# sbelharbi/tcam-wsol-video

Hardware: AMD Instinct MI355X
Metric: frames/sec CAM+bbox, ResNet50-TCAM 224×224, 1/2/4/8 MI355X (higher is better)
Workload: dtype fp32

## Files before the change

include/tcam_hip.h:

```cpp
#ifndef TCAM_HIP_H
#define TCAM_HIP_H

#include <stdint.h>

#ifdef __cplusplus
extern "C" {
#endif

#define TCAM_OK 0
#define TCAM_E_ARG (-1)
#define TCAM_E_NOMEM (-2)

int tcam_abi_version(void);
const char* tcam_arch(void);

typedef struct tcam_conv_src {
    const float* ptr;
    int C, H, W;
    int stride;
    int up2;
} tcam_conv_src;

int tcam_conv_weight_dims(int K, int Cout, int* Kpad, int* Mpad);

int tcam_conv2d(const tcam_conv_src* srcs, int nsrc, int B,
                const float* wt, const float* bias, const float* residual,
                float* out, int Cout, int Hout, int Wout,
                int KH, int KW, int pad, int relu, void* stream);

int tcam_conv_force_tile(int id);

int tcam_conv_x6_weight_dims(int K, int Cout, int* Kpad, int* Mpad);
size_t tcam_conv_x6_ws_bytes(void);
int tcam_conv2d_x6(const tcam_conv_src* srcs, int nsrc, int B,
                   const void* wt, const float* bias, const void* residual,
                   void* out, int Cout, int Hout, int Wout,
                   int KH, int KW, int pad_h, int pad_w, int relu,
                   int out_cstride, int out_coff, void* ws, size_t ws_bytes,
                   void* stream);
typedef struct tcam_conv_dst {
    void* ptr;
    int c_begin, cstride, coff;
} tcam_conv_dst;
int tcam_conv2d_x6_multi(const tcam_conv_src* srcs, int nsrc, int B,
                         const void* wt, const float* bias, int Cout, int Hout, int Wout,
                         int KH, int KW, int pad_h, int pad_w, int relu,
                         const tcam_conv_dst* dst, int ndst, void* ws, size_t ws_bytes,
                         void* stream);
int tcam_conv_x6_force_tile(int id);
int tcam_conv_x6_force_streamk(int grid);
int tcam_conv_x6_debug(int flags);

int tcam_s3_from_nchw(const float* in, void* out, int B, int C, int H, int W, int Cpad,
                      void* stream);
int tcam_s3_to_nchw(const void* in, float* out, int B, int C, int H, int W, void* stream);
int tcam_maxpool3x3s2_s3(const void* in, void* out, int B, int C, int H, int W, int Ho,
                         int Wo, void* stream);
int tcam_pool2d_s3(const void* in, void* out, int B, int C, int H, int W, int Ho, int Wo,
                   int KH, int KW, int stride, int pad, int mode, int out_cstride,
                   int out_coff, void* stream);
int tcam_up2_resize_s3(const void* in, void* out, int B, int C, int H, int W, int Ho, int Wo,
                       void* stream);
size_t tcam_wgap_s3_ws_bytes(int B, int C, int HW);
int tcam_wgap_s3(const void* x, const float* fc_w, const float* fc_b, float* logits,
                 float* mean, float* ws, int B, int C, int HW, int classes, void* stream);
int tcam_seghead_cam_s3(const void* x, const float* w, const float* b, float* fcams,
                        float* cam, uint8_t* cam_u8, int B, int Cin, int H, int W,
                        int argmax, void* stream);
int tcam_resize_cam(const float* fcams_in, float* fcams_out, float* cam, uint8_t* cam_u8,
                    int B, int Hi, int Wi, int Ho, int Wo, int argmax, void* stream);

int tcam_resize_ac_bwd(const float* dout, float* din, int BC, int Hi, int Wi, int Ho, int Wo,
                       void* stream);
int tcam_std_cam_s3(const void* A, const float* fc_w, const int32_t* cls, float* low,
                    float* cam, uint8_t* cam_u8, int B, int C, int h, int w, int Ho, int Wo,
                    void* stream);

int tcam_conv2d_f16x3(const tcam_conv_src* srcs, int nsrc, int B, const void* wt,
                      const float* wscale, const float* bias, const void* residual, void* out,
                      int Cout, int Hout, int Wout, int KH, int KW, int pad_h, int pad_w,
                      int relu, int out_cstride, int out_coff, int* oflow, void* ws,
                      size_t ws_bytes, void* stream);
int tcam_conv2d_f16x3_multi(const tcam_conv_src* srcs, int nsrc, int B, const void* wt,
                            const float* wscale, const float* bias, int Cout, int Hout,
                            int Wout, int KH, int KW, int pad_h, int pad_w, int relu,
                            const tcam_conv_dst* dst, int ndst, int* oflow, void* ws,
                            size_t ws_bytes, void* stream);
typedef struct tcam_conv_prob {
    tcam_conv_src src;
    const void* wt;
    const float* wscale;
    const float* bias;
    void* out;
    int Cout, Hout, Wout, KH, KW, pad_h, pad_w, relu, out_cstride, out_coff;
} tcam_conv_prob;
int tcam_conv2d_group(const tcam_conv_prob* probs, int nprob, int B, int fmt, int tile,
                      int* oflow, void* stream);
int tcam_stem_window(int KH, int KW, int stride, int* IR, int* IC);
int tcam_stem_f16x3(const float* img, const void* wt, const float* wscale, const float* bias,
                    const int32_t* ktab, int nk, void* out, int B, int C, int H, int W,
                    int Cout, int KH, int KW, int stride, int pad, int* oflow, void* stream);
int tcam_s2_from_nchw(const float* in, void* out, int B, int C, int H, int W, int Cpad,
                      void* stream);
int tcam_s2_to_nchw(const void* in, float* out, int B, int C, int H, int W, void* stream);
int tcam_maxpool3x3s2_s2(const void* in, void* out, int B, int C, int H, int W, int Ho,
                         int Wo, void* stream);
int tcam_pool2d_s2(const void* in, void* out, int B, int C, int H, int W, int Ho, int Wo,
                   int KH, int KW, int stride, int pad, int mode, int out_cstride,
                   int out_coff, void* stream);
int tcam_up2_resize_s2(const void* in, void* out, int B, int C, int H, int W, int Ho, int Wo,
                       void* stream);
int tcam_wgap_s2(const void* x, const float* fc_w, const float* fc_b, float* logits,
                 float* mean, float* ws, int B, int C, int HW, int classes, void* stream);
int tcam_seghead_cam_s2(const void* x, const float* w, const float* b, float* fcams,
                        float* cam, uint8_t* cam_u8, int B, int Cin, int H, int W,
                        int argmax, void* stream);
int tcam_std_cam_s2(const void* A, const float* fc_w, const int32_t* cls, float* low,
                    float* cam, uint8_t* cam_u8, int B, int C, int h, int w, int Ho, int Wo,
                    void* stream);

int tcam_conv2d_f16(const tcam_conv_src* srcs, int nsrc, int B, const void* wt,
                    const float* bias, const void* residual, void* out, int Cout, int Hout,
                    int Wout, int KH, int KW, int pad_h, int pad_w, int relu, int out_cstride,
                    int out_coff, void* ws, size_t ws_bytes, void* stream);
int tcam_s1_from_nchw(const float* in, void* out, int B, int C, int H, int W, int Cpad,
                      void* stream);
int tcam_s1_to_nchw(const void* in, float* out, int B, int C, int H, int W, void* stream);
int tcam_maxpool3x3s2_s1(const void* in, void* out, int B, int C, int H, int W, int Ho,
                         int Wo, void* stream);
int tcam_pool2d_s1(const void* in, void* out, int B, int C, int H, int W, int Ho, int Wo,
                   int KH, int KW, int stride, int pad, int mode, int out_cstride,
                   int out_coff, void* stream);
int tcam_up2_resize_s1(const void* in, void* out, int B, int C, int H, int W, int Ho, int Wo,
                       void* stream);
int tcam_wgap_s1(const void* x, const float* fc_w, const float* fc_b, float* logits,
                 float* mean, float* ws, int B, int C, int HW, int classes, void* stream);
int tcam_seghead_cam_s1(const void* x, const float* w, const float* b, float* fcams,
                        float* cam, uint8_t* cam_u8, int B, int Cin, int H, int W,
                        int argmax, void* stream);
int tcam_std_cam_s1(const void* A, const float* fc_w, const int32_t* cls, float* low,
                    float* cam, uint8_t* cam_u8, int B, int C, int h, int w, int Ho, int Wo,
                    void* stream);

int tcam_maxpool3x3s2(const float* in, float* out, int B, int C, int H, int W,
                      int Ho, int Wo, void* stream);

int tcam_up2_resize(const float* in, float* out, int B, int C, int H, int W,
                    int Ho, int Wo, void* stream);

int tcam_wgap(const float* x, const float* fc_w, const float* fc_b,
              float* logits, float* ws, int B, int C, int HW, int classes,
              void* stream);

int tcam_seghead_cam(const float* x, const float* w, const float* b,
                     float* fcams, float* cam, uint8_t* cam_u8,
                     int B, int Cin, int H, int W, int argmax, void* stream);

int tcam_std_cam(const float* A, const float* fc_w, const int32_t* cls,
                 float* low, float* cam, uint8_t* cam_u8, int B, int C,
                 int h, int w, int Ho, int Wo, void* stream);

int tcam_temporal_max(const float* cams, const int32_t* idx, float* out,
                      int M, int k1, int hw, float t, void* stream);

int tcam_temporal_cam(const float* cams, int N, const int32_t* idx, float* out,
                      uint8_t* out_u8, int M, int k1, int hw, float t, float* scale_ws,
                      void* stream);

int tcam_topk_flags(const float* logits, const int32_t* target, int32_t* top1,
                    int32_t* top5, int B, int C, void* stream);

void tcam_bbox_set_chunks(int n);
size_t tcam_bbox_ws_bytes(int B, int H, int W);
int tcam_bbox_levels(const uint8_t* cam_u8, int32_t* boxes, int32_t* vmax,
                     void* ws, int B, int H, int W, void* stream);

int tcam_bbox_set_debug(uint64_t* buf);
int tcam_bbox_fill_variant(int v);
int tcam_s2_to_s3(const void* in, void* out, long groups, void* stream);
int tcam_s3_to_s2(const void* in, void* out, long groups, void* stream);
int tcam_bbox_scan_line(const uint8_t* p, const uint8_t* u, uint8_t* out, int n, int mode,
                        void* stream);
int tcam_bbox_level_variant(int v);
int tcam_bbox_set_inc_debug(uint64_t* buf);

int tcam_box_accumulate(const int32_t* boxes, const int32_t* vmax,
                        const double* taus, int T, const int32_t* gt,
                        const int32_t* ngt, int G, const int32_t* top1,
                        const int32_t* top5, const double* iou_thr, int n_iou,
                        int32_t* counters, double* best_iou, int B,
                        void* stream);

size_t tcam_bbox_multi_ws_bytes(int B, int H, int W);
int tcam_bbox_multi_iou(const uint8_t* cam_u8, const int32_t* gt, const int32_t* ngt, int G,
                        double* iou, int32_t* vmax, int32_t* canon, void* ws, int B, int H,
                        int W, void* stream);
int tcam_box_accumulate_multi(const double* iou, const int32_t* canon, const int32_t* vmax,
                              const double* taus, int T, const int32_t* gt,
                              const int32_t* ngt, int G, const int32_t* top1,
                              const int32_t* top5, const double* iou_thr, int n_iou,
                              int32_t* counters, double* best_iou, int B, void* stream);
size_t tcam_bbox_contours_ws_bytes(int H, int W);
int tcam_bbox_contours(const uint8_t* cam_u8, int level, int32_t* records, int cap,
                       int32_t* count, void* ws, int H, int W, void* stream);

int tcam_flag_count(const int32_t* flags, int B, int32_t* acc, void* stream);

size_t tcam_bilateral_ws_bytes(int N, int K, int H, int W, int dim);
int tcam_bilateral_batch(const float* images, const float* ins, float* outs,
                         void* ws, size_t ws_bytes, int N, int K, int H, int W,
                         float s_rgb, float s_xy, void* stream);

int tcam_bilateral_prepare(const float* images, void* ws, size_t ws_bytes, int N, int K,
                           int H, int W, float s_rgb, float s_xy, void* stream);
int tcam_bilateral_apply(const float* ins, float* outs, void* ws, size_t ws_bytes, int N,
                         int K, int H, int W, float s_rgb, float s_xy, void* stream);

int tcam_colorbilateral_batch(const float* images, const float* ins, float* outs,
                              void* ws, size_t ws_bytes, int N, int K, int H, int W,
                              float s_rgb, int dim, void* stream);

int tcam_bilateral_status(const void* ws, int N, int* status);
void tcam_bilateral_set_debug(void* dbg);

void bilateralfilter_batch(float* images, int len_images, float* ins,
                           int len_ins, float* outs, int len_outs, int N,
                           int K, int H, int W, float sigmargb,
                           float sigmaxy);
void colorbilateralfilter_batch(float* images, int len_images, float* ins,
                                int len_ins, float* outs, int len_outs, int N,
                                int K, int H, int W, float sigmargb, int DIM);

size_t tcam_crf_energy_ws_bytes(void);
int tcam_crf_energy(const float* seg, const float* as, long n, int N, float* loss,
                    float* ws, void* stream);
int tcam_crf_grad(const float* as, const float* grad_out, long n, int N, float* grad,
                  void* stream);


size_t tcam_bn_ws_bytes(long P, int C);
int tcam_bn_stats_s3(const void* y, long P, int C, float eps, float momentum, float* mean,
                     float* invstd, float* run_mean, float* run_var, void* ws, void* stream);
int tcam_bn_relu_s3(const void* y, const float* mean, const float* invstd, const float* gamma,
                    const float* beta, void* out, long P, int C, void* stream);
int tcam_bn_relu_bwd_s3(const void* dout, const void* out, const void* y, const float* mean,
                        const float* invstd, const float* gamma, void* dy, float* dgamma,
                        float* dbeta, long P, int C, void* ws, void* stream);
int tcam_up2_bwd_s3(const void* gup, void* gx, int B, int C, int H, int W, void* stream);
size_t tcam_conv_wgrad_ws_bytes(const tcam_conv_src* srcs, int nsrc, int B, int Cout,
                                int Hout, int Wout, int KH, int KW);
int tcam_conv_wgrad_s3(const tcam_conv_src* srcs, int nsrc, int B, const void* dy, int Cout,
                       int Hout, int Wout, int KH, int KW, int pad_h, int pad_w,
                       int cout_store, float* dw, void* ws, size_t ws_bytes, void* stream);
int tcam_conv_wgrad_s3_f16x3(const tcam_conv_src* srcs, int nsrc, int B, const void* dy,
                             int Cout, int Hout, int Wout, int KH, int KW, int pad_h, int pad_w,
                             int cout_store, float* dw, void* ws, size_t ws_bytes, int* oflow,
                             void* stream);
int tcam_bn_stats_s2(const void* y, long P, int C, float eps, float momentum, float* mean,
                     float* invstd, float* run_mean, float* run_var, void* ws, void* stream);
int tcam_bn_relu_s2(const void* y, const float* mean, const float* invstd, const float* gamma,
                    const float* beta, void* out, long P, int C, void* stream);
int tcam_bn_relu_bwd_s3s2(const void* dout, const void* out, const void* y, const float* mean,
                          const float* invstd, const float* gamma, void* dy, float* dgamma,
                          float* dbeta, long P, int C, void* ws, uint32_t* amax, void* stream);
int tcam_dy_scaled_s2(const void* dy, long P, int C, uint32_t* amax, int compute, float* scale,
                      void* dy2, void* stream);
size_t tcam_bn_bwd_scaled_ws_bytes(long P, int C);
int tcam_bn_relu_bwd_scaled_s3s2(const void* dout, const void* out, const void* y,
                                 const float* mean, const float* invstd, const float* gamma,
                                 const float* beta, void* dy3, void* dy2, float* scale,
                                 float* dgamma, float* dbeta, long P, int C, void* ws,
                                 void* stream);
int tcam_bn_relu_bwd_fused_s1(const void* dout, const void* out, const void* y,
                              const float* mean, const float* invstd, const float* gamma,
                              const float* beta, void* dy, float* dgamma, float* dbeta, long P,
                              int C, void* ws, void* stream);
int tcam_conv_wgrad_s2_f16x3(const tcam_conv_src* srcs, int nsrc, int B, const void* dy2,
                             const float* dscale, int Cout, int Hout, int Wout, int KH, int KW,
                             int pad_h, int pad_w, int cout_store, float* dw, void* ws,
                             size_t ws_bytes, void* stream);
int tcam_pack_weight_f16x3(const float* w, void* out, float* wscale, int mode, int CoutW,
                           int CtotW, int KH, int KW, int c0, int cout_sel, int cin_pad,
                           const float* kdiv, void* stream);
typedef struct tcam_pack_item {
    const float* w;
    void* out;
    float* wscale;
    const float* kdiv;
    int mode, CoutW, CtotW, KH, KW, c0, cout_sel, cin_pad;
} tcam_pack_item;
size_t tcam_pack_table_bytes(int n);
int tcam_pack_weights(const tcam_pack_item* items, int n, int f16x3, void* table, void* stream);
int tcam_bottleneck_f16x3(const void* x, int B, int H, int W, int cin, const void* w1,
                          const float* s1, const float* b1, const void* w2, const float* s2,
                          const float* b2, const void* w3, const float* s3, const float* b3,
                          int ds, void* out, int* oflow, void* stream);
int tcam_bottleneck_f16(const void* x, int B, int H, int W, int cin, const void* w1,
                        const float* b1, const void* w2, const float* b2, const void* w3,
                        const float* b3, int ds, void* out, void* stream);
void tcam_bottleneck_set_debug(void* dbg);
int tcam_conv2d_f16x3_s3out(const tcam_conv_src* srcs, int nsrc, int B, const void* wt,
                            const float* wscale, const float* bias, void* out, int Cout,
                            int Hout, int Wout, int KH, int KW, int pad_h, int pad_w, int relu,
                            int out_cstride, int out_coff, void* ws, size_t ws_bytes,
                            void* stream);
int tcam_timer_arm(void* start, void* stop);
int tcam_wgrad_force_fp32(int on);
int tcam_pack_weight_x6(const float* w, void* out, int mode, int CoutW, int CtotW, int KH,
                        int KW, int c0, int cout_sel, int cin_pad, void* stream);
int tcam_up2_resize_bwd_s3(const void* g, void* gx, int B, int C, int H, int W, int Ho, int Wo,
                           void* stream);
size_t tcam_chansum_ws_bytes(int B, int C, long HW);
int tcam_chansum_nchw(const float* x, int B, int C, long HW, float* out, void* ws,
                      void* stream);
int tcam_softmax2(const float* fcams, float* S, int B, long HW, void* stream);
size_t tcam_tcam_loss_ws_bytes(int B, long HW);
int tcam_tcam_losses(const float* fcams, const float* S, const int32_t* seeds, const float* AS,
                     int B, long HW, float lam_sl, float lam_crf, float lam_size, float elb_t,
                     float* losses, float* dfcams, void* ws, void* stream);
int tcam_tcam_losses_ex(const float* fcams, const float* S, const int32_t* seeds,
                        const float* AS, const float* gx, const float* extra, int B, long HW,
                        float lam_sl, float lam_crf, float lam_size, float elb_t, float* losses,
                        float* dfcams, void* ws, void* stream);
size_t tcam_tcam_loss_terms_ws_bytes(int B, long HW);
int tcam_tcam_losses_terms(const float* fcams, const float* S, const int32_t* seeds,
                           const float* AS, const float* gx, const float* extra,
                           const float* fg_size, const float* msk, int B, long HW,
                           float lam_sl, float lam_crf, float lam_size, float elb_t,
                           float lam_bgfg, float lam_fgsz, float lam_eob, float t_bgfg,
                           float t_fgsz, float t_eob, float eps, float* losses, float* dfcams,
                           void* ws, void* stream);
int tcam_teacher_stats(const float* cams, const uint8_t* roi, const int32_t* bbox, int B,
                       int H, int W, float* msk, float* fg_size, void* stream);
int tcam_mosaic_gather(const float* src, const int32_t* idx, int G, int L, int C, int H, int W,
                       float* out, void* stream);
int tcam_mosaic_scatter(const float* mosaic, const int32_t* occ_start, const int32_t* occ,
                        int B, int L, int C, int H, int W, float coef, int accumulate,
                        float* dst, void* stream);
int tcam_sgd_step(float* p, const float* g, float* buf, long n, float lr, float momentum,
                  float dampening, float weight_decay, int nesterov, int first,
                  float grad_scale, void* stream);
int tcam_sgd_step_gated(float* p, const float* g, float* buf, long n, float lr, float momentum,
                        float dampening, float weight_decay, int nesterov, float grad_scale,
                        const float* gate, int* steps, int* skipped, void* stream);

int tcam_bn_stats_s1(const void* y, long P, int C, float eps, float momentum, float* mean,
                     float* invstd, float* run_mean, float* run_var, void* ws, void* stream);
int tcam_bn_relu_s1(const void* y, const float* mean, const float* invstd, const float* gamma,
                    const float* beta, void* out, long P, int C, void* stream);
int tcam_bn_relu_bwd_s1(const void* dout, const void* out, const void* y, const float* mean,
                        const float* invstd, const float* gamma, void* dy, float* dgamma,
                        float* dbeta, long P, int C, void* ws, void* stream);
int tcam_up2_bwd_s1(const void* gup, void* gx, int B, int C, int H, int W, void* stream);
int tcam_up2_resize_bwd_s1(const void* g, void* gx, int B, int C, int H, int W, int Ho, int Wo,
                           void* stream);
int tcam_conv_wgrad_s1(const tcam_conv_src* srcs, int nsrc, int B, const void* dy, int Cout,
                       int Hout, int Wout, int KH, int KW, int pad_h, int pad_w,
                       int cout_store, float* dw, void* ws, size_t ws_bytes, void* stream);
int tcam_pack_weight_f16(const float* w, void* out, int mode, int CoutW, int CtotW, int KH,
                         int KW, int c0, int cout_sel, int cin_pad, void* stream);
int tcam_amp_unscale(float* g, long n, const float* scale, float* found_inf, void* stream);
int tcam_sgd_step_amp(float* p, const float* g, float* buf, long n, float lr, float momentum,
                      float dampening, float weight_decay, int nesterov, float grad_scale,
                      const float* gate, int* steps, int* skipped, float* scale, int* tracker,
                      float growth_factor, float backoff_factor, int growth_interval,
                      void* stream);

int tcam_bn_add_relu_s2(const void* y, const float* mean, const float* invstd, const float* gamma,
                        const float* beta, const void* yd, const float* meand,
                        const float* invstdd, const float* gammad, const float* betad,
                        const void* res, void* out, long P, int C, void* stream);
int tcam_bn_add_relu_s1(const void* y, const float* mean, const float* invstd, const float* gamma,
                        const float* beta, const void* yd, const float* meand,
                        const float* invstdd, const float* gammad, const float* betad,
                        const void* res, void* out, long P, int C, void* stream);
int tcam_grad_add_mask_s3s2(const void* a, const void* d, const void* o, void* r, long P, int C,
                            void* stream);
int tcam_grad_add_mask_s1(const void* a, const void* d, const void* o, void* r, long P, int C,
                          void* stream);
size_t tcam_maxpool_bwd_ws_bytes(int B, int C, int Ho, int Wo);
int tcam_maxpool3x3s2_bwd_s3s2(const void* gout, const void* x, void* gin, void* ws, int B, int C,
                               int H, int W, int Ho, int Wo, void* stream);
int tcam_maxpool3x3s2_bwd_s1(const void* gout, const void* x, void* gin, void* ws, int B, int C,
                             int H, int W, int Ho, int Wo, void* stream);
int tcam_zero_up2(const void* in, void* out, int gbytes, int B, int C, int H, int W, int Hi,
                  int Wi, void* stream);
int tcam_im2col(const void* x, void* out, int gbytes, int B, int C, int H, int W, int KH, int KW,
                int stride, int pad, int Ho, int Wo, void* stream);
size_t tcam_wgrad11_ws_bytes(int B, int Cin, int Hin, int Win, int stride, int Cout, int Ho,
                             int Wo);
int tcam_wgrad11_s2_f16x3(const void* x, int B, int Cin, int Hin, int Win, int stride,
                          const void* dy2, const float* dscale, int Cout, int Ho, int Wo,
                          float* dw, void* ws, size_t ws_bytes, void* stream);
int tcam_wgrad11_s1(const void* x, int B, int Cin, int Hin, int Win, int stride, const void* dy,
                    int Cout, int Ho, int Wo, float* dw, void* ws, size_t ws_bytes, void* stream);
size_t tcam_conv_wgrad_generic_ws_bytes(const tcam_conv_src* srcs, int nsrc, int B, int Cout,
                                        int Hout, int Wout, int KH, int KW);
int tcam_conv_wgrad_s3s2(const tcam_conv_src* srcs, int nsrc, int B, const void* dy, int Cout,
                         int Hout, int Wout, int KH, int KW, int pad_h, int pad_w,
                         int cout_store, float* dw, void* ws, size_t ws_bytes, void* stream);
size_t tcam_cls_pool_ws_bytes(int B, int C);
int tcam_cls_fwd_s2(const void* x, int B, long HW, int C, const float* w, const float* bias,
                    int K, float* pooled, float* logits, void* ws, void* stream);
int tcam_cls_fwd_s1(const void* x, int B, long HW, int C, const float* w, const float* bias,
                    int K, float* pooled, float* logits, void* ws, void* stream);
int tcam_ce_loss(const float* logits, const int32_t* labels, int B, int K, float lam,
                 const float* gscale, float* loss, float* dlogits, void* stream);
int tcam_cls_bwd(const float* dlogits, const float* pooled, const float* w, int B, int K, int C,
                 int r16, float* dw, float* db, float* dpooled, void* stream);
int tcam_pool_bwd_s3(const float* dpooled, int B, long HW, int C, void* dout, void* stream);
int tcam_pool_bwd_s1(const float* dpooled, int B, long HW, int C, void* dout, void* stream);

size_t tcam_relu_bwd_ws_bytes(long P, int C);
int tcam_relu_bwd_s3s2(const void* dout, const void* out, void* dz, float* db, uint32_t* amax,
                       long P, int C, void* ws, size_t ws_bytes, void* stream);
int tcam_relu_bwd_s1(const void* dout, const void* out, void* dz, float* db, uint32_t* amax,
                     long P, int C, void* ws, size_t ws_bytes, void* stream);
int tcam_maxpool2x2_bwd_s3s2(const void* gout, const void* x, void* gin, int B, int C, int H,
                             int W, int Ho, int Wo, void* stream);
int tcam_maxpool2x2_bwd_s1(const void* gout, const void* x, void* gin, int B, int C, int H, int W,
                           int Ho, int Wo, void* stream);

size_t tcam_seeder_ws_bytes(int B, int H, int W);
int tcam_prepare_std_cams(const float* cams, float* out, int B, int h, int w, int Ho, int Wo,
                          void* stream);
int tcam_tcam_seeder(const float* cams, const uint8_t* roi, int32_t* seeds, int B, int H,
                     int W, int seed_tech, int min_, int max_, float max_p, float min_p,
                     int fg_erode_k, int fg_erode_iter, int ksz, int ignore_idx,
                     int roi_method, double p_min_area_roi, int use_roi,
                     unsigned long long seed, unsigned long long offset, uint8_t* roi_out,
                     float* th_out, void* ws, size_t ws_bytes, void* stream);
int tcam_get_roi(const float* cams, int B, int H, int W, int roi_method,
                 double p_min_area_roi, double thresh, const double* thresh_b,
                 uint8_t* roi_out, int32_t* bbox_out, float* th_out, void* ws,
                 size_t ws_bytes, void* stream);
int tcam_stotsu_roi_thresh(const float* cams, int B, int h, int w, int S, float* th_out,
                           void* stream);

int tcam_resample_coeffs(int in_size, int out_size, int* bounds, int* kk);
int tcam_frames_preprocess(const uint8_t* frames, int B, int Hin, int Win, const int* bh,
                           const int* kh, int ksh, int Rw, const int* bv, const int* kv,
                           int ksv, int Rh, const int* crop, const uint8_t* flip, int th,
                           int tw, const float* mean3, const float* std3, float* norm,
                           float* raw, uint8_t* u8, void* stream);


#define TCAM_JPEG_E_NOTJPEG (-20)
#define TCAM_JPEG_E_UNSUPPORTED (-21)
#define TCAM_JPEG_E_CORRUPT (-22)
int tcam_jpeg_pack(const uint8_t* const* data, const size_t* len, int n, void* blob,
                   size_t cap, int64_t* sizes, int* dims);
int tcam_jpeg_decode(const void* host_blob, const void* dev_blob, void* ws, size_t ws_bytes,
                     uint8_t* out, void* stream);
int tcam_jpeg_debug_rounds(const void* host_blob, int* dev_rounds);

#ifdef __cplusplus
}
#endif
#endif
```

tcam_wsol_video_amd/_lib.py:

```python
from __future__ import annotations

import ctypes as C
import os

_HERE = os.path.dirname(os.path.abspath(__file__))
LIB_PATH = os.environ.get("TCAM_LIB_PATH") or os.path.join(_HERE, "libtcam_hip.so")

_lib = None


class NativeLibraryError(RuntimeError):
    pass


class tcam_conv_src(C.Structure):
    _fields_ = [("ptr", C.c_void_p), ("C", C.c_int), ("H", C.c_int), ("W", C.c_int),
                ("stride", C.c_int), ("up2", C.c_int)]


class tcam_pack_item(C.Structure):
    _fields_ = [("w", C.c_void_p), ("out", C.c_void_p), ("wscale", C.c_void_p),
                ("kdiv", C.c_void_p), ("mode", C.c_int), ("CoutW", C.c_int), ("CtotW", C.c_int),
                ("KH", C.c_int), ("KW", C.c_int), ("c0", C.c_int), ("cout_sel", C.c_int),
                ("cin_pad", C.c_int)]


class tcam_conv_dst(C.Structure):
    _fields_ = [("ptr", C.c_void_p), ("c_begin", C.c_int), ("cstride", C.c_int),
                ("coff", C.c_int)]


class tcam_conv_prob(C.Structure):
    _fields_ = [("src", tcam_conv_src), ("wt", C.c_void_p), ("wscale", C.c_void_p),
                ("bias", C.c_void_p), ("out", C.c_void_p)] + [
        (n, C.c_int) for n in ("Cout", "Hout", "Wout", "KH", "KW", "pad_h", "pad_w", "relu",
                               "out_cstride", "out_coff")]


_P = C.c_void_p
_I = C.c_int
_F = C.c_float

SIGNATURES = {
    "tcam_abi_version": (_I, []),
    "tcam_arch": (C.c_char_p, []),
    "tcam_conv2d": (_I, [C.POINTER(tcam_conv_src), _I, _I, _P, _P, _P, _P, _I, _I, _I,
                         _I, _I, _I, _I, _P]),
    "tcam_conv_weight_dims": (_I, [_I, _I, C.POINTER(_I), C.POINTER(_I)]),
    "tcam_conv_force_tile": (_I, [_I]),
    "tcam_conv2d_x6": (_I, [C.POINTER(tcam_conv_src), _I, _I, _P, _P, _P, _P, _I, _I, _I,
                            _I, _I, _I, _I, _I, _I, _I, _P, C.c_size_t, _P]),
    "tcam_conv2d_x6_multi": (_I, [C.POINTER(tcam_conv_src), _I, _I, _P, _P, _I, _I, _I, _I,
                                  _I, _I, _I, _I, C.POINTER(tcam_conv_dst), _I, _P, C.c_size_t,
                                  _P]),
    "tcam_conv2d_f16x3": (_I, [C.POINTER(tcam_conv_src), _I, _I, _P, _P, _P, _P, _P, _I, _I,
                               _I, _I, _I, _I, _I, _I, _I, _I, _P, _P, C.c_size_t, _P]),
    "tcam_conv2d_f16x3_multi": (_I, [C.POINTER(tcam_conv_src), _I, _I, _P, _P, _P, _I, _I,
                                     _I, _I, _I, _I, _I, _I, C.POINTER(tcam_conv_dst), _I, _P,
                                     _P, C.c_size_t, _P]),
    "tcam_conv2d_group": (_I, [C.POINTER(tcam_conv_prob), _I, _I, _I, _I, _P, _P]),
    "tcam_conv_x6_ws_bytes": (C.c_size_t, []),
    "tcam_conv_x6_weight_dims": (_I, [_I, _I, C.POINTER(_I), C.POINTER(_I)]),
    "tcam_conv_x6_force_tile": (_I, [_I]),
    "tcam_wgrad_force_fp32": (_I, [_I]),
    "tcam_resample_coeffs": (_I, [_I, _I, _P, _P]),
    "tcam_frames_preprocess": (_I, [_P, _I, _I, _I, _P, _P, _I, _I, _P, _P, _I, _I, _P, _P,
                                    _I, _I, C.POINTER(_F), C.POINTER(_F), _P, _P, _P, _P]),
    "tcam_jpeg_pack": (_I, [_P, _P, _I, _P, C.c_size_t, _P, _P]),
    "tcam_jpeg_decode": (_I, [_P, _P, _P, C.c_size_t, _P, _P]),
    "tcam_jpeg_debug_rounds": (_I, [_P, _P]),
    "tcam_conv_x6_force_streamk": (_I, [_I]),
    "tcam_conv_x6_debug": (_I, [_I]),
    "tcam_s3_from_nchw": (_I, [_P, _P, _I, _I, _I, _I, _I, _P]),
    "tcam_s3_to_nchw": (_I, [_P, _P, _I, _I, _I, _I, _P]),
    "tcam_maxpool3x3s2_s3": (_I, [_P, _P, _I, _I, _I, _I, _I, _I, _P]),
    "tcam_up2_resize_s3": (_I, [_P, _P, _I, _I, _I, _I, _I, _I, _P]),
    "tcam_pool2d_s3": (_I, [_P, _P, _I, _I, _I, _I, _I, _I, _I, _I, _I, _I, _I, _I, _I, _P]),
    "tcam_wgap_s3_ws_bytes": (C.c_size_t, [_I, _I, _I]),
    "tcam_wgap_s3": (_I, [_P, _P, _P, _P, _P, _P, _I, _I, _I, _I, _P]),
    "tcam_seghead_cam_s3": (_I, [_P, _P, _P, _P, _P, _P, _I, _I, _I, _I, _I, _P]),
    "tcam_resize_cam": (_I, [_P, _P, _P, _P, _I, _I, _I, _I, _I, _I, _P]),
    "tcam_resize_ac_bwd": (_I, [_P, _P, _I, _I, _I, _I, _I, _P]),
    "tcam_std_cam_s3": (_I, [_P, _P, _P, _P, _P, _P, _I, _I, _I, _I, _I, _I, _P]),
    "tcam_s2_from_nchw": (_I, [_P, _P, _I, _I, _I, _I, _I, _P]),
    "tcam_s2_to_nchw": (_I, [_P, _P, _I, _I, _I, _I, _P]),
    "tcam_maxpool3x3s2_s2": (_I, [_P, _P, _I, _I, _I, _I, _I, _I, _P]),
    "tcam_up2_resize_s2": (_I, [_P, _P, _I, _I, _I, _I, _I, _I, _P]),
    "tcam_pool2d_s2": (_I, [_P, _P, _I, _I, _I, _I, _I, _I, _I, _I, _I, _I, _I, _I, _I, _P]),
    "tcam_wgap_s2": (_I, [_P, _P, _P, _P, _P, _P, _I, _I, _I, _I, _P]),
    "tcam_seghead_cam_s2": (_I, [_P, _P, _P, _P, _P, _P, _I, _I, _I, _I, _I, _P]),
    "tcam_std_cam_s2": (_I, [_P, _P, _P, _P, _P, _P, _I, _I, _I, _I, _I, _I, _P]),
    "tcam_maxpool3x3s2": (_I, [_P, _P, _I, _I, _I, _I, _I, _I, _P]),
    "tcam_up2_resize": (_I, [_P, _P, _I, _I, _I, _I, _I, _I, _P]),
    "tcam_wgap": (_I, [_P, _P, _P, _P, _P, _I, _I, _I, _I, _P]),
    "tcam_seghead_cam": (_I, [_P, _P, _P, _P, _P, _P, _I, _I, _I, _I, _I, _P]),
    "tcam_std_cam": (_I, [_P, _P, _P, _P, _P, _P, _I, _I, _I, _I, _I, _I, _P]),
    "tcam_temporal_max": (_I, [_P, _P, _P, _I, _I, _I, _F, _P]),
    "tcam_temporal_cam": (_I, [_P, _I, _P, _P, _P, _I, _I, _I, _F, _P, _P]),
    "tcam_topk_flags": (_I, [_P, _P, _P, _P, _I, _I, _P]),
    "tcam_bbox_ws_bytes": (C.c_size_t, [_I, _I, _I]),
    "tcam_bbox_multi_ws_bytes": (C.c_size_t, [_I, _I, _I]),
    "tcam_bbox_multi_iou": (_I, [_P, _P, _P, _I, _P, _P, _P, _P, _I, _I, _I, _P]),
    "tcam_box_accumulate_multi": (_I, [_P, _P, _P, _P, _I, _P, _P, _I, _P, _P, _P, _I, _P, _P,
                                       _I, _P]),
    "tcam_bbox_contours_ws_bytes": (C.c_size_t, [_I, _I]),
    "tcam_bbox_contours": (_I, [_P, _I, _P, _I, _P, _P, _I, _I, _P]),
    "tcam_flag_count": (_I, [_P, _I, _P, _P]),
    "tcam_bbox_levels": (_I, [_P, _P, _P, _P, _I, _I, _I, _P]),
    "tcam_bbox_scan_line": (_I, [_P, _P, _P, _I, _I, _P]),
    "tcam_s2_to_s3": (_I, [_P, _P, C.c_long, _P]),
    "tcam_s3_to_s2": (_I, [_P, _P, C.c_long, _P]),
    "tcam_bbox_set_debug": (_I, [_P]),
    "tcam_bbox_fill_variant": (_I, [_I]),
    "tcam_bbox_level_variant": (_I, [_I]),
    "tcam_bbox_set_inc_debug": (_I, [_P]),
    "tcam_box_accumulate": (_I, [_P, _P, _P, _I, _P, _P, _I, _P, _P, _P, _I, _P, _P, _I,
                                 _P]),
    "tcam_bilateral_ws_bytes": (C.c_size_t, [_I, _I, _I, _I, _I]),
    "tcam_bilateral_batch": (_I, [_P, _P, _P, _P, C.c_size_t, _I, _I, _I, _I, _F, _F, _P]),
    "tcam_bilateral_prepare": (_I, [_P, _P, C.c_size_t, _I, _I, _I, _I, _F, _F, _P]),
    "tcam_bilateral_apply": (_I, [_P, _P, _P, C.c_size_t, _I, _I, _I, _I, _F, _F, _P]),
    "tcam_colorbilateral_batch": (_I, [_P, _P, _P, _P, C.c_size_t, _I, _I, _I, _I, _F, _I,
                                       _P]),
    "tcam_bilateral_status": (_I, [_P, _I, C.POINTER(_I)]),
    "tcam_bilateral_set_debug": (None, [_P]),
    "tcam_crf_energy_ws_bytes": (C.c_size_t, []),
    "tcam_bn_ws_bytes": (C.c_size_t, [C.c_long, _I]),
    "tcam_bn_stats_s3": (_I, [_P, C.c_long, _I, _F, _F, _P, _P, _P, _P, _P, _P]),
    "tcam_bn_relu_s3": (_I, [_P, _P, _P, _P, _P, _P, C.c_long, _I, _P]),
    "tcam_bn_relu_bwd_s3": (_I, [_P, _P, _P, _P, _P, _P, _P, _P, _P, C.c_long, _I, _P, _P]),
    "tcam_up2_bwd_s3": (_I, [_P, _P, _I, _I, _I, _I, _P]),
    "tcam_conv_wgrad_ws_bytes": (C.c_size_t, [C.POINTER(tcam_conv_src), _I, _I, _I, _I, _I,
                                              _I, _I]),
    "tcam_conv_wgrad_s3": (_I, [C.POINTER(tcam_conv_src), _I, _I, _P, _I, _I, _I, _I, _I, _I,
                                _I, _I, _P, _P, C.c_size_t, _P]),
    "tcam_timer_arm": (_I, [_P, _P]),
    "tcam_bn_stats_s2": (_I, [_P, C.c_long, _I, _F, _F, _P, _P, _P, _P, _P, _P]),
    "tcam_bn_relu_s2": (_I, [_P, _P, _P, _P, _P, _P, C.c_long, _I, _P]),
    "tcam_bn_relu_bwd_s3s2": (_I, [_P, _P, _P, _P, _P, _P, _P, _P, _P, C.c_long, _I, _P, _P,
                                   _P]),
    "tcam_dy_scaled_s2": (_I, [_P, C.c_long, _I, _P, _I, _P, _P, _P]),
    "tcam_bn_bwd_scaled_ws_bytes": (C.c_size_t, [C.c_long, _I]),
    "tcam_bn_relu_bwd_scaled_s3s2": (_I, [_P, _P, _P, _P, _P, _P, _P, _P, _P, _P, _P, _P,
                                          C.c_long, _I, _P, _P]),
    "tcam_bn_relu_bwd_fused_s1": (_I, [_P, _P, _P, _P, _P, _P, _P, _P, _P, _P, C.c_long, _I,
                                       _P, _P]),
    "tcam_conv_wgrad_s2_f16x3": (_I, [C.POINTER(tcam_conv_src), _I, _I, _P, _P, _I, _I, _I, _I,
                                      _I, _I, _I, _I, _P, _P, C.c_size_t, _P]),
    "tcam_pack_weight_f16x3": (_I, [_P, _P, _P, _I, _I, _I, _I, _I, _I, _I, _I, _P, _P]),
    "tcam_pack_table_bytes": (C.c_size_t, [_I]),
    "tcam_pack_weights": (_I, [_P, _I, _I, _P, _P]),
    "tcam_bottleneck_set_debug": (None, [_P]),
    "tcam_bbox_set_chunks": (None, [_I]),
    "tcam_bottleneck_f16": (_I, [_P, _I, _I, _I, _I, _P, _P, _P, _P, _P, _P, _I, _P, _P]),
    "tcam_bottleneck_f16x3": (_I, [_P, _I, _I, _I, _I, _P, _P, _P, _P, _P, _P, _P, _P, _P, _I,
                                   _P, _P, _P]),
    "tcam_conv2d_f16x3_s3out": (_I, [C.POINTER(tcam_conv_src), _I, _I, _P, _P, _P, _P, _I, _I,
                                     _I, _I, _I, _I, _I, _I, _I, _I, _P, C.c_size_t, _P]),
    "tcam_conv_wgrad_s3_f16x3": (_I, [C.POINTER(tcam_conv_src), _I, _I, _P, _I, _I, _I, _I, _I,
                                      _I, _I, _I, _P, _P, C.c_size_t, _P, _P]),
    "tcam_pack_weight_x6": (_I, [_P, _P, _I, _I, _I, _I, _I, _I, _I, _I, _P]),
    "tcam_up2_resize_bwd_s3": (_I, [_P, _P, _I, _I, _I, _I, _I, _I, _P]),
    "tcam_chansum_ws_bytes": (C.c_size_t, [_I, _I, C.c_long]),
    "tcam_chansum_nchw": (_I, [_P, _I, _I, C.c_long, _P, _P, _P]),
    "tcam_softmax2": (_I, [_P, _P, _I, C.c_long, _P]),
    "tcam_tcam_loss_ws_bytes": (C.c_size_t, [_I, C.c_long]),
    "tcam_tcam_losses": (_I, [_P, _P, _P, _P, _I, C.c_long, _F, _F, _F, _F, _P, _P, _P, _P]),
    "tcam_tcam_losses_ex": (_I, [_P, _P, _P, _P, _P, _P, _I, C.c_long, _F, _F, _F, _F, _P, _P,
                                 _P, _P]),
    "tcam_tcam_loss_terms_ws_bytes": (C.c_size_t, [_I, C.c_long]),
    "tcam_tcam_losses_terms": (_I, [_P, _P, _P, _P, _P, _P, _P, _P, _I, C.c_long] + [_F] * 11 +
                               [_P, _P, _P, _P]),
    "tcam_teacher_stats": (_I, [_P, _P, _P, _I, _I, _I, _P, _P, _P]),
    "tcam_mosaic_gather": (_I, [_P, _P, _I, _I, _I, _I, _I, _P, _P]),
    "tcam_mosaic_scatter": (_I, [_P, _P, _P, _I, _I, _I, _I, _I, _F, _I, _P, _P]),
    "tcam_sgd_step": (_I, [_P, _P, _P, C.c_long, _F, _F, _F, _F, _I, _I, _F, _P]),
    "tcam_sgd_step_gated": (_I, [_P, _P, _P, C.c_long, _F, _F, _F, _F, _I, _F, _P, _P, _P,
                                 _P]),
    "tcam_seeder_ws_bytes": (C.c_size_t, [_I, _I, _I]),
    "tcam_prepare_std_cams": (_I, [_P, _P, _I, _I, _I, _I, _I, _P]),
    "tcam_tcam_seeder": (_I, [_P, _P, _P, _I, _I, _I, _I, _I, _I, _F, _F, _I, _I, _I, _I, _I,
                              C.c_double, _I, C.c_ulonglong, C.c_ulonglong, _P, _P, _P,
                              C.c_size_t, _P]),
    "tcam_get_roi": (_I, [_P, _I, _I, _I, _I, C.c_double, C.c_double, _P, _P, _P, _P, _P,
                          C.c_size_t, _P]),
    "tcam_stotsu_roi_thresh": (_I, [_P, _I, _I, _I, _I, _P, _P]),
    "tcam_crf_energy": (_I, [_P, _P, C.c_long, _I, _P, _P, _P]),
    "tcam_crf_grad": (_I, [_P, _P, C.c_long, _I, _P, _P]),
    "tcam_stem_window": (_I, [_I, _I, _I, C.POINTER(_I), C.POINTER(_I)]),
    "tcam_stem_f16x3": (_I, [_P, _P, _P, _P, _P, _I, _P, _I, _I, _I, _I, _I, _I, _I, _I, _I,
                             _P, _P]),
    "tcam_conv2d_f16": (_I, [C.POINTER(tcam_conv_src), _I, _I, _P, _P, _P, _P, _I, _I, _I,
                             _I, _I, _I, _I, _I, _I, _I, _P, C.c_size_t, _P]),
    "tcam_s1_from_nchw": (_I, [_P, _P, _I, _I, _I, _I, _I, _P]),
    "tcam_s1_to_nchw": (_I, [_P, _P, _I, _I, _I, _I, _P]),
    "tcam_maxpool3x3s2_s1": (_I, [_P, _P, _I, _I, _I, _I, _I, _I, _P]),
    "tcam_up2_resize_s1": (_I, [_P, _P, _I, _I, _I, _I, _I, _I, _P]),
    "tcam_pool2d_s1": (_I, [_P, _P, _I, _I, _I, _I, _I, _I, _I, _I, _I, _I, _I, _I, _I, _P]),
    "tcam_wgap_s1": (_I, [_P, _P, _P, _P, _P, _P, _I, _I, _I, _I, _P]),
    "tcam_seghead_cam_s1": (_I, [_P, _P, _P, _P, _P, _P, _I, _I, _I, _I, _I, _P]),
    "tcam_std_cam_s1": (_I, [_P, _P, _P, _P, _P, _P, _I, _I, _I, _I, _I, _I, _P]),
    "tcam_bn_stats_s1": (_I, [_P, C.c_long, _I, _F, _F, _P, _P, _P, _P, _P, _P]),
    "tcam_bn_relu_s1": (_I, [_P, _P, _P, _P, _P, _P, C.c_long, _I, _P]),
    "tcam_bn_relu_bwd_s1": (_I, [_P, _P, _P, _P, _P, _P, _P, _P, _P, C.c_long, _I, _P, _P]),
    "tcam_up2_bwd_s1": (_I, [_P, _P, _I, _I, _I, _I, _P]),
    "tcam_up2_resize_bwd_s1": (_I, [_P, _P, _I, _I, _I, _I, _I, _I, _P]),
    "tcam_conv_wgrad_s1": (_I, [C.POINTER(tcam_conv_src), _I, _I, _P, _I, _I, _I, _I, _I, _I,
                                _I, _I, _P, _P, C.c_size_t, _P]),
    "tcam_pack_weight_f16": (_I, [_P, _P, _I, _I, _I, _I, _I, _I, _I, _I, _P]),
    "tcam_amp_unscale": (_I, [_P, C.c_long, _P, _P, _P]),
    "tcam_sgd_step_amp": (_I, [_P, _P, _P, C.c_long, _F, _F, _F, _F, _I, _F, _P, _P, _P, _P,
                               _P, _F, _F, _I, _P]),
    "tcam_bn_add_relu_s2": (_I, [_P, _P, _P, _P, _P, _P, _P, _P, _P, _P, _P, _P, C.c_long, _I,
                                 _P]),
    "tcam_bn_add_relu_s1": (_I, [_P, _P, _P, _P, _P, _P, _P, _P, _P, _P, _P, _P, C.c_long, _I,
                                 _P]),
    "tcam_grad_add_mask_s3s2": (_I, [_P, _P, _P, _P, C.c_long, _I, _P]),
    "tcam_grad_add_mask_s1": (_I, [_P, _P, _P, _P, C.c_long, _I, _P]),
    "tcam_maxpool_bwd_ws_bytes": (C.c_size_t, [_I, _I, _I, _I]),
    "tcam_maxpool3x3s2_bwd_s3s2": (_I, [_P, _P, _P, _P, _I, _I, _I, _I, _I, _I, _P]),
    "tcam_maxpool3x3s2_bwd_s1": (_I, [_P, _P, _P, _P, _I, _I, _I, _I, _I, _I, _P]),
    "tcam_zero_up2": (_I, [_P, _P, _I, _I, _I, _I, _I, _I, _I, _P]),
    "tcam_im2col": (_I, [_P, _P, _I, _I, _I, _I, _I, _I, _I, _I, _I, _I, _I, _P]),
    "tcam_wgrad11_ws_bytes": (C.c_size_t, [_I, _I, _I, _I, _I, _I, _I, _I]),
    "tcam_wgrad11_s2_f16x3": (_I, [_P, _I, _I, _I, _I, _I, _P, _P, _I, _I, _I, _P, _P,
                                   C.c_size_t, _P]),
    "tcam_wgrad11_s1": (_I, [_P, _I, _I, _I, _I, _I, _P, _I, _I, _I, _P, _P, C.c_size_t, _P]),
    "tcam_conv_wgrad_generic_ws_bytes": (C.c_size_t, [C.POINTER(tcam_conv_src), _I, _I, _I, _I,
                                                      _I, _I, _I]),
    "tcam_conv_wgrad_s3s2": (_I, [C.POINTER(tcam_conv_src), _I, _I, _P, _I, _I, _I, _I, _I, _I,
                                  _I, _I, _P, _P, C.c_size_t, _P]),
    "tcam_cls_pool_ws_bytes": (C.c_size_t, [_I, _I]),
    "tcam_cls_fwd_s2": (_I, [_P, _I, C.c_long, _I, _P, _P, _I, _P, _P, _P, _P]),
    "tcam_cls_fwd_s1": (_I, [_P, _I, C.c_long, _I, _P, _P, _I, _P, _P, _P, _P]),
    "tcam_ce_loss": (_I, [_P, _P, _I, _I, _F, _P, _P, _P, _P]),
    "tcam_cls_bwd": (_I, [_P, _P, _P, _I, _I, _I, _I, _P, _P, _P, _P]),
    "tcam_pool_bwd_s3": (_I, [_P, _I, C.c_long, _I, _P, _P]),
    "tcam_pool_bwd_s1": (_I, [_P, _I, C.c_long, _I, _P, _P]),
    "tcam_relu_bwd_ws_bytes": (C.c_size_t, [C.c_long, _I]),
    "tcam_relu_bwd_s3s2": (_I, [_P, _P, _P, _P, _P, C.c_long, _I, _P, C.c_size_t, _P]),
    "tcam_relu_bwd_s1": (_I, [_P, _P, _P, _P, _P, C.c_long, _I, _P, C.c_size_t, _P]),
    "tcam_maxpool2x2_bwd_s3s2": (_I, [_P, _P, _P, _I, _I, _I, _I, _I, _I, _P]),
    "tcam_maxpool2x2_bwd_s1": (_I, [_P, _P, _P, _I, _I, _I, _I, _I, _I, _P]),
    "bilateralfilter_batch": (None, [_P, _I, _P, _I, _P, _I, _I, _I, _I, _I, _F, _F]),
    "colorbilateralfilter_batch": (None, [_P, _I, _P, _I, _P, _I, _I, _I, _I, _I, _F, _I]),
}


def load(path: str = LIB_PATH):
    global _lib
    if _lib is not None:
        return _lib
    if not os.path.exists(path):
        raise NativeLibraryError(
            f"{path} not found: build it with `python -c 'import __graft_entry__ as g; "
            f"g.build()'` (hipcc --offload-arch=gfx950). There is no CPU fallback.")
    lib = C.CDLL(path)
    for name, (res, args) in SIGNATURES.items():
        fn = getattr(lib, name)
        fn.restype = res
        fn.argtypes = args
    _lib = lib
    return lib


def check(rc: int, what: str) -> None:
    if rc != 0:
        raise RuntimeError(f"{what} failed with code {rc}")
```

tcam_wsol_video_amd/csrc/bbox.hip:

```cpp
#include "common.h"

namespace {

constexpr int MAXH = 256, MAXW = 256;
constexpr int MAXP = 260;
constexpr int BIGH = 320, BIGW = 320;
constexpr int BIGP = 324;
constexpr uint32_t INACT = 0xFFFFFFFFu;
constexpr int NTB = 1024;
constexpr int DBG_SLOTS = 16;
uint64_t* g_dbg = nullptr;
int g_fill_waves = NTB / 64;
int g_fill_maxit = 1 << 30;
int g_fill_variant = 0;
int g_level_variant = 0;
int g_bbox_chunks = 0;
uint64_t* g_inc_dbg = nullptr;

__device__ inline uint64_t rt() { return __builtin_amdgcn_s_memrealtime(); }

__host__ __device__ inline int pitch_of(int W) {
    int d = (W + 3) / 4;
    if ((d & 1) == 0) d += 1;
    return 4 * d;
}

__device__ inline int block_max_i(int v, int* red) {
    v = wave_max_i(v);
    const int lane = threadIdx.x & 63, wid = threadIdx.x >> 6;
    __syncthreads();
    if (lane == 0) red[wid] = v;
    __syncthreads();
    if (threadIdx.x == 0) {
        int m = red[0];
        for (int i = 1; i < NTB / 64; ++i) m = max(m, red[i]);
        red[NTB / 64] = m;
    }
    __syncthreads();
    return red[NTB / 64];
}
__device__ inline int block_min_i(int v, int* red) {
    return -block_max_i(-v, red);
}

__device__ void emit_sorted(const uint8_t* psi, int P, const int* hist, int* cur, int H, int W,
                            int b, uint16_t* __restrict__ slist, int32_t* __restrict__ cgt) {
    const int tid = threadIdx.x, nt = blockDim.x;
    __syncthreads();
    if (tid < 64) {
        int h[4], own = 0;
#pragma unroll
        for (int k = 0; k < 4; ++k) {
            h[k] = hist[4 * tid + 1 + k];
            own += h[k];
        }
        int incl = own;
#pragma unroll
        for (int o = 1; o < 64; o <<= 1) {
            const int t = __shfl_down(incl, o, 64);
            if (tid + o < 64) incl += t;
        }
        int above = incl - own;
        int32_t* cg = cgt + (long)b * 257;
#pragma unroll
        for (int k = 3; k >= 0; --k) {
            above += h[k];
            cg[4 * tid + k] = above;
            cur[4 * tid + k] = above;
        }
        if (tid == 0) cg[256] = 0;
    }
    __syncthreads();
    uint16_t* out = slist + (long)b * H * W;
    for (int i = tid; i < H * W; i += nt) {
        const int y = i / W, x = i - y * W;
        const int v = psi[y * P + x];
        if (v) out[atomicAdd(&cur[v], 1)] = (uint16_t)(y << 8 | x);
    }
}

template <int MH, int MP, bool IMG_LDS>
__global__ __launch_bounds__(NTB) void fill_kernel(const uint8_t* __restrict__ cam_u8,
                                                   uint8_t* __restrict__ psi_out,
                                                   int32_t* __restrict__ vmax_out,
                                                   int32_t* __restrict__ canon,
                                                   int32_t* __restrict__ lev_list,
                                                   int32_t* __restrict__ nlev, int H, int W,
                                                   uint64_t* __restrict__ dbg,
                                                   uint16_t* __restrict__ slist,
                                                   int32_t* __restrict__ cgt) {
    const uint64_t t0 = rt();
    __shared__ uint8_t img[IMG_LDS ? MH * MP : 4];
    __shared__ uint8_t psi[MH * MP];
    __shared__ int red[NTB / 64 + 1];
    __shared__ int hist[257];
    __shared__ int cur[257];
    __shared__ int changed;
    const int b = blockIdx.x;
    const int P = pitch_of(W);
    const uint8_t* src = cam_u8 + (long)b * H * W;
    int vm = 0;
    for (int i0 = threadIdx.x; i0 < H * W; i0 += 8 * NTB) {
        uint8_t v[8];
#pragma unroll
        for (int u = 0; u < 8; ++u) {
            const int i = i0 + u * NTB;
            v[u] = i < H * W ? src[i] : 0;
        }
#pragma unroll
        for (int u = 0; u < 8; ++u) {
            const int i = i0 + u * NTB;
            if (i >= H * W) continue;
            const int y = i / W, x = i - y * W;
            if (IMG_LDS) img[y * P + x] = v[u];
            psi[y * P + x] = 255;
            vm = max(vm, (int)v[u]);
        }
    }
    vm = block_max_i(vm, red);
    if (threadIdx.x == 0) vmax_out[b] = vm;
    const uint64_t t1 = rt();
    int iters = 0;
    const int nd = (W + 3) / 4;
    for (;;) {
        if (threadIdx.x == 0) changed = 0;
        __syncthreads();
        int ch = 0;
        if (threadIdx.x < H) {
            uint32_t* prow = reinterpret_cast<uint32_t*>(psi + threadIdx.x * P);
            const uint32_t* irow = reinterpret_cast<const uint32_t*>(img + threadIdx.x * P);
            const uint8_t* grow = src + threadIdx.x * W;
            auto idw = [&](int d) -> uint32_t {
                if (IMG_LDS) return irow[d];
                uint32_t v = 0;
#pragma unroll
                for (int e = 0; e < 4; ++e)
                    if (4 * d + e < W) v |= (uint32_t)grow[4 * d + e] << (8 * e);
                return v;
            };
            int prev = -1;
            uint32_t pv = prow[0], iv = idw(0);
            for (int d = 0; d < nd; ++d) {
                const uint32_t pn = d + 1 < nd ? prow[d + 1] : 0u;
                const uint32_t in = d + 1 < nd ? idw(d + 1) : 0u;
                uint32_t o = pv;
#pragma unroll
                for (int e = 0; e < 4; ++e) {
                    if (4 * d + e < W) {
                        const int c = (pv >> (8 * e)) & 255, u = (iv >> (8 * e)) & 255;
                        const int nv = max(u, min(c, prev));
                        prev = nv;
                        o = (o & ~(255u << (8 * e))) | ((uint32_t)nv << (8 * e));
                    }
                }
                if (o != pv) { prow[d] = o; ch = 1; }
                pv = pn;
                iv = in;
            }
            prev = -1;
            pv = prow[nd - 1];
            iv = idw(nd - 1);
            for (int d = nd - 1; d >= 0; --d) {
                const uint32_t pn = d > 0 ? prow[d - 1] : 0u;
                const uint32_t in = d > 0 ? idw(d - 1) : 0u;
                uint32_t o = pv;
#pragma unroll
                for (int e = 3; e >= 0; --e) {
                    if (4 * d + e < W) {
                        const int c = (pv >> (8 * e)) & 255, u = (iv >> (8 * e)) & 255;
                        const int nv = max(u, min(c, prev));
                        prev = nv;
                        o = (o & ~(255u << (8 * e))) | ((uint32_t)nv << (8 * e));
                    }
                }
                if (o != pv) { prow[d] = o; ch = 1; }
                pv = pn;
                iv = in;
            }
        }
        __syncthreads();
        if (threadIdx.x < W) {
            const int x = threadIdx.x;
            auto iat = [&](int y) -> int {
                return IMG_LDS ? (int)img[y * P + x] : (int)src[y * W + x];
            };
            int prev = -1;
            int c[4], u[4], cn[4], un[4];
#pragma unroll
            for (int e = 0; e < 4; ++e) {
                c[e] = e < H ? psi[e * P + x] : 0;
                u[e] = e < H ? iat(e) : 0;
            }
            for (int y0 = 0; y0 < H; y0 += 4) {
#pragma unroll
                for (int e = 0; e < 4; ++e) {
                    const int y = y0 + 4 + e;
                    cn[e] = y < H ? psi[y * P + x] : 0;
                    un[e] = y < H ? iat(y) : 0;
                }
#pragma unroll
                for (int e = 0; e < 4; ++e) {
                    const int y = y0 + e;
                    if (y < H) {
                        const int nv = max(u[e], min(c[e], prev));
                        if (nv != c[e]) { psi[y * P + x] = (uint8_t)nv; ch = 1; }
                        prev = nv;
                    }
                }
#pragma unroll
                for (int e = 0; e < 4; ++e) { c[e] = cn[e]; u[e] = un[e]; }
            }
            prev = -1;
            const int top = ((H - 1) / 4) * 4;
#pragma unroll
            for (int e = 0; e < 4; ++e) {
                const int y = top + e;
                c[e] = y < H ? psi[y * P + x] : 0;
                u[e] = y < H ? iat(y) : 0;
            }
            for (int y0 = top; y0 >= 0; y0 -= 4) {
#pragma unroll
                for (int e = 0; e < 4; ++e) {
                    const int y = y0 - 4 + e;
                    cn[e] = y >= 0 ? psi[y * P + x] : 0;
                    un[e] = y >= 0 ? iat(y) : 0;
                }
#pragma unroll
                for (int e = 3; e >= 0; --e) {
                    const int y = y0 + e;
                    if (y < H) {
                        const int nv = max(u[e], min(c[e], prev));
                        if (nv != c[e]) { psi[y * P + x] = (uint8_t)nv; ch = 1; }
                        prev = nv;
                    }
                }
#pragma unroll
                for (int e = 0; e < 4; ++e) { c[e] = cn[e]; u[e] = un[e]; }
            }
        }
        if (ch) changed = 1;
        __syncthreads();
        ++iters;
        if (!__builtin_amdgcn_readfirstlane(changed)) break;
        __syncthreads();
    }
    const uint64_t t2 = rt();
    uint8_t* dst = psi_out + (long)b * H * W;
    for (int i = threadIdx.x; i < 257; i += NTB) hist[i] = 0;
    __syncthreads();
    for (int i = threadIdx.x; i < H * W; i += NTB) {
        int y = i / W, x = i - y * W;
        const uint8_t v = psi[y * P + x];
        dst[i] = v;
        atomicAdd(&hist[v], 1);
    }
    __syncthreads();
    if (threadIdx.x == 0) {
        int n = 0, next = vm - 1;
        for (int L = vm - 1; L >= 0; --L) {
            if (hist[L + 1] > 0) next = L;
            canon[b * 256 + L] = next;
        }
        for (int L = 0; L < vm; ++L)
            if (hist[L + 1] > 0) lev_list[b * 256 + n++] = L;
        nlev[b] = n;
        if (dbg) {
            uint64_t* d = dbg + (long)b * DBG_SLOTS;
            d[0] = t1 - t0; d[1] = t2 - t1; d[2] = rt() - t2; d[3] = iters; d[4] = n;
        }
    }
    if (slist) emit_sorted(psi, P, hist, cur, H, W, b, slist, cgt);
}

constexpr int NTF = 256;

template <int LDN>
__device__ __forceinline__ bool sweep_line(uint32_t (&pl)[LDN], const uint32_t (&ul)[LDN]) {
    uint32_t diff = 0;
    int prev = -1;
#pragma unroll
    for (int d = 0; d < LDN; ++d) {
        const uint32_t w = pl[d];
        uint32_t uw = ul[d];
        asm volatile("" : "+v"(uw));
        const int n0 = max((int)(uw & 255u), min((int)(w & 255u), prev));
        const int n1 = max((int)((uw >> 8) & 255u), min((int)((w >> 8) & 255u), n0));
        const int n2 = max((int)((uw >> 16) & 255u), min((int)((w >> 16) & 255u), n1));
        const int n3 = max((int)(uw >> 24), min((int)(w >> 24), n2));
        prev = n3;
        uint32_t o = (uint32_t)n0 | ((uint32_t)n1 << 8) | ((uint32_t)n2 << 16) |
                     ((uint32_t)n3 << 24);
        asm volatile("" : "+v"(o));
        diff |= o ^ w;
        pl[d] = o;
        __builtin_amdgcn_sched_barrier(0);
    }
    prev = -1;
#pragma unroll
    for (int d = LDN - 1; d >= 0; --d) {
        const uint32_t w = pl[d];
        uint32_t uw = ul[d];
        asm volatile("" : "+v"(uw));
        const int n3 = max((int)(uw >> 24), min((int)(w >> 24), prev));
        const int n2 = max((int)((uw >> 16) & 255u), min((int)((w >> 16) & 255u), n3));
        const int n1 = max((int)((uw >> 8) & 255u), min((int)((w >> 8) & 255u), n2));
        const int n0 = max((int)(uw & 255u), min((int)(w & 255u), n1));
        prev = n0;
        uint32_t o = (uint32_t)n0 | ((uint32_t)n1 << 8) | ((uint32_t)n2 << 16) |
                     ((uint32_t)n3 << 24);
        asm volatile("" : "+v"(o));
        diff |= o ^ w;
        pl[d] = o;
        __builtin_amdgcn_sched_barrier(0);
    }
    return diff != 0;
}

template <int LDN>
__global__ __launch_bounds__(NTF) void fill_reg_kernel(const uint8_t* __restrict__ cam_u8,
                                                       uint8_t* __restrict__ psi_out,
// ... 419 lines not shown
        a = find_root(lab, a);
        b = find_root(lab, b);
        if (a == b) return;
        if (a > b) { uint32_t t = a; a = b; b = t; }
        uint32_t old = atomicMin(&lab[b], a);
        if (old == b) return;
        b = old;
    }
}

struct LevelCtx {
    const uint32_t* bm;
    int H, W, wpr, BW;
    __device__ inline int bit(int y, int x) const {
        if ((unsigned)y >= (unsigned)H || (unsigned)x >= (unsigned)W) return 0;
        return (bm[y * wpr + (x >> 5)] >> (x & 31)) & 1;
    }
    __device__ inline int pair(int y, int x) const {
        if ((unsigned)y >= (unsigned)H || (unsigned)x >= (unsigned)W) return 0;
        return (bm[y * wpr + (x >> 5)] >> (x & 31)) & 3;
    }
    __device__ inline uint32_t word(int y, int j) const {
        if ((unsigned)y >= (unsigned)H || (unsigned)j >= (unsigned)wpr) return 0u;
        return bm[y * wpr + j];
    }
};

__device__ inline uint32_t root_of(const uint32_t* lab, uint32_t b) {
    uint32_t v = lab[b];
    return (v & RFLAG) ? b : v;
}

template <int LH, int LW, int QW>
__global__ __launch_bounds__(NTB) void level_kernel(const uint8_t* __restrict__ psi_g,
                                                    const int32_t* __restrict__ vmax,
                                                    const int32_t* __restrict__ lev_list,
                                                    const int32_t* __restrict__ nlev,
                                                    int32_t* __restrict__ boxes, int H, int W,
                                                    uint64_t* __restrict__ dbg) {
    uint64_t ph[8] = {0, 0, 0, 0, 0, 0, 0, 0};
    uint64_t tp = rt();
#define PHASE(k) do { if (dbg) { uint64_t t_ = rt(); ph[k] += t_ - tp; tp = t_; } } while (0)
    __shared__ uint32_t bm[LH * (LW / 32)];
    __shared__ uint32_t lab[(LH / 2) * (LW / 2)];
    __shared__ int red[4 * (NTB / 64) + 4];

    const int b = blockIdx.x / LEVEL_CHUNKS;
    const int chunk = blockIdx.x % LEVEL_CHUNKS;
    const int nl = __builtin_amdgcn_readfirstlane(nlev[b]);
    if (chunk >= nl) return;
    const int wpr = (W + 31) / 32;
    const int NW = H * wpr;
    const int BW = (W + 1) / 2, BH = (H + 1) / 2, NB = BH * BW;
    const int tid = threadIdx.x, lane = tid & 63, wid = tid >> 6;

    uint32_t pv[QW][8];
    const uint8_t* src = psi_g + (long)b * H * W;
#pragma unroll
    for (int q = 0; q < QW; ++q) {
        const int w = tid + q * NTB;
#pragma unroll
        for (int d = 0; d < 8; ++d) pv[q][d] = 0u;
        if (w < NW) {
            const int y = w / wpr, x0 = (w - y * wpr) * 32;
#pragma unroll
            for (int d = 0; d < 8; ++d) {
                uint32_t v = 0;
#pragma unroll
                for (int e = 0; e < 4; ++e) {
                    const int x = x0 + 4 * d + e;
                    if (x < W) v |= (uint32_t)src[y * W + x] << (8 * e);
                }
                pv[q][d] = v;
            }
        }
    }
    LevelCtx cx{bm, H, W, wpr, BW};

    for (int li = chunk; li < nl; li += LEVEL_CHUNKS) {
        const int L = lev_list[b * 256 + li];
        int32_t* box = boxes + ((long)b * 256 + L) * 4;
#pragma unroll
        for (int q = 0; q < QW; ++q) {
            const int w = tid + q * NTB;
            if (w < NW) {
                uint32_t bits = 0;
#pragma unroll
                for (int d = 0; d < 8; ++d)
#pragma unroll
                    for (int e = 0; e < 4; ++e)
                        bits |= (uint32_t)(((pv[q][d] >> (8 * e)) & 255u) > (uint32_t)L) << (4 * d + e);
                bm[w] = bits;
            }
        }
        __syncthreads();
        PHASE(0);
        for (int by = wid; by < BH; by += NTB / 64) {
            const int y = 2 * by;
            int carry = -1;
            for (int base = 0; base < BW; base += 64) {
                const int bx = base + lane;
                int t = 0, u = 0, tl = 0, ul = 0;
                if (bx < BW) {
                    t = cx.pair(y, 2 * bx);
                    u = cx.pair(y + 1, 2 * bx);
                    if (bx > 0) {
                        tl = cx.bit(y, 2 * bx - 1);
                        ul = cx.bit(y + 1, 2 * bx - 1);
                    }
                }
                const bool act = (t | u) != 0;
                const bool joined = act && ((t | u) & 1) && (tl | ul);
                const uint64_t starts = __ballot(act && !joined);
                const uint64_t acts = __ballot(act);
                const uint64_t below = lane == 63 ? starts : (starts & ((2ull << lane) - 1));
                int head = below ? base + 63 - __builtin_clzll(below) : carry;
                if (bx < BW) lab[by * BW + bx] = act ? (uint32_t)(by * BW + head) : INACT;
                const int last = __shfl(head, 63, 64);
                carry = ((acts >> 63) & 1) ? last : -1;
            }
        }
        __syncthreads();
        PHASE(1);
        for (int i0 = 0; i0 < NB; i0 += NTB) {
            const int i = i0 + tid;
            uint32_t hi = INACT, ht = INACT, hl = INACT, hr = INACT;
            if (i < NB && i >= BW) {
                hi = lab[i];
                if (hi != INACT) {
                    const int by = i / BW, bx = i - by * BW, y = 2 * by, x = 2 * bx;
                    const int top = cx.pair(y, x);
                    if (top) {
                        if (cx.pair(y - 1, x)) ht = lab[i - BW];
                        if (bx > 0 && (top & 1) && cx.bit(y - 1, x - 1)) hl = lab[i - BW - 1];
                        if (bx + 1 < BW && (top & 2) && cx.bit(y - 1, x + 2)) hr = lab[i - BW + 1];
                    }
                }
            }
            const uint32_t phi = __shfl_up(hi, 1, 64);
            const uint32_t pht = __shfl_up(ht, 1, 64);
            const uint32_t phr = __shfl_up(hr, 1, 64);
            const bool same_run = lane > 0 && phi == hi && (i % BW) != 0;
            auto seen = [&](uint32_t h) { return same_run && (h == pht || h == phr); };
            if (hi != INACT) {
                if (hl != INACT && !seen(hl)) unite(lab, hi, hl);
                if (ht != INACT && !seen(ht)) unite(lab, hi, ht);
                if (hr != INACT && !seen(hr)) unite(lab, hi, hr);
            }
        }
        __syncthreads();
        PHASE(2);
        for (;;) {
            int ch = 0;
            for (int i = tid; i < NB; i += NTB) {
                const uint32_t v = lab[i];
                if (v == INACT || v == (uint32_t)i) continue;
                const uint32_t w = lab[v];
                if (w != v) { lab[i] = w; ch = 1; }
            }
            ch = block_max_i(ch, red);
            if (!ch) break;
        }
        for (int i = tid; i < NB; i += NTB)
            if (lab[i] == (uint32_t)i) lab[i] = RFLAG;
        __syncthreads();
        PHASE(3);
        {
            const int nsj = (W + 1 + 31) / 32;
            const int nstrips = (H + 1) * nsj;
            const int per = (nstrips + NTB - 1) / NTB;
            uint32_t cr = INACT, cacc = 0;
            for (int st = tid * per; st < min(nstrips, (tid + 1) * per); ++st) {
                const int wy = st / nsj - 1, j = st % nsj;
                const uint32_t t0 = cx.word(wy, j), t1 = cx.word(wy + 1, j);
                const uint32_t tp = cx.word(wy, j - 1), bp = cx.word(wy + 1, j - 1);
                const uint32_t tl = (t0 << 1) | (tp >> 31), tr = t0;
                const uint32_t bl = (t1 << 1) | (bp >> 31), br = t1;
                uint32_t m3 = (tl & tr & (bl | br)) | (bl & br & (tl | tr));
                const uint32_t m4 = tl & tr & bl & br;
                const int nvalid = W + 1 - 32 * j;
                if (nvalid < 32) m3 &= (1u << nvalid) - 1u;
                while (m3) {
                    const int s0 = __builtin_ctz(m3);
                    const uint32_t rest = ~(m3 >> s0);
                    const int len = rest ? __builtin_ctz(rest) : 32 - s0;
                    const uint32_t run = (len >= 32 ? 0xFFFFFFFFu : ((1u << len) - 1u)) << s0;
                    const uint32_t contrib = __builtin_popcount(run) + __builtin_popcount(m4 & run);
                    const int wx = 32 * j - 1 + s0;
                    int py, px;
                    if ((tl >> s0) & 1) { py = wy; px = wx; }
                    else if ((tr >> s0) & 1) { py = wy; px = wx + 1; }
                    else if ((bl >> s0) & 1) { py = wy + 1; px = wx; }
                    else { py = wy + 1; px = wx + 1; }
                    const uint32_t r = root_of(lab, (py >> 1) * BW + (px >> 1));
                    if (r != cr) {
                        if (cr != INACT) atomicAdd(&lab[cr], cacc);
                        cr = r;
                        cacc = 0;
                    }
                    cacc += contrib;
                    m3 &= ~run;
                }
            }
            if (cr != INACT) atomicAdd(&lab[cr], cacc);
        }
        __syncthreads();
        PHASE(4);
        int ma = -1;
        for (int i = tid; i < NB; i += NTB) {
            const uint32_t v = lab[i];
            if (v != INACT && (v & RFLAG)) ma = max(ma, (int)(v & ~RFLAG));
        }
        ma = block_max_i(ma, red);
        for (int i = tid; i < NB; i += NTB) {
            const uint32_t v = lab[i];
            if (v != INACT && (v & RFLAG))
                lab[i] = ((int)(v & ~RFLAG) == ma) ? (RFLAG | 0x7FFFFFFEu) : NOKEY;
        }
        __syncthreads();
        for (int i = tid; i < NB; i += NTB) {
            if (lab[i] == INACT) continue;
            const uint32_t r = root_of(lab, i);
            const int by = i / BW;
            if ((int)r / BW != by || lab[r] == NOKEY) continue;
            const int x = 2 * (i - by * BW), y = 2 * by;
            const int top = cx.pair(y, x);
            int k;
            if (top & 1) k = y * W + x;
            else if (top & 2) k = y * W + x + 1;
            else if (cx.bit(y + 1, x)) k = (y + 1) * W + x;
            else k = (y + 1) * W + x + 1;
            atomicMin(&lab[r], RFLAG | (uint32_t)(k + 1));
        }
        __syncthreads();
        int best = 0;
        for (int i = tid; i < NB; i += NTB) {
            const uint32_t v = lab[i];
            if (v != INACT && (v & RFLAG) && v != NOKEY) best = max(best, (int)(v & ~RFLAG));
        }
        best = block_max_i(best, red);
        const int fp = best - 1;
        const uint32_t wroot = root_of(lab, ((fp / W) >> 1) * BW + ((fp % W) >> 1));
        PHASE(5);
        int x0 = W, y0 = H, x1 = -1, y1 = -1;
        for (int i = tid; i < NB; i += NTB) {
            if (lab[i] == INACT || root_of(lab, i) != wroot) continue;
            const int by = i / BW, x = 2 * (i - by * BW), y = 2 * by;
            const int top = cx.pair(y, x), bot = cx.pair(y + 1, x);
            if (top | bot) {
                x0 = min(x0, ((top | bot) & 1) ? x : x + 1);
                x1 = max(x1, ((top | bot) & 2) ? x + 1 : x);
                y0 = min(y0, top ? y : y + 1);
                y1 = max(y1, bot ? y + 1 : y);
            }
        }
        x0 = wave_min_i(x0); y0 = wave_min_i(y0);
        x1 = wave_max_i(x1); y1 = wave_max_i(y1);
        if (lane == 0) {
            red[4 * wid + 0] = x0; red[4 * wid + 1] = y0;
            red[4 * wid + 2] = x1; red[4 * wid + 3] = y1;
        }
        __syncthreads();
        if (tid == 0) {
            for (int w = 1; w < NTB / 64; ++w) {
                x0 = min(x0, red[4 * w + 0]); y0 = min(y0, red[4 * w + 1]);
                x1 = max(x1, red[4 * w + 2]); y1 = max(y1, red[4 * w + 3]);
            }
            box[0] = x0;
            box[1] = y0;
            box[2] = min(x1 + 1, W - 1);
            box[3] = min(y1 + 1, H - 1);
        }
        __syncthreads();
        PHASE(6);
    }
    if (dbg && tid == 0) {
        uint64_t* d = dbg + (long)(gridDim.x + blockIdx.x) * DBG_SLOTS;
        for (int k = 0; k < 7; ++k) d[k] = ph[k];
    }
#undef PHASE
}

__global__ void expand_kernel(const int32_t* __restrict__ canon, const int32_t* __restrict__ vmax,
                              int32_t* __restrict__ boxes, int B) {
    const int i = blockIdx.x * blockDim.x + threadIdx.x;
    if (i >= B * 256) return;
    const int b = i / 256, L = i % 256;
    if (L >= vmax[b]) return;
    const int c = canon[b * 256 + L];
    if (c == L) return;
    const int32_t* s = boxes + ((long)b * 256 + c) * 4;
    int32_t* d = boxes + ((long)b * 256 + L) * 4;
    d[0] = s[0]; d[1] = s[1]; d[2] = s[2]; d[3] = s[3];
}

__global__ void accumulate_kernel(const int32_t* __restrict__ boxes,
                                  const int32_t* __restrict__ vmax, const double* __restrict__ taus,
                                  int T, const int32_t* __restrict__ gt,
                                  const int32_t* __restrict__ ngt, int G,
                                  const int32_t* __restrict__ top1,
                                  const int32_t* __restrict__ top5,
                                  const double* __restrict__ iou_thr, int n_iou,
                                  int32_t* __restrict__ counters, double* __restrict__ best_iou,
                                  int B) {
    long id = (long)blockIdx.x * blockDim.x + threadIdx.x;
    if (id >= (long)B * T) return;
    const int b = (int)(id / T), i = (int)(id % T);
    const int vm = vmax[b];
    const int thr = (int)(taus[i] * (double)vm);
    int a0 = 0, a1 = 0, a2 = 0, a3 = 0;
    if (thr < vm) {
        const int32_t* bx = boxes + ((long)b * 256 + thr) * 4;
        a0 = bx[0]; a1 = bx[1]; a2 = bx[2]; a3 = bx[3];
    }
    double best = 0.0;
    const int ng = ngt[b];
    for (int g = 0; g < ng; ++g) {
        const int32_t* q = gt + ((long)b * G + g) * 4;
        long mnx = max(a0, q[0]), mny = max(a1, q[1]);
        long mxx = min(a2, q[2]), mxy = min(a3, q[3]);
        long inter = max(0L, mxx - mnx + 1) * max(0L, mxy - mny + 1);
        long area_a = (long)(a2 - a0 + 1) * (a3 - a1 + 1);
        long area_b = (long)(q[2] - q[0] + 1) * (q[3] - q[1] + 1);
        long den = area_a + area_b - inter;
        double iou = den <= 0 ? 0.0 : (double)inter / (double)den;
        if (g == 0 || iou > best) best = iou;
    }
    if (best_iou) best_iou[id] = best;
    for (int j = 0; j < n_iou; ++j) {
        if (best >= iou_thr[j]) {
            atomicAdd(&counters[(0 * n_iou + j) * T + i], 1);
            if (top1[b]) atomicAdd(&counters[(1 * n_iou + j) * T + i], 1);
            if (top5[b]) atomicAdd(&counters[(2 * n_iou + j) * T + i], 1);
        }
    }
}


constexpr int INC_CHUNKS = 1;
constexpr int INC_MAX_CHUNKS = 4;
constexpr int IH = 224, IW = 224, IWPR = 7, IBW = 112, INB = IBW * (IH / 2);

__device__ inline unsigned long long block_max_u64(unsigned long long v,
                                                   unsigned long long* red) {
#pragma unroll
    for (int o = 32; o > 0; o >>= 1) {
        const unsigned long long t = __shfl_xor(v, o, 64);
        v = t > v ? t : v;
    }
    const int lane = threadIdx.x & 63, wid = threadIdx.x >> 6;
    __syncthreads();
    if (lane == 0) red[wid] = v;
    __syncthreads();
    if (threadIdx.x == 0) {
        unsigned long long m = red[0];
        for (int i = 1; i < NTB / 64; ++i) m = red[i] > m ? red[i] : m;
        red[NTB / 64] = m;
    }
    __syncthreads();
    return red[NTB / 64];
}

constexpr int32_t AFLAG = 1 << 30, AMASK = AFLAG - 1;
constexpr int LCAP = INB * 2;

__device__ inline uint32_t find_root_pk(const uint32_t* pk, uint32_t x) {
    uint32_t p = pk[x] >> 16;
    while (p != x) {
        x = p;
        p = pk[x] >> 16;
    }
    return x;
}

__device__ inline void unite_pk(uint32_t* pk, uint32_t a, uint32_t b, uint32_t* hl, int* nh) {
    for (;;) {
        a = find_root_pk(pk, a);
        b = find_root_pk(pk, b);
        if (a == b) return;
        if (a > b) { uint32_t t = a; a = b; b = t; }
        const uint32_t old = atomicMin(&pk[b], a << 16 | 0xFFFFu);
        if ((old >> 16) == b) {
            hl[atomicAdd(nh, 1)] = b << 16 | (old & 0xFFFFu);
            return;
        }
        b = old >> 16;
    }
}

__device__ inline int win_contrib(int c) { return c == 4 ? 2 : (c == 3 ? 1 : 0); }

__global__ __launch_bounds__(NTB) void level_inc_kernel(const uint8_t* __restrict__ psi_g,
                                                        const int32_t* __restrict__ lev_list,
                                                        const int32_t* __restrict__ nlev,
                                                        int32_t* __restrict__ boxes, int H,
                                                        int W, uint32_t* __restrict__ plist_g,
                                                        uint32_t* __restrict__ hlist_g,
                                                        uint64_t* __restrict__ dbg, int nch) {
    uint64_t ph[8] = {0, 0, 0, 0, 0, 0, 0, 0};
    uint32_t n_full = 0, n_fallback = 0;
    uint64_t tp = rt();
#define IPHASE(k) do { if (dbg) { uint64_t t_ = rt(); ph[k] += t_ - tp; tp = t_; } } while (0)
    __shared__ uint32_t bm[IH * IWPR];
    __shared__ uint32_t db[IH * IWPR];
    __shared__ uint32_t pk[INB];
    __shared__ int32_t area[INB];
    __shared__ uint16_t lst[LCAP];
    __shared__ unsigned long long redl[NTB / 64 + 1];
    __shared__ int red[4 * (NTB / 64) + 4];
    __shared__ int wsum[NTB / 64 + 1];
    __shared__ int s_nhook;
    __shared__ unsigned long long s_pbest;
    const int b = blockIdx.x / nch, chunk = blockIdx.x % nch;
    uint32_t* plist = plist_g + (long)blockIdx.x * IH * IW;
    uint32_t* hlist = hlist_g + (long)blockIdx.x * INB;
    const int nl = __builtin_amdgcn_readfirstlane(nlev[b]);
    const int l0 = nl * chunk / nch, l1 = nl * (chunk + 1) / nch;
    if (l0 >= l1) return;
    const int wpr = (W + 31) / 32, NW = H * wpr;
    const int BW = (W + 1) / 2, BH = (H + 1) / 2, NB = BH * BW;
    const int tid = threadIdx.x, lane = tid & 63, wid = tid >> 6;
    constexpr int QW = 2;

    uint32_t pv[QW][8];
    const uint8_t* src = psi_g + (long)b * H * W;
#pragma unroll
    for (int q = 0; q < QW; ++q) {
        const int w = tid + q * NTB;
#pragma unroll
        for (int d = 0; d < 8; ++d) pv[q][d] = 0u;
        if (w < NW) {
            const int y = w / wpr, x0 = (w - y * wpr) * 32;
#pragma unroll
            for (int d = 0; d < 8; ++d) {
                uint32_t v = 0;
#pragma unroll
                for (int e = 0; e < 4; ++e) {
                    const int x = x0 + 4 * d + e;
                    if (x < W) v |= (uint32_t)src[y * W + x] << (8 * e);
                }
                pv[q][d] = v;
            }
        }
    }
    for (int i = tid; i < NB; i += NTB) {
        pk[i] = INACT;
        area[i] = 0;
    }
    if (tid == 0) s_pbest = 0;
    uint32_t ob[QW] = {0u, 0u};
    LevelCtx cx{bm, H, W, wpr, BW};
    uint32_t pwin = INACT;
    int bx0 = 0, by0 = 0, bx1 = 0, by1 = 0;
    auto isnew = [&](int y, int x) -> int {
        if ((unsigned)y >= (unsigned)H || (unsigned)x >= (unsigned)W) return 0;
        return (db[y * wpr + (x >> 5)] >> (x & 31)) & 1;
    };

    for (int li = l1 - 1; li >= l0; --li) {
        const int L = lev_list[b * 256 + li];
        uint32_t nb[QW], df[QW];
#pragma unroll
        for (int q = 0; q < QW; ++q) {
            const int w = tid + q * NTB;
            uint32_t bits = 0;
#pragma unroll
            for (int d = 0; d < 8; ++d)
#pragma unroll
                for (int e = 0; e < 4; ++e)
                    bits |= (uint32_t)(((pv[q][d] >> (8 * e)) & 255u) > (uint32_t)L) << (4 * d + e);
            nb[q] = w < NW ? bits : 0u;
            df[q] = nb[q] & ~ob[q];
            if (w < NW) {
                bm[w] = nb[q];
                db[w] = df[q];
            }
        }
        int cnt = __builtin_popcount(df[0]) + __builtin_popcount(df[1]);
        int incl = cnt;
#pragma unroll
        for (int o = 1; o < 64; o <<= 1) {
            const int t = __shfl_up(incl, o, 64);
            if (lane >= o) incl += t;
        }
        if (lane == 63) wsum[wid] = incl;
        __syncthreads();
        if (tid == 0) {
            s_nhook = 0;
            int acc = 0;
            for (int i = 0; i < NTB / 64; ++i) {
                const int t = wsum[i];
                wsum[i] = acc;
                acc += t;
            }
            wsum[NTB / 64] = acc;
        }
        __syncthreads();
        const int nnew = wsum[NTB / 64];
        const bool inl = nnew <= LCAP;
        {
            int pos = wsum[wid] + incl - cnt;
#pragma unroll
            for (int q = 0; q < QW; ++q) {
                uint32_t bits = df[q];
                const int w = tid + q * NTB, y = w / wpr, xb = (w - y * wpr) * 32;
                while (bits) {
                    const int x = xb + __builtin_ctz(bits);
                    bits &= bits - 1;
                    if (inl) lst[pos++] = (uint16_t)(y << 8 | x);
                    else plist[pos++] = (uint32_t)(y << 8 | x);
                }
            }
        }
        __syncthreads();
        const volatile uint32_t* plv = plist;
        auto newpx = [&](int it) -> uint32_t { return inl ? (uint32_t)lst[it] : plv[it]; };
        IPHASE(0);
        for (int it = tid; it < nnew; it += NTB) {
            const uint32_t pp = newpx(it);
            const int y = (int)(pp >> 8), x = (int)(pp & 255);
            const uint32_t blk = (y >> 1) * BW + (x >> 1);
            if (pk[blk] == INACT) pk[blk] = blk << 16 | 0xFFFFu;
        }
        __syncthreads();
        IPHASE(1);
        for (int it = tid; it < nnew * 8; it += NTB) {
            const uint32_t pp = newpx(it >> 3);
            const int y = (int)(pp >> 8), x = (int)(pp & 255);
            const int d = (it & 7) + ((it & 7) >= 4);
            const int dy = d / 3 - 1, dx = d % 3 - 1;
            if (!cx.bit(y + dy, x + dx)) continue;
            const uint32_t blk = (y >> 1) * BW + (x >> 1);
            const uint32_t nbk = ((y + dy) >> 1) * BW + ((x + dx) >> 1);
            if (nbk != blk) unite_pk(pk, blk, nbk, hlist, &s_nhook);
        }
        __syncthreads();
        IPHASE(2);
        const int nhook = s_nhook;
        const volatile uint32_t* hlv = hlist;
        for (int it = tid; it < nhook; it += NTB) {
            const uint32_t e = hlv[it], i = e >> 16, k = e & 0xFFFFu;
            if (k != 0xFFFFu) {
                const uint32_t r = find_root_pk(pk, i);
                atomicAdd(&area[r], area[i] & AMASK);
                atomicOr(&area[r], AFLAG);
                atomicMin(&pk[r], r << 16 | k);
                area[i] = 0;
            }
        }
        IPHASE(3);
        for (int it = tid; it < nnew * 4; it += NTB) {
            const uint32_t pp = newpx(it >> 2);
            const int y = (int)(pp >> 8), x = (int)(pp & 255);
            {
                const uint32_t r = find_root_pk(pk, (y >> 1) * BW + (x >> 1));
                if ((it & 3) == 0) atomicMin(&pk[r], r << 16 | (uint32_t)(y * W + x));
                int dsum = 0;
                {
                    const int wy = y - 1 + ((it >> 1) & 1), wx = x - 1 + (it & 1);
                    {
                        int cn = 0, co = 0;
                        bool owner = true;
#pragma unroll
                        for (int k = 0; k < 4; ++k) {
                            const int qy = wy + (k >> 1), qx = wx + (k & 1);
                            const int nbit = cx.bit(qy, qx), nw = isnew(qy, qx);
                            cn += nbit;
                            co += nbit & (nw ^ 1);
                            if (nw && (qy < y || (qy == y && qx < x))) owner = false;
                        }
                        if (owner) dsum += win_contrib(cn) - win_contrib(co);
                    }
                }
                if (dsum) atomicAdd(&area[r], dsum);
            }
        }
        __syncthreads();
        IPHASE(4);
#pragma unroll
        for (int q = 0; q < QW; ++q) ob[q] = nb[q];
        unsigned long long best = 0;
        auto cand = [&](uint32_t x) {
            const uint32_t r = find_root_pk(pk, x);
            if (r != x) pk[x] = r << 16 | 0xFFFFu;
            const unsigned long long a =
                ((unsigned long long)(uint32_t)(area[r] & AMASK) << 32) | (pk[r] & 0xFFFFu);
            best = a > best ? a : best;
        };
        for (int it = tid; it < nnew; it += NTB) {
            const uint32_t pp = newpx(it);
            cand(((pp >> 8) >> 1) * BW + ((pp & 255) >> 1));
        }
        for (int it = tid; it < nhook; it += NTB) cand(hlv[it] >> 16);
        if (tid == 0 && pwin != INACT) cand(pwin);
        IPHASE(5);
        best = block_max_u64(best, redl);
        if (__builtin_amdgcn_readfirstlane((int)(best < s_pbest))) {
            ++n_fallback;
            best = 0;
            for (int i = tid; i < NB; i += NTB) {
                const uint32_t v = pk[i];
                if ((v >> 16) == (uint32_t)i) {
                    const unsigned long long a =
                        ((unsigned long long)(uint32_t)(area[i] & AMASK) << 32) | (v & 0xFFFFu);
                    best = a > best ? a : best;
                }
            }
            best = block_max_u64(best, redl);
        }
        const uint32_t fp = (uint32_t)best;
        const uint32_t wb = ((fp / W) >> 1) * BW + ((fp % W) >> 1);
        const uint32_t wroot = find_root_pk(pk, wb);
        IPHASE(6);
        const bool grow = wroot == pwin && !(area[wroot] & AFLAG);
        n_full += grow ? 0 : 1;
        int x0 = W, y0 = H, x1 = -1, y1 = -1;
        if (grow) {
            for (int it = tid; it < nnew; it += NTB) {
                const uint32_t pp = newpx(it);
                const int y = (int)(pp >> 8), x = (int)(pp & 255);
                if ((pk[(y >> 1) * BW + (x >> 1)] >> 16) != wroot) continue;
                x0 = min(x0, x); x1 = max(x1, x);
                y0 = min(y0, y); y1 = max(y1, y);
            }
            if (tid == 0) {
                x0 = min(x0, bx0); y0 = min(y0, by0);
                x1 = max(x1, bx1); y1 = max(y1, by1);
            }
        } else
        for (int i = tid; i < NB; i += NTB) {
            const uint32_t w = pk[i];
            if (w == INACT) continue;
            const uint32_t v = w >> 16;
            const uint32_t r = v == (uint32_t)i ? v : find_root_pk(pk, i);
            if (r != v) pk[i] = r << 16 | 0xFFFFu;
            if (r != wroot) continue;
            const int by = i / BW, x = 2 * (i - by * BW), y = 2 * by;
            const int top = cx.pair(y, x), bot = cx.pair(y + 1, x);
            if (top | bot) {
                x0 = min(x0, ((top | bot) & 1) ? x : x + 1);
                x1 = max(x1, ((top | bot) & 2) ? x + 1 : x);
                y0 = min(y0, top ? y : y + 1);
                y1 = max(y1, bot ? y + 1 : y);
            }
        }
        x0 = wave_min_i(x0); y0 = wave_min_i(y0);
        x1 = wave_max_i(x1); y1 = wave_max_i(y1);
        if (lane == 0) {
            red[4 * wid + 0] = x0; red[4 * wid + 1] = y0;
            red[4 * wid + 2] = x1; red[4 * wid + 3] = y1;
        }
        __syncthreads();
        if (tid == 0) {
            for (int w = 1; w < NTB / 64; ++w) {
                x0 = min(x0, red[4 * w + 0]); y0 = min(y0, red[4 * w + 1]);
                x1 = max(x1, red[4 * w + 2]); y1 = max(y1, red[4 * w + 3]);
            }
            int32_t* box = boxes + ((long)b * 256 + L) * 4;
            box[0] = x0;
            box[1] = y0;
            box[2] = min(x1 + 1, W - 1);
            box[3] = min(y1 + 1, H - 1);
            bx0 = x0; by0 = y0; bx1 = x1; by1 = y1;
            area[wroot] &= AMASK;
            s_pbest = best;
        }
        pwin = wroot;
        __syncthreads();
        IPHASE(7);
    }
    if (dbg && tid == 0) {
        uint64_t* d = dbg + (long)blockIdx.x * DBG_SLOTS;
        for (int k = 0; k < 8; ++k) d[k] = ph[k];
        d[8] = l1 - l0;
        d[9] = n_full;
        d[10] = n_fallback;
    }
#undef IPHASE
}

constexpr int SCAP = INB;
constexpr uint32_t SAMASK = (1u << 17) - 1;
constexpr uint32_t XR_EMPTY = 0x00FFu;

__device__ inline uint32_t lds_ld(const uint32_t* p) { return *(const volatile uint32_t*)p; }

__device__ inline void ar_max_y1(uint32_t* w, uint32_t y) {
    uint32_t old = lds_ld(w);
    while ((old >> 24) < y) {
        const uint32_t prev = atomicCAS(w, old, (old & 0x00FFFFFFu) | (y << 24));
        if (prev == old) return;
        old = prev;
    }
}

__device__ inline void xr_widen(uint32_t* xr, uint32_t r, uint32_t x0, uint32_t x1) {
    uint32_t* w = xr + (r >> 1);
    const int sh = (int)(r & 1u) * 16;
    uint32_t old = lds_ld(w);
    for (;;) {
        const uint32_t cur = (old >> sh) & 0xFFFFu;
        const uint32_t nv = min(cur & 255u, x0) | max(cur >> 8, x1) << 8;
        if (nv == cur) return;
        const uint32_t prev = atomicCAS(w, old, (old & ~(0xFFFFu << sh)) | (nv << sh));
        if (prev == old) return;
        old = prev;
    }
}

__device__ inline unsigned long long block_max_u64_all(unsigned long long v,
                                                       unsigned long long* red) {
#pragma unroll
    for (int o = 32; o > 0; o >>= 1) {
        const unsigned long long t = __shfl_xor(v, o, 64);
        v = t > v ? t : v;
    }
    __syncthreads();
    if ((threadIdx.x & 63) == 0) red[threadIdx.x >> 6] = v;
    __syncthreads();
#pragma unroll
    for (int i = 0; i < NTB / 64; ++i) v = red[i] > v ? red[i] : v;
    return v;
}

__global__ __launch_bounds__(NTB) void level_sorted_kernel(
    const uint16_t* __restrict__ slist_g, const int32_t* __restrict__ cgt_g,
    const int32_t* __restrict__ lev_list, const int32_t* __restrict__ nlev,
    int32_t* __restrict__ boxes, int H, int W, uint32_t* __restrict__ hlist_g,
    uint64_t* __restrict__ dbg, int nch, int compress) {
    uint64_t ph[8] = {0, 0, 0, 0, 0, 0, 0, 0};
    uint32_t n_comp = 0, n_fallback = 0;
    uint64_t tp = rt();
#define SPHASE(k) do { if (dbg) { uint64_t t_ = rt(); ph[k] += t_ - tp; tp = t_; } } while (0)
    __shared__ uint32_t bm[IH * IWPR];
    __shared__ uint32_t db[IH * IWPR];
    __shared__ uint32_t pk[INB];
    __shared__ uint32_t ar[INB];
    __shared__ uint32_t xr[INB / 2];
    __shared__ uint16_t lst[SCAP];
    __shared__ unsigned long long redl[NTB / 64 + 1];
    __shared__ int s_nhook, s_nmerge;
    __shared__ unsigned long long s_pbest, s_best;
    const int b = blockIdx.x / nch, chunk = blockIdx.x % nch;
    uint32_t* hlist = hlist_g + (long)blockIdx.x * INB;
    const uint16_t* slist = slist_g + (long)b * H * W;
    const int32_t* cgt = cgt_g + (long)b * 257;
    const int nl = __builtin_amdgcn_readfirstlane(nlev[b]);
    const int l0 = nl * chunk / nch, l1 = nl * (chunk + 1) / nch;
    if (l0 >= l1) return;
    const int wpr = (W + 31) / 32, NW = H * wpr;
    const int BW = (W + 1) / 2, BH = (H + 1) / 2, NB = BH * BW;
    const int tid = threadIdx.x, lane = tid & 63, wid = tid >> 6;
    for (int i = tid; i < NB; i += NTB) {
        pk[i] = INACT;
        ar[i] = 0;
    }
    for (int i = tid; i < (NB + 1) / 2; i += NTB) xr[i] = XR_EMPTY | XR_EMPTY << 16;
    for (int w = tid; w < NW; w += NTB) bm[w] = 0u;
    if (tid == 0) s_pbest = 0;
    LevelCtx cx{bm, H, W, wpr, BW};
    uint32_t pwin = INACT;
    auto isnew = [&](int y, int x) -> int {
        if ((unsigned)y >= (unsigned)H || (unsigned)x >= (unsigned)W) return 0;
        return (db[y * wpr + (x >> 5)] >> (x & 31)) & 1;
    };
    int s_hi = 0;

    for (int li = l1 - 1; li >= l0; --li) {
        const int L = __builtin_amdgcn_readfirstlane(lev_list[b * 256 + li]);
        const int s0 = s_hi, s1 = min(max(__builtin_amdgcn_readfirstlane(cgt[L]), s0), H * W);
        s_hi = s1;
        const int nnew = s1 - s0;
        const bool inl = nnew <= SCAP;
        for (int w = tid; w < NW; w += NTB) db[w] = 0u;
        if (tid == 0) {
            s_nhook = 0;
            s_nmerge = 0;
            s_best = 0;
        }
        __syncthreads();
        SPHASE(0);
        for (int it = tid; it < nnew; it += NTB) {
            const uint32_t pp = slist[s0 + it];
            if (inl) lst[it] = (uint16_t)pp;
            const int y = (int)(pp >> 8), x = (int)(pp & 255);
            const uint32_t bit = 1u << (x & 31);
            atomicOr(&bm[y * wpr + (x >> 5)], bit);
            atomicOr(&db[y * wpr + (x >> 5)], bit);
            const uint32_t blk = (y >> 1) * BW + (x >> 1);
            if (pk[blk] == INACT) pk[blk] = blk << 16 | 0xFFFFu;
        }
        __syncthreads();
        auto newpx = [&](int it) -> uint32_t { return inl ? (uint32_t)lst[it] : slist[s0 + it]; };
        SPHASE(1);
        for (int it = tid; it < nnew * 3; it += NTB) {
            const int q = it / 3, k = it - 3 * q;
            const uint32_t pp = newpx(q);
            const int y = (int)(pp >> 8), x = (int)(pp & 255);
            const int sy = (y & 1) ? 1 : -1, sx = (x & 1) ? 1 : -1;
            int ny, nx, set;
            if (k == 0) {
                ny = y; nx = x + sx;
                set = cx.bit(y, nx) | cx.bit(y - sy, nx);
            } else if (k == 1) {
                ny = y + sy; nx = x;
                set = cx.bit(ny, x) | cx.bit(ny, x - sx);
            } else {
                ny = y + sy; nx = x + sx;
                set = cx.bit(ny, nx);
            }
            if (set)
                unite_pk(pk, (y >> 1) * BW + (x >> 1), (ny >> 1) * BW + (nx >> 1), hlist,
                         &s_nhook);
        }
        __syncthreads();
        SPHASE(2);
        const int nhook = s_nhook;
        const volatile uint32_t* hlv = hlist;
        for (int it = tid; it < nhook; it += NTB) {
            const uint32_t e = hlv[it], i = e >> 16, k = e & 0xFFFFu;
            if (k != 0xFFFFu) {
                const uint32_t r = find_root_pk(pk, i);
                const uint32_t a = ar[i];
                const uint32_t xi = (xr[i >> 1] >> ((i & 1u) * 16)) & 0xFFFFu;
                atomicAdd(&ar[r], a & SAMASK);
                ar_max_y1(&ar[r], a >> 24);
                xr_widen(xr, r, xi & 255u, xi >> 8);
                atomicMin(&pk[r], r << 16 | k);
                s_nmerge = 1;
            }
        }
        SPHASE(3);
        for (int it = tid; it < nnew * 4; it += NTB) {
            {
                const uint32_t pp = newpx(it >> 2);
                const int y = (int)(pp >> 8), x = (int)(pp & 255);
                const uint32_t r = find_root_pk(pk, (y >> 1) * BW + (x >> 1));
                if ((it & 3) == 0) atomicMin(&pk[r], r << 16 | (uint32_t)(y * W + x));
                const int wy = y - 1 + ((it >> 1) & 1), wx = x - 1 + (it & 1);
                int cn = 0, co = 0;
                bool owner = true;
#pragma unroll
                for (int k = 0; k < 4; ++k) {
                    const int qy = wy + (k >> 1), qx = wx + (k & 1);
                    const int nbit = cx.bit(qy, qx), nw = isnew(qy, qx);
                    cn += nbit;
                    co += nbit & (nw ^ 1);
                    if (nw && (qy < y || (qy == y && qx < x))) owner = false;
                }
                const int dsum = owner ? win_contrib(cn) - win_contrib(co) : 0;
                if (dsum) atomicAdd(&ar[r], (uint32_t)dsum);
                if ((it & 3) == 0) {
                    xr_widen(xr, r, (uint32_t)x, (uint32_t)x);
                    ar_max_y1(&ar[r], (uint32_t)y);
                }
            }
        }
        __syncthreads();
        SPHASE(4);
        if (__builtin_amdgcn_readfirstlane(s_nmerge) && compress) {
            ++n_comp;
            for (int i = tid; i < NB; i += NTB) {
                const uint32_t w = pk[i];
                if (w == INACT || (w >> 16) == (uint32_t)i) continue;
                const uint32_t p = w >> 16;
                if ((pk[p] >> 16) == p) continue;
                pk[i] = find_root_pk(pk, p) << 16 | 0xFFFFu;
            }
        }
        unsigned long long best = 0;
        auto cand = [&](uint32_t x) {
            const uint32_t r = find_root_pk(pk, x);
            if (r != x) pk[x] = r << 16 | 0xFFFFu;
            const unsigned long long a =
                ((unsigned long long)(ar[r] & SAMASK) << 32) | (pk[r] & 0xFFFFu);
            best = a > best ? a : best;
        };
        for (int it = tid; it < nnew; it += NTB) {
            const uint32_t pp = newpx(it);
            cand(((pp >> 8) >> 1) * BW + ((pp & 255) >> 1));
        }
        for (int it = tid; it < nhook; it += NTB) cand(hlv[it] >> 16);
        if (tid == 0 && pwin != INACT) cand(pwin);
        SPHASE(5);
#pragma unroll
        for (int o = 32; o > 0; o >>= 1) {
            const unsigned long long t = __shfl_xor(best, o, 64);
            best = t > best ? t : best;
        }
        if (lane == 0 && best) atomicMax(&s_best, best);
        __syncthreads();
        best = s_best;
        if (__builtin_amdgcn_readfirstlane((int)(best < s_pbest))) {
            ++n_fallback;
            best = 0;
            for (int i = tid; i < NB; i += NTB) {
                const uint32_t v = pk[i];
                if ((v >> 16) == (uint32_t)i) {
                    const unsigned long long a =
                        ((unsigned long long)(ar[i] & SAMASK) << 32) | (v & 0xFFFFu);
                    best = a > best ? a : best;
                }
            }
            best = block_max_u64_all(best, redl);
        }
        const uint32_t fp = (uint32_t)best;
        const uint32_t wroot = find_root_pk(pk, ((fp / W) >> 1) * BW + ((fp % W) >> 1));
        SPHASE(6);
        if (tid == 0) {
            const uint32_t xw = (xr[wroot >> 1] >> ((wroot & 1u) * 16)) & 0xFFFFu;
            int32_t* box = boxes + ((long)b * 256 + L) * 4;
            box[0] = (int)(xw & 255u);
            box[1] = (int)(fp / W);
            box[2] = min((int)(xw >> 8) + 1, W - 1);
            box[3] = min((int)(ar[wroot] >> 24) + 1, H - 1);
            s_pbest = best;
        }
        pwin = wroot;
        __syncthreads();
        SPHASE(7);
    }
    if (dbg && tid == 0) {
        uint64_t* d = dbg + (long)blockIdx.x * DBG_SLOTS;
        for (int k = 0; k < 8; ++k) d[k] = ph[k];
        d[8] = l1 - l0;
        d[9] = n_comp;
        d[10] = n_fallback;
    }
#undef SPHASE
}
}

static size_t inc_list_offset(int B, int H, int W) {
    const size_t psi = ((size_t)B * H * W + 15) / 16 * 16;
    return (psi + (size_t)B * (256 + 256 + 1) * sizeof(int32_t) + 255) / 256 * 256;
}

static size_t inc_hook_offset(int B, int H, int W) {
    return inc_list_offset(B, H, W) + (size_t)B * INC_MAX_CHUNKS * IH * IW * sizeof(uint32_t);
}

static size_t sorted_list_offset(int B, int H, int W) {
    return inc_hook_offset(B, H, W) + (size_t)B * INC_MAX_CHUNKS * INB * sizeof(uint32_t);
}

static size_t sorted_cgt_offset(int B, int H, int W) {
    return (sorted_list_offset(B, H, W) + (size_t)B * H * W * sizeof(uint16_t) + 255) / 256 * 256;
}

extern "C" void tcam_bbox_set_chunks(int n) { g_bbox_chunks = n; }

extern "C" size_t tcam_bbox_ws_bytes(int B, int H, int W) {
    return sorted_cgt_offset(B, H, W) + (size_t)B * 257 * sizeof(int32_t);
}

extern "C" int tcam_bbox_levels(const uint8_t* cam_u8, int32_t* boxes, int32_t* vmax,
                                void* ws, int B, int H, int W, void* stream) {
    TCAM_REQUIRE(cam_u8 && boxes && vmax && ws && B > 0);
    TCAM_REQUIRE(H > 0 && W > 0 && H <= BIGH && W <= BIGW);
    const bool big = H > MAXH || W > MAXW;
    hipStream_t st = as_stream(stream);
    uint8_t* psi = (uint8_t*)ws;
    int32_t* canon = (int32_t*)((char*)ws + ((size_t)B * H * W + 15) / 16 * 16);
    int32_t* lev_list = canon + (size_t)B * 256;
    int32_t* nlev = lev_list + (size_t)B * 256;
    const bool small = !big && H <= IH && W <= IW && !g_dbg;
    const bool sorted = small && g_level_variant == 0;
    uint16_t* slist = sorted ? reinterpret_cast<uint16_t*>((char*)ws + sorted_list_offset(B, H, W))
                             : nullptr;
    int32_t* cgt = reinterpret_cast<int32_t*>((char*)ws + sorted_cgt_offset(B, H, W));
    if (big)
        fill_kernel<BIGH, BIGP, false><<<B, NTB, 0, st>>>(cam_u8, psi, vmax, canon, lev_list,
                                                          nlev, H, W, g_dbg, nullptr, nullptr);
    else if (g_fill_variant == 1)
        fill_kernel<MAXH, MAXP, true><<<B, NTB, 0, st>>>(cam_u8, psi, vmax, canon, lev_list,
                                                         nlev, H, W, g_dbg, slist, cgt);
    else if (g_fill_variant == 0)
        fill_scan_kernel<<<B, NTS, 0, st>>>(cam_u8, psi, vmax, canon, lev_list, nlev, H, W, slist,
                                            cgt, g_dbg, g_fill_waves, g_fill_maxit);
    else if (H <= 224 && W <= 224)
        fill_reg_kernel<56><<<B, NTF, 0, st>>>(cam_u8, psi, vmax, canon, lev_list, nlev, H, W,
                                               g_dbg, slist, cgt);
    else
        fill_reg_kernel<64><<<B, NTF, 0, st>>>(cam_u8, psi, vmax, canon, lev_list, nlev, H, W,
                                               g_dbg, slist, cgt);
    TCAM_CHECK_LAUNCH();
    static const int nch = [] {
        const char* e = getenv("TCAM_BBOX_INC_CHUNKS");
        const int v = e ? atoi(e) : INC_CHUNKS;
        return v >= 1 && v <= INC_MAX_CHUNKS ? v : INC_CHUNKS;
    }();
    const int nc = (g_bbox_chunks >= 1 && g_bbox_chunks <= INC_MAX_CHUNKS) ? g_bbox_chunks : nch;
    static const int compress = [] {
        const char* e = getenv("TCAM_BBOX_COMPRESS");
        return e ? atoi(e) : 0;
    }();
    if (sorted)
        level_sorted_kernel<<<B * nc, NTB, 0, st>>>(
            slist, cgt, lev_list, nlev, boxes, H, W,
            reinterpret_cast<uint32_t*>((char*)ws + inc_hook_offset(B, H, W)), g_inc_dbg, nc,
            compress);
    else if (small && g_level_variant == 2)
        level_inc_kernel<<<B * nc, NTB, 0, st>>>(
            psi, lev_list, nlev, boxes, H, W,
            reinterpret_cast<uint32_t*>((char*)ws + inc_list_offset(B, H, W)),
            reinterpret_cast<uint32_t*>((char*)ws + inc_hook_offset(B, H, W)), g_inc_dbg, nc);
    else if (big)
        level_kernel<BIGH, BIGW, 4><<<B * LEVEL_CHUNKS, NTB, 0, st>>>(
            psi, vmax, lev_list, nlev, boxes, H, W, g_dbg ? g_dbg + 0 : nullptr);
    else
        level_kernel<MAXH, MAXW, 2><<<B * LEVEL_CHUNKS, NTB, 0, st>>>(
            psi, vmax, lev_list, nlev, boxes, H, W, g_dbg ? g_dbg + 0 : nullptr);
    TCAM_CHECK_LAUNCH();
    expand_kernel<<<cdiv((long)B * 256, 256), 256, 0, st>>>(canon, vmax, boxes, B);
    TCAM_CHECK_LAUNCH();
    return TCAM_OK;
}

extern "C" int tcam_bbox_scan_line(const uint8_t* p, const uint8_t* u, uint8_t* out, int n,
                                   int mode, void* stream) {
    TCAM_REQUIRE(p && u && out && n > 0 && n <= 256);
    scan_line_kernel<<<1, 64, 0, as_stream(stream)>>>(p, u, out, n, mode);
    TCAM_CHECK_LAUNCH();
    return TCAM_OK;
}

extern "C" int tcam_bbox_set_inc_debug(uint64_t* buf) {
    g_inc_dbg = buf;
    return TCAM_OK;
}

extern "C" int tcam_bbox_level_variant(int v) {
    g_level_variant = v;
    return TCAM_OK;
}

extern "C" int tcam_bbox_fill_variant(int v) {
    if (v >= 1000) {
        g_fill_maxit = v == 1000 ? 1 << 30 : v - 1000;
        return TCAM_OK;
    }
    if (v >= 100) {
        g_fill_waves = v - 100;
        return TCAM_OK;
    }
    g_fill_variant = v;
    return TCAM_OK;
}

extern "C" int tcam_bbox_set_debug(uint64_t* buf) {
    g_dbg = buf;
    return TCAM_OK;
}

extern "C" int tcam_box_accumulate(const int32_t* boxes, const int32_t* vmax, const double* taus,
                                   int T, const int32_t* gt, const int32_t* ngt, int G,
                                   const int32_t* top1, const int32_t* top5,
                                   const double* iou_thr, int n_iou, int32_t* counters,
                                   double* best_iou, int B, void* stream) {
    TCAM_REQUIRE(boxes && vmax && taus && gt && ngt && top1 && top5 && iou_thr && counters);
    TCAM_REQUIRE(T > 0 && G > 0 && n_iou > 0 && B > 0);
    long total = (long)B * T;
    accumulate_kernel<<<cdiv(total, 256), 256, 0, as_stream(stream)>>>(
        boxes, vmax, taus, T, gt, ngt, G, top1, top5, iou_thr, n_iou, counters, best_iou, B);
    TCAM_CHECK_LAUNCH();
    return TCAM_OK;
}
```

tcam_wsol_video_amd/csrc/bbox_multi.hip:

```cpp
#include "common.h"

namespace {

constexpr int MT = 1024;
constexpr int MAX_HW = 320;
constexpr int MWPR = MAX_HW / 32;
constexpr int MAX_G = 64;

__device__ __forceinline__ int ald(const int* p) {
    return __hip_atomic_load(p, __ATOMIC_RELAXED, __HIP_MEMORY_SCOPE_AGENT);
}
__device__ __forceinline__ void ast(int* p, int v) {
    __hip_atomic_store(p, v, __ATOMIC_RELAXED, __HIP_MEMORY_SCOPE_AGENT);
}

__device__ int uf_find(int* par, int x) {
    int cur = ald(par + x);
    if (cur != x) {
        int prev = x, nxt;
        while (cur > (nxt = ald(par + cur))) {
            ast(par + prev, nxt);
            prev = cur;
            cur = nxt;
        }
    }
    return cur;
}

__device__ void uf_unite(int* par, int a, int b) {
    int ar = uf_find(par, a), br = uf_find(par, b);
    while (ar != br) {
        if (ar < br) {
            const int old = atomicCAS(par + br, br, ar);
            if (old == br) return;
            br = old;
        } else {
            const int old = atomicCAS(par + ar, ar, br);
            if (old == ar) return;
            ar = old;
        }
    }
}

struct Scratch {
    int* par;
    int* x0;
    int* x1;
    int* y1;
};

__device__ __forceinline__ int bm_bit(const uint32_t* bm, int wpr, int y, int x) {
    return (bm[y * wpr + (x >> 5)] >> (x & 31)) & 1;
}

__device__ void label_level(const uint8_t* __restrict__ u8, int L, int H, int W, uint32_t* bm,
                            const Scratch& s) {
    const int tid = threadIdx.x;
    const int wpr = (W + 31) >> 5;
    const int HW = H * W;
    for (int w = tid; w < H * wpr; w += MT) {
        const int y = w / wpr, x0 = (w - y * wpr) * 32;
        uint32_t bits = 0;
        const uint8_t* row = u8 + (long)y * W;
        for (int e = 0; e < 32; ++e) {
            const int x = x0 + e;
            if (x < W && (int)row[x] > L) bits |= 1u << e;
        }
        bm[w] = bits;
    }
    __syncthreads();
    for (int p = tid; p < HW; p += MT) {
        const int y = p / W, x = p - y * W;
        const uint32_t wd = bm[y * wpr + (x >> 5)];
        const int c = (wd >> (x & 31)) & 1;
        const uint32_t other = (c ? ~wd : wd) & ((2u << (x & 31)) - 1u);
        const int start = other ? (32 - __builtin_clz(other)) : 0;
        ast(s.par + p, y * W + (x & ~31) + start);
        ast(s.x0 + p, W);
        ast(s.x1 + p, -1);
        ast(s.y1 + p, -1);
    }
    __threadfence();
    __syncthreads();
    for (int p = tid; p < HW; p += MT) {
        const int y = p / W, x = p - y * W;
        const int c = bm_bit(bm, wpr, y, x);
        const int cw = x > 0 ? bm_bit(bm, wpr, y, x - 1) : -1;
        if ((x & 31) == 0 && x > 0 && cw == c) uf_unite(s.par, p, p - 1);
        if (y == 0) continue;
        const int cn = bm_bit(bm, wpr, y - 1, x);
        const int cnw = x > 0 ? bm_bit(bm, wpr, y - 1, x - 1) : -1;
        if (c) {
            const int cne = x + 1 < W ? bm_bit(bm, wpr, y - 1, x + 1) : 0;
            if (cn) {
                if (!(cw == 1 && cnw == 1)) uf_unite(s.par, p, p - W);
            } else {
                if (cnw == 1 && cw != 1) uf_unite(s.par, p, p - W - 1);
                if (cne) uf_unite(s.par, p, p - W + 1);
            }
        } else if (!cn && !(cw == 0 && cnw == 0)) {
            uf_unite(s.par, p, p - W);
        }
    }
    __threadfence();
    __syncthreads();
    for (int p = tid; p < HW; p += MT) {
        const int y = p / W, x = p - y * W;
        const int c = bm_bit(bm, wpr, y, x);
        if (x > 0 && bm_bit(bm, wpr, y, x - 1) == c) continue;
        int j = x >> 5;
        uint32_t m = c ? ~bm[y * wpr + j] : bm[y * wpr + j];
        m &= ~0u << (x & 31);
        while (!m && ++j < wpr) m = c ? ~bm[y * wpr + j] : bm[y * wpr + j];
        const int xe = min(W - 1, (m ? 32 * j + __builtin_ctz(m) : 32 * wpr) - 1);
        const int r = uf_find(s.par, p);
        atomicMin(s.x0 + r, x);
        atomicMax(s.x1 + r, xe);
        atomicMax(s.y1 + r, y);
    }
    __threadfence();
    __syncthreads();
}

__device__ __forceinline__ bool root_box(const Scratch& s, const uint32_t* bm, int r, int H,
                                         int W, int& hole, int (&b)[4]) {
    const int wpr = (W + 31) >> 5;
    const int y0 = r / W, x0 = ald(s.x0 + r), x1 = ald(s.x1 + r), y1 = ald(s.y1 + r);
    hole = !bm_bit(bm, wpr, y0, r - y0 * W);
    if (hole) {
        if (x0 == 0 || y0 == 0 || x1 == W - 1 || y1 == H - 1) return false;
        b[0] = x0 - 1;
        b[1] = y0 - 1;
        b[2] = min(x1 + 2, W - 1);
        b[3] = min(y1 + 2, H - 1);
    } else {
        b[0] = x0;
        b[1] = y0;
        b[2] = min(x1 + 1, W - 1);
        b[3] = min(y1 + 1, H - 1);
    }
    return true;
}

__device__ __forceinline__ double max_iou(const int (&a)[4], const int* gt, int ng) {
    double best = 0.0;
    for (int g = 0; g < ng; ++g) {
        const int* q = gt + 4 * g;
        const long mnx = max(a[0], q[0]), mny = max(a[1], q[1]);
        const long mxx = min(a[2], q[2]), mxy = min(a[3], q[3]);
        const long inter = max(0L, mxx - mnx + 1) * max(0L, mxy - mny + 1);
        const long area_a = (long)(a[2] - a[0] + 1) * (a[3] - a[1] + 1);
        const long area_b = (long)(q[2] - q[0] + 1) * (q[3] - q[1] + 1);
        const long den = area_a + area_b - inter;
        const double iou = den <= 0 ? 0.0 : (double)inter / (double)den;
        if (g == 0 || iou > best) best = iou;
    }
    return best;
}

__global__ __launch_bounds__(256) void u8_levels_kernel(const uint8_t* __restrict__ cam_u8,
                                                        int HW, int32_t* __restrict__ vmax,
                                                        int32_t* __restrict__ canon,
                                                        int32_t* __restrict__ lev_list,
                                                        int32_t* __restrict__ nlev) {
    __shared__ int hist[257];
    __shared__ int cnt;
    const int b = blockIdx.x, tid = threadIdx.x;
    hist[tid] = 0;
    if (tid == 0) {
        hist[256] = 0;
        cnt = 0;
    }
    __syncthreads();
    const uint8_t* u = cam_u8 + (long)b * HW;
    for (int i = tid; i < HW; i += 256) atomicOr(&hist[u[i]], 1);
    __syncthreads();
    int vm = 0;
    for (int v = 255; v > 0; --v)
        if (hist[v]) { vm = v; break; }
    if (tid == 0) vmax[b] = vm;
    const int L = tid;
    int c = -1;
    if (L < vm) {
        int v = L + 1;
        while (!hist[v]) ++v;
        c = v - 1;
    }
    canon[b * 256 + L] = c;
    if (L < vm && hist[L + 1]) lev_list[b * 256 + atomicAdd(&cnt, 1)] = L;
    __syncthreads();
    if (tid == 0) nlev[b] = cnt;
}

__global__ __launch_bounds__(MT) void multi_level_kernel(
    const uint8_t* __restrict__ cam_u8, const int32_t* __restrict__ gt,
    const int32_t* __restrict__ ngt, int G, const int32_t* __restrict__ lev_list,
    const int32_t* __restrict__ nlev, double* __restrict__ iou_out, int H, int W, int chunks,
    int* __restrict__ scratch) {
    __shared__ uint32_t bm[MAX_HW * MWPR];
    __shared__ int gbox[4 * MAX_G];
    __shared__ unsigned long long best_bits;
    const int b = blockIdx.x / chunks, chunk = blockIdx.x % chunks;
    const int nl = nlev[b];
    if (chunk >= nl) return;
    const int HW = H * W, tid = threadIdx.x;
    int* base = scratch + (long)blockIdx.x * 4 * HW;
    const Scratch s{base, base + HW, base + 2 * HW, base + 3 * HW};
    const int ng = min(ngt[b], MAX_G);
    for (int i = tid; i < 4 * ng; i += MT) gbox[i] = gt[(long)b * G * 4 + i];
    const uint8_t* u8 = cam_u8 + (long)b * HW;
    for (int li = chunk; li < nl; li += chunks) {
        const int L = lev_list[b * 256 + li];
        if (tid == 0) best_bits = 0ull;
        label_level(u8, L, H, W, bm, s);
        double best = 0.0;
        for (int p = tid; p < HW; p += MT) {
            if (ald(s.par + p) != p) continue;
            int hole, box[4];
            if (!root_box(s, bm, p, H, W, hole, box)) continue;
            best = fmax(best, max_iou(box, gbox, ng));
        }
        atomicMax(&best_bits, (unsigned long long)__double_as_longlong(best));
        __syncthreads();
        if (tid == 0) iou_out[b * 256 + L] = __longlong_as_double((long long)best_bits);
        __syncthreads();
    }
}

__global__ __launch_bounds__(MT) void contour_records_kernel(const uint8_t* __restrict__ u8,
                                                             int L, int H, int W,
                                                             int* __restrict__ scratch,
                                                             int32_t* __restrict__ rec, int cap,
                                                             int32_t* __restrict__ count) {
    __shared__ uint32_t bm[MAX_HW * MWPR];
    const int HW = H * W, tid = threadIdx.x;
    const Scratch s{scratch, scratch + HW, scratch + 2 * HW, scratch + 3 * HW};
    if (tid == 0) *count = 0;
    label_level(u8, L, H, W, bm, s);
    for (int p = tid; p < HW; p += MT) {
        if (ald(s.par + p) != p) continue;
        int hole, box[4];
        if (!root_box(s, bm, p, H, W, hole, box)) continue;
        int parent = -1;
        if (p % W > 0) {
            const int q = uf_find(s.par, p - 1);
            if (hole) {
                parent = q;
            } else {
                int h2, b2[4];
                if (root_box(s, bm, q, H, W, h2, b2)) parent = q;
            }
        }
        const int k = atomicAdd(count, 1);
        if (k < cap) {
            int32_t* r = rec + 8 * (long)k;
            r[0] = hole; r[1] = p; r[2] = parent;
            r[3] = box[0]; r[4] = box[1]; r[5] = box[2]; r[6] = box[3]; r[7] = 0;
        }
    }
}

__global__ void multi_accumulate_kernel(const double* __restrict__ iou_tab,
                                        const int32_t* __restrict__ canon,
                                        const int32_t* __restrict__ vmax,
                                        const double* __restrict__ taus, int T,
                                        const int32_t* __restrict__ gt,
                                        const int32_t* __restrict__ ngt, int G,
                                        const int32_t* __restrict__ top1,
                                        const int32_t* __restrict__ top5,
                                        const double* __restrict__ iou_thr, int n_iou,
                                        int32_t* __restrict__ counters,
                                        double* __restrict__ best_iou, int B) {
    const long id = (long)blockIdx.x * blockDim.x + threadIdx.x;
    if (id >= (long)B * T) return;
    const int b = (int)(id / T), i = (int)(id % T);
    const int vm = vmax[b];
    const int thr = (int)(taus[i] * (double)vm);
    double best;
    if (thr < vm) {
        best = iou_tab[b * 256 + canon[b * 256 + thr]];
    } else {
        const int zero[4] = {0, 0, 0, 0};
        best = max_iou(zero, gt + (long)b * G * 4, ngt[b]);
    }
    if (best_iou) best_iou[id] = best;
    for (int j = 0; j < n_iou; ++j) {
        if (best >= iou_thr[j]) {
            atomicAdd(&counters[(0 * n_iou + j) * T + i], 1);
            if (top1[b]) atomicAdd(&counters[(1 * n_iou + j) * T + i], 1);
            if (top5[b]) atomicAdd(&counters[(2 * n_iou + j) * T + i], 1);
        }
    }
}

__global__ void flag_count_kernel(const int32_t* __restrict__ flags, int B,
                                  int32_t* __restrict__ acc) {
    int v = 0;
    for (int i = threadIdx.x; i < B; i += 64) v += flags[i] != 0;
    for (int o = 32; o > 0; o >>= 1) v += __shfl_xor(v, o, 64);
    if (threadIdx.x == 0) acc[0] += v;
}

int multi_chunks(int B) {
    const int c = 256 / (B > 0 ? B : 1);
    return c < 1 ? 1 : (c > 255 ? 255 : c);
}

size_t lev_bytes(int B) { return ((size_t)B * (256 + 256 + 1) * sizeof(int32_t) + 255) / 256 * 256; }

}

extern "C" size_t tcam_bbox_multi_ws_bytes(int B, int H, int W) {
    return lev_bytes(B) + (size_t)B * multi_chunks(B) * 4 * H * W * sizeof(int32_t);
}

extern "C" int tcam_bbox_multi_iou(const uint8_t* cam_u8, const int32_t* gt, const int32_t* ngt,
                                   int G, double* iou, int32_t* vmax, int32_t* canon, void* ws,
                                   int B, int H, int W, void* stream) {
    TCAM_REQUIRE(cam_u8 && gt && ngt && iou && vmax && canon && ws && B > 0 && G > 0);
    TCAM_REQUIRE(G <= MAX_G && H > 0 && W > 0 && H <= MAX_HW && W <= MAX_HW);
    hipStream_t st = as_stream(stream);
    int32_t* lev_list = (int32_t*)ws;
    int32_t* nlev = lev_list + (size_t)B * 256;
    int* scratch = (int*)((char*)ws + lev_bytes(B));
    const int chunks = multi_chunks(B);
    u8_levels_kernel<<<B, 256, 0, st>>>(cam_u8, H * W, vmax, canon, lev_list, nlev);
    TCAM_CHECK_LAUNCH();
    multi_level_kernel<<<B * chunks, MT, 0, st>>>(cam_u8, gt, ngt, G, lev_list, nlev, iou, H, W,
                                                  chunks, scratch);
    TCAM_CHECK_LAUNCH();
    return TCAM_OK;
}

extern "C" int tcam_box_accumulate_multi(const double* iou, const int32_t* canon,
                                         const int32_t* vmax, const double* taus, int T,
                                         const int32_t* gt, const int32_t* ngt, int G,
                                         const int32_t* top1, const int32_t* top5,
                                         const double* iou_thr, int n_iou, int32_t* counters,
                                         double* best_iou, int B, void* stream) {
    TCAM_REQUIRE(iou && canon && vmax && taus && gt && ngt && top1 && top5 && iou_thr &&
                 counters);
    TCAM_REQUIRE(T > 0 && G > 0 && n_iou > 0 && B > 0);
    const long total = (long)B * T;
    multi_accumulate_kernel<<<cdiv(total, 256), 256, 0, as_stream(stream)>>>(
        iou, canon, vmax, taus, T, gt, ngt, G, top1, top5, iou_thr, n_iou, counters, best_iou,
        B);
    TCAM_CHECK_LAUNCH();
    return TCAM_OK;
}

extern "C" size_t tcam_bbox_contours_ws_bytes(int H, int W) {
    return (size_t)4 * H * W * sizeof(int32_t);
}

extern "C" int tcam_bbox_contours(const uint8_t* cam_u8, int level, int32_t* records, int cap,
                                  int32_t* count, void* ws, int H, int W, void* stream) {
    TCAM_REQUIRE(cam_u8 && records && count && ws && cap > 0 && level >= 0 && level < 256);
    TCAM_REQUIRE(H > 0 && W > 0 && H <= MAX_HW && W <= MAX_HW);
    contour_records_kernel<<<1, MT, 0, as_stream(stream)>>>(cam_u8, level, H, W, (int*)ws,
                                                             records, cap, count);
    TCAM_CHECK_LAUNCH();
    return TCAM_OK;
}

extern "C" int tcam_flag_count(const int32_t* flags, int B, int32_t* acc, void* stream) {
    TCAM_REQUIRE(flags && acc && B > 0);
    flag_count_kernel<<<1, 64, 0, as_stream(stream)>>>(flags, B, acc);
    TCAM_CHECK_LAUNCH();
    return TCAM_OK;
}
```

tcam_wsol_video_amd/metrics.py:

```python
from __future__ import annotations

import os
from copy import deepcopy
from typing import Dict, List, Optional, Sequence, Union

import numpy as np
import torch
import torch.distributed as dist

from . import ops

_RESIZE_LENGTH = 224


def check_scoremap_validity(scoremap) -> None:
    if not isinstance(scoremap, np.ndarray):
        raise TypeError(f"Scoremap must be a numpy array; it is {type(scoremap)}.")
    if scoremap.dtype != float:
        raise TypeError(f"Scoremap must be of np.float type; it is of {scoremap.dtype} type.")
    if len(scoremap.shape) != 2:
        raise ValueError(f"Scoremap must be a 2D array; it is {len(scoremap.shape)}D.")
    if np.isnan(scoremap).any():
        raise ValueError("Scoremap must not contain nans.")
    if (scoremap > 1).any() or (scoremap < 0).any():
        raise ValueError("Scoremap must be in range [0, 1]."
                         f"scoremap.min()={scoremap.min()}, scoremap.max()={scoremap.max()}.")


def check_box_convention(boxes, convention: str) -> None:
    boxes = np.asarray(boxes)
    if (boxes < 0).any():
        raise RuntimeError("Box coordinates must be non-negative.")
    if len(boxes.shape) == 1:
        boxes = np.expand_dims(boxes, 0)
    elif len(boxes.shape) != 2:
        raise RuntimeError("Box array must have dimension (4) or (num_boxes, 4).")
    if boxes.shape[1] != 4:
        raise RuntimeError("Box array must have dimension (4) or (num_boxes, 4).")
    if convention == "x0y0x1y1":
        widths, heights = boxes[:, 2] - boxes[:, 0], boxes[:, 3] - boxes[:, 1]
    elif convention == "xywh":
        widths, heights = boxes[:, 2], boxes[:, 3]
    else:
        raise ValueError(f"Unknown convention {convention}.")
    if (widths < 0).any() or (heights < 0).any():
        raise RuntimeError(f"Boxes do not follow the {convention} convention.")


def resize_bbox(box, image_size, resize_size):
    check_box_convention(np.array(box), "x0y0x1y1")
    x0, y0, x1, y1 = map(float, box)
    iw, ih = map(float, image_size)
    nw, nh = map(float, resize_size)
    return int(x0 * nw / iw), int(y0 * nh / ih), int(x1 * nw / iw), int(y1 * nh / ih)


def calculate_multiple_iou(box_a, box_b) -> np.ndarray:
    box_a, box_b = np.asarray(box_a), np.asarray(box_b)
    check_box_convention(box_a, "x0y0x1y1")
    check_box_convention(box_b, "x0y0x1y1")
    a, b = box_a[:, None, :], box_b[None, :, :]
    ix = np.maximum(0, np.minimum(a[..., 2], b[..., 2]) - np.maximum(a[..., 0], b[..., 0]) + 1)
    iy = np.maximum(0, np.minimum(a[..., 3], b[..., 3]) - np.maximum(a[..., 1], b[..., 1]) + 1)
    inter = ix * iy
    area_a = (a[..., 2] - a[..., 0] + 1) * (a[..., 3] - a[..., 1] + 1)
    area_b = (b[..., 2] - b[..., 0] + 1) * (b[..., 3] - b[..., 1] + 1)
    den = area_a + area_b - inter
    deg = np.where(den <= 0)
    den[deg] = 1
    ious = inter / den
    ious[deg] = 0
    return ious


def _meta_path(metadata, key: str) -> str:
    if isinstance(metadata, str):
        return f"{metadata.rstrip('/')}/{key}.txt"
    if isinstance(metadata, dict):
        return metadata[key]
    return getattr(metadata, key)


def load_resized_boxes(metadata, resize_length: int = _RESIZE_LENGTH) -> Dict[str, list]:
    with open(_meta_path(metadata, "image_ids")) as f:
        ids = [ln.strip("\n") for ln in f.readlines()]
    boxes: Dict[str, list] = {}
    with open(_meta_path(metadata, "localization")) as f:
        for ln in f.readlines():
            i, a, b, c, d = ln.strip("\n").split(",")
            boxes.setdefault(i, []).append((float(a), float(b), float(c), float(d)))
    sizes = {}
    with open(_meta_path(metadata, "image_sizes")) as f:
        for ln in f.readlines():
            i, w, h = ln.strip("\n").split(",")
            sizes[i] = (int(w), int(h))
    return {i: [resize_bbox(b, sizes[i], (resize_length, resize_length)) for b in boxes[i]]
            for i in ids}


def _u8_from_scoremap(scoremap: np.ndarray, device) -> torch.Tensor:
    check_scoremap_validity(scoremap)
    u8 = (scoremap * 255).astype(np.uint8)
    return torch.from_numpy(np.ascontiguousarray(u8))[None].to(device)


def opencv_contour_order(records: np.ndarray) -> np.ndarray:
    kids: Dict[int, list] = {}
    by_key = {}
    for r in records:
        by_key[int(r[1])] = r
        kids.setdefault(int(r[2]), []).append(int(r[1]))
    out = []
    stack = sorted(kids.get(-1, []))
    while stack:
        k = stack.pop()
        out.append(by_key[k][3:7])
        stack.extend(sorted(kids.get(k, [])))
    return np.asarray(out, dtype=np.int64).reshape(-1, 4)


def compute_bboxes_from_scoremaps(scoremap: Optional[np.ndarray], scoremap_threshold_list,
                                  multi_contour_eval: bool = False,
                                  bbox: Optional[list] = None, device="cuda"):
    taus = list(scoremap_threshold_list)
    if scoremap is None:
        assert bbox is not None
        return [np.array([bbox]) for _ in taus], [1] * len(taus)
    if multi_contour_eval:
        check_scoremap_validity(scoremap)
        u8h = np.ascontiguousarray((scoremap * 255).astype(np.uint8))
        u8 = torch.from_numpy(u8h).to(device)
        mx = int(u8h.max())
        present = np.zeros(257, bool)
        present[np.unique(u8h)] = True
        cache: Dict[int, np.ndarray] = {}
        out, counts = [], []
        for t in taus:
            thr = int(t * mx)
            if thr >= mx:
                out.append(np.zeros((1, 4), np.int64))
                counts.append(1)
                continue
            c = thr + 1
            while not present[c]:
                c += 1
            if c not in cache:
                cache[c] = opencv_contour_order(ops.bbox_contours(u8, c - 1))
            out.append(cache[c])
            counts.append(len(cache[c]))
        return out, counts
    u8 = _u8_from_scoremap(scoremap, device)
    boxes, vmax = ops.bbox_levels(u8)
    mx = int(vmax[0].item())
    table = boxes[0].cpu().numpy().astype(np.int64)
    out = []
    for t in taus:
        thr = int(t * mx)
        out.append(table[thr][None] if thr < mx else np.zeros((1, 4), np.int64))
    return out, [1] * len(taus)


_DRAIN_CHUNKS = int(os.environ.get("TCAM_BBOX_DRAIN_CHUNKS", "4"))


class BoxEvaluator:

    def __init__(self, cam_threshold_list: Sequence[float],
                 iou_threshold_list: Sequence[int] = (30, 50, 70),
                 gt_bboxes: Optional[Dict[str, list]] = None, multi_contour_eval: bool = False,
                 device: Union[str, torch.device] = "cuda", metadata=None, **unused):
        self.cam_threshold_list = list(cam_threshold_list)
        self.iou_threshold_list = list(iou_threshold_list)
        self.multi_contour_eval = multi_contour_eval
        if gt_bboxes is None and metadata is not None:
            gt_bboxes = load_resized_boxes(metadata, _RESIZE_LENGTH)
        self.gt_bboxes = gt_bboxes or {}
        self.device = torch.device(device)
        T = len(self.cam_threshold_list)
        self.taus = torch.tensor(self.cam_threshold_list, dtype=torch.float64, device=self.device)
        self.iou_thr = torch.tensor([t / 100 for t in self.iou_threshold_list],
                                    dtype=torch.float64, device=self.device)
        self.counters = torch.zeros((3, len(self.iou_threshold_list), T), dtype=torch.int32,
                                    device=self.device)
        self.cls_correct = torch.zeros(1, dtype=torch.int32, device=self.device)
        self.cnt = 0
        self.best_tau_list: List[float] = []
        self.curve_s = None
        self.top1 = None
        self.top5 = None
        self.curve_top_1_5 = None
        self._flush = None
        self._join = None

    def accumulate_batch(self, cam_u8: torch.Tensor, gt: torch.Tensor, ngt: torch.Tensor,
                         top1: torch.Tensor, top5: torch.Tensor,
                         best_iou: Optional[torch.Tensor] = None, drain: bool = False,
                         gate: Optional[torch.Tensor] = None) -> None:
        if gate is not None:
            tot, cls = self.counters, self.cls_correct
            self.counters, self.cls_correct = torch.zeros_like(tot), torch.zeros_like(cls)
            try:
                self.accumulate_batch(cam_u8, gt, ngt, top1, top5, best_iou, drain)
            finally:
                keep = (gate == 0).to(torch.int32)
                tot.add_(self.counters * keep)
                cls.add_(self.cls_correct * keep)
                self.counters, self.cls_correct = tot, cls
            return
        if self.multi_contour_eval:
            iou, canon, vmax = ops.bbox_multi_iou(cam_u8, gt, ngt)
            ops.box_accumulate_multi(iou, canon, vmax, self.taus, gt, ngt, top1, top5,
                                     self.iou_thr, self.counters, best_iou)
        else:
            boxes, vmax = ops.bbox_levels(cam_u8, chunks=_DRAIN_CHUNKS if drain else 0)
            ops.box_accumulate(boxes, vmax, self.taus, gt, ngt, top1, top5, self.iou_thr,
                               self.counters, best_iou)
        ops.flag_count(top1, self.cls_correct)
        self.cnt += int(cam_u8.shape[0])

    def accumulate(self, scoremap, image_id: str, target: int, preds_ordered,
                   bbox=None, bbox_status=None) -> None:
        if scoremap is None:
            raise NotImplementedError("C_BOX boxes are outside the TCAM hot path")
        assert bbox is None and bbox_status is None
        gt = np.asarray(self.gt_bboxes[image_id], dtype=np.int32).reshape(-1, 4)
        u8 = _u8_from_scoremap(scoremap, self.device)
        preds = list(np.asarray(preds_ordered).tolist())
        top1 = torch.tensor([int(target == preds[0])], dtype=torch.int32, device=self.device)
        top5 = torch.tensor([int(target in preds[:5])], dtype=torch.int32, device=self.device)
        self.accumulate_batch(u8, torch.from_numpy(gt)[None].to(self.device),
                              torch.tensor([gt.shape[0]], dtype=torch.int32, device=self.device),
                              top1, top5)

    def _sync(self) -> None:
        if self._flush is not None:
            self._flush()
        if self.device.type == "cuda":
            torch.cuda.synchronize(self.device)

    @property
    def num_correct(self) -> Dict[int, np.ndarray]:
        self._sync()
        c = self.counters[0].double().cpu().numpy()
        return {t: c[j] for j, t in enumerate(self.iou_threshold_list)}

    @property
    def num_correct_top1(self) -> Dict[int, np.ndarray]:
        self._sync()
        c = self.counters[1].double().cpu().numpy()
        return {t: c[j] for j, t in enumerate(self.iou_threshold_list)}

    @property
    def num_correct_top5(self) -> Dict[int, np.ndarray]:
        self._sync()
        c = self.counters[2].double().cpu().numpy()
        return {t: c[j] for j, t in enumerate(self.iou_threshold_list)}

    def _synch_across_gpus(self) -> None:
        if not (dist.is_available() and dist.is_initialized()):
            return
        if self._join is not None:
            self._join()
        elif self._flush is not None:
            self._flush()
        dist.all_reduce(self.counters)
        dist.all_reduce(self.cls_correct)
        cnt = torch.tensor([self.cnt], dtype=torch.float64, device=self.counters.device)
        dist.all_reduce(cnt)
        self.cnt = int(cnt.item())

    def classification_accuracy(self) -> float:
        self._sync()
        return int(self.cls_correct.item()) / float(self.cnt) * 100

    def compute(self) -> List[float]:
        max_box_acc = []
        self.best_tau_list = []
        self.curve_s = {"x": self.cam_threshold_list}
        self.top1, self.top5 = [], []
        self.curve_top_1_5 = {"x": self.cam_threshold_list, "top1": dict(), "top5": dict()}
        nc, n1, n5 = self.num_correct, self.num_correct_top1, self.num_correct_top5
        for thr in self.iou_threshold_list:
            acc = nc[thr] * 100. / float(self.cnt)
            max_box_acc.append(acc.max())
            self.curve_s[thr] = acc
            self.best_tau_list.append(float(self.cam_threshold_list[np.argmax(acc)]))
            loc = n1[thr] * 100. / float(self.cnt)
            self.top1.append(loc.max())
            self.curve_top_1_5["top1"][thr] = deepcopy(loc)
            loc = n5[thr] * 100. / float(self.cnt)
            self.top5.append(loc.max())
            self.curve_top_1_5["top5"][thr] = deepcopy(loc)
        return max_box_acc
```

tcam_wsol_video_amd/ops.py:

```python
from __future__ import annotations

import ctypes as C
from typing import List, Optional, Sequence, Tuple

import torch

from . import _lib
from ._lib import check, tcam_conv_dst, tcam_conv_prob, tcam_conv_src


_TIMER = None


_EVENT_POOL: list = []
_EVENT_NEXT = 0


def set_launch_timer(timer: Optional[list], reserve: int = 0) -> None:
    global _TIMER, _EVENT_NEXT
    _TIMER = timer
    if timer is not None:
        _EVENT_NEXT = 0
        _grow_event_pool(2 * int(reserve))


def _grow_event_pool(n: int) -> None:
    while len(_EVENT_POOL) < n:
        e = torch.cuda.Event(enable_timing=True)
        e.record()
        _EVENT_POOL.append(e)


def _timer_events():
    global _EVENT_NEXT
    _grow_event_pool(_EVENT_NEXT + 2)
    e = _EVENT_POOL[_EVENT_NEXT], _EVENT_POOL[_EVENT_NEXT + 1]
    _EVENT_NEXT += 2
    return e


def _timer_arm(lib, e0, e1) -> None:
    check(lib.tcam_timer_arm(e0.cuda_event, e1.cuda_event), "tcam_timer_arm")


def _timer_disarm(lib) -> None:
    check(lib.tcam_timer_arm(None, None), "tcam_timer_arm")


def _ptr(t: Optional[torch.Tensor]) -> Optional[int]:
    return None if t is None else t.data_ptr()


def _stream() -> int:
    return torch.cuda.current_stream().cuda_stream


def _dev(*ts: Optional[torch.Tensor]) -> None:
    for t in ts:
        if t is None:
            continue
        if not t.is_cuda:
            raise RuntimeError("tcam ops run on the GPU only (no CPU fallback); got a CPU tensor")
        if not t.is_contiguous():
            raise RuntimeError("tcam ops require contiguous tensors")


class ConvSrc:

    __slots__ = ("t", "stride", "up2")

    def __init__(self, t: torch.Tensor, stride: int = 1, up2: bool = False):
        self.t, self.stride, self.up2 = t, int(stride), bool(up2)


def conv_weight_dims(k: int, cout: int) -> Tuple[int, int]:
    kp, mp = C.c_int(), C.c_int()
    check(_lib.load().tcam_conv_weight_dims(k, cout, C.byref(kp), C.byref(mp)),
          "tcam_conv_weight_dims")
    return kp.value, mp.value


def pack_conv_weight(ws: Sequence[torch.Tensor]) -> torch.Tensor:
    w = torch.cat(list(ws), dim=1)
    cout, ctot, kh, kw = w.shape
    k = ctot * kh * kw
    kp, mp = conv_weight_dims(k, cout)
    wt = w.permute(2, 3, 1, 0).reshape(k, cout)
    out = torch.zeros((kp, mp), dtype=torch.float32, device=w.device)
    out[:k, :cout] = wt
    return out.contiguous()


def conv2d(srcs: Sequence[ConvSrc], wt: torch.Tensor, bias: torch.Tensor, cout: int,
           hout: int, wout: int, ksize: int, pad: int, relu: bool,
           residual: Optional[torch.Tensor] = None,
           out: Optional[torch.Tensor] = None) -> torch.Tensor:
    lib = _lib.load()
    B = srcs[0].t.shape[0]
    _dev(wt, bias, residual, *[s.t for s in srcs])
    if out is None:
        out = torch.empty((B, cout, hout, wout), device=wt.device, dtype=torch.float32)
    arr = (tcam_conv_src * len(srcs))()
    for i, s in enumerate(srcs):
        t = s.t
        assert t.dtype == torch.float32 and t.dim() == 4 and t.shape[0] == B
        arr[i] = tcam_conv_src(t.data_ptr(), t.shape[1], t.shape[2], t.shape[3], s.stride,
                               1 if s.up2 else 0)
    timer = _TIMER
    if timer is not None:
        e0, e1 = _timer_events()
        e0.record()
    check(lib.tcam_conv2d(arr, len(srcs), B, _ptr(wt), _ptr(bias), _ptr(residual), _ptr(out),
                          cout, hout, wout, ksize, ksize, pad, 1 if relu else 0, _stream()),
          "tcam_conv2d")
    if timer is not None:
        e1.record()
        kdim = wt.shape[0]
        timer.append(("conv", 2.0 * cout * kdim * B * hout * wout, e0, e1,
                      f"M{cout} K{kdim} N{B * hout * wout} k{ksize} src{len(srcs)}"))
    return out


def maxpool3x3s2(x: torch.Tensor) -> torch.Tensor:
    lib = _lib.load()
    _dev(x)
    B, Cc, H, W = x.shape
    Ho, Wo = (H - 1) // 2 + 1, (W - 1) // 2 + 1
    out = torch.empty((B, Cc, Ho, Wo), device=x.device, dtype=x.dtype)
    check(lib.tcam_maxpool3x3s2(_ptr(x), _ptr(out), B, Cc, H, W, Ho, Wo, _stream()),
          "tcam_maxpool3x3s2")
    return out


def up2_resize(x: torch.Tensor, size: Tuple[int, int]) -> torch.Tensor:
    lib = _lib.load()
    _dev(x)
    B, Cc, H, W = x.shape
    out = torch.empty((B, Cc, size[0], size[1]), device=x.device, dtype=x.dtype)
    check(lib.tcam_up2_resize(_ptr(x), _ptr(out), B, Cc, H, W, size[0], size[1], _stream()),
          "tcam_up2_resize")
    return out


def wgap(x: torch.Tensor, fc_w: torch.Tensor, fc_b: torch.Tensor) -> torch.Tensor:
    lib = _lib.load()
    _dev(x, fc_w, fc_b)
    B, Cc, H, W = x.shape
    classes = fc_w.shape[0]
    ws = torch.empty((B, Cc), device=x.device, dtype=torch.float32)
    out = torch.empty((B, classes), device=x.device, dtype=torch.float32)
    check(lib.tcam_wgap(_ptr(x), _ptr(fc_w), _ptr(fc_b), _ptr(out), _ptr(ws), B, Cc, H * W,
                        classes, _stream()), "tcam_wgap")
    return out


def seghead_cam(x: torch.Tensor, w: torch.Tensor, b: torch.Tensor, want_fcams: bool = True,
                want_u8: bool = True, argmax: bool = False):
    lib = _lib.load()
    _dev(x, w, b)
    B, Cin, H, W = x.shape
    fcams = torch.empty((B, 2, H, W), device=x.device) if want_fcams else None
    cam = torch.empty((B, H, W), device=x.device)
    u8 = torch.empty((B, H, W), device=x.device, dtype=torch.uint8) if want_u8 else None
    check(lib.tcam_seghead_cam(_ptr(x), _ptr(w), _ptr(b), _ptr(fcams), _ptr(cam), _ptr(u8), B,
                               Cin, H, W, 1 if argmax else 0, _stream()), "tcam_seghead_cam")
    return fcams, cam, u8


def std_cam(A: torch.Tensor, fc_w: torch.Tensor, cls: torch.Tensor, size: Tuple[int, int],
            want_u8: bool = True):
    lib = _lib.load()
    cls = cls.to(device=A.device, dtype=torch.int32).contiguous()
    _dev(A, fc_w, cls)
    if is_act(A):
        B, h, w, Cc = s3_dims(A)
        name = f"tcam_std_cam_{_lay(A)}"
        fn = getattr(lib, name)
    else:
        B, Cc, h, w = A.shape
        fn, name = lib.tcam_std_cam, "tcam_std_cam"
    low = torch.empty((B, h, w), device=A.device)
    cam = torch.empty((B, size[0], size[1]), device=A.device)
    u8 = torch.empty((B, size[0], size[1]), device=A.device, dtype=torch.uint8) if want_u8 else None
    check(fn(_ptr(A), _ptr(fc_w), _ptr(cls), _ptr(low), _ptr(cam), _ptr(u8), B, Cc, h, w,
             size[0], size[1], _stream()), name)
    return low, cam, u8


def temporal_max(cams: torch.Tensor, idx: torch.Tensor, t: float = 0.0) -> torch.Tensor:
    lib = _lib.load()
    idx = idx.to(device=cams.device, dtype=torch.int32).contiguous()
    _dev(cams, idx)
    N = cams.shape[0]
    hw_shape = cams.shape[1:]
    M, k1 = idx.shape
    out = torch.empty((M,) + tuple(hw_shape), device=cams.device, dtype=torch.float32)
    hw = int(torch.tensor(hw_shape).prod().item()) if len(hw_shape) else 1
    check(lib.tcam_temporal_max(_ptr(cams), _ptr(idx), _ptr(out), M, k1, hw, float(t),
                                _stream()), "tcam_temporal_max")
    return out


def temporal_cam(cams: torch.Tensor, idx: torch.Tensor, t: float = 0.0,
                 want_cam: bool = True, want_u8: bool = True):
    lib = _lib.load()
    idx = idx.to(device=cams.device, dtype=torch.int32).contiguous()
    _dev(cams, idx)
    if cams.dtype != torch.float32 or cams.dim() != 3:
        raise ValueError("cams must be a (N, H, W) float32 tensor")
    N, H, W = cams.shape
    M, k1 = idx.shape
    if M > 65535:
        raise ValueError("at most 65535 output frames per launch")
    out = torch.empty((M, H, W), device=cams.device) if want_cam else None
    u8 = torch.empty((M, H, W), device=cams.device, dtype=torch.uint8) if want_u8 else None
    scale = torch.empty(N, device=cams.device) if t > 0 else None
    check(lib.tcam_temporal_cam(_ptr(cams), N, _ptr(idx), _ptr(out), _ptr(u8), M, k1, H * W,
                                float(t), _ptr(scale), _stream()), "tcam_temporal_cam")
    return out, u8


def topk_flags(logits: torch.Tensor, target: torch.Tensor):
    lib = _lib.load()
    target = target.to(device=logits.device, dtype=torch.int32).contiguous()
    _dev(logits, target)
    B, Cc = logits.shape
    top1 = torch.empty(B, device=logits.device, dtype=torch.int32)
    top5 = torch.empty(B, device=logits.device, dtype=torch.int32)
    check(lib.tcam_topk_flags(_ptr(logits), _ptr(target), _ptr(top1), _ptr(top5), B, Cc,
                              _stream()), "tcam_topk_flags")
    return top1, top5


def bbox_levels(cam_u8: torch.Tensor, chunks: int = 0):
    lib = _lib.load()
    _dev(cam_u8)
    assert cam_u8.dtype == torch.uint8 and cam_u8.dim() == 3
    B, H, W = cam_u8.shape
    boxes = torch.empty((B, 256, 4), device=cam_u8.device, dtype=torch.int32)
    vmax = torch.empty((B,), device=cam_u8.device, dtype=torch.int32)
    ws = torch.empty(int(lib.tcam_bbox_ws_bytes(B, H, W)), device=cam_u8.device,
                     dtype=torch.uint8)
    lib.tcam_bbox_set_chunks(int(chunks))
    try:
        check(lib.tcam_bbox_levels(_ptr(cam_u8), _ptr(boxes), _ptr(vmax), _ptr(ws), B, H, W,
                                   _stream()), "tcam_bbox_levels")
    finally:
        lib.tcam_bbox_set_chunks(0)
    return boxes, vmax


def box_accumulate(boxes: torch.Tensor, vmax: torch.Tensor, taus: torch.Tensor,
                   gt: torch.Tensor, ngt: torch.Tensor, top1: torch.Tensor, top5: torch.Tensor,
                   iou_thr: torch.Tensor, counters: torch.Tensor,
                   best_iou: Optional[torch.Tensor] = None) -> torch.Tensor:
    lib = _lib.load()
    _dev(boxes, vmax, taus, gt, ngt, top1, top5, iou_thr, counters, best_iou)
    B = boxes.shape[0]
    T = taus.shape[0]
    G = gt.shape[1]
    assert taus.dtype == torch.float64 and iou_thr.dtype == torch.float64
    assert gt.dtype == torch.int32 and counters.dtype == torch.int32
    assert counters.shape == (3, iou_thr.shape[0], T)
    check(lib.tcam_box_accumulate(_ptr(boxes), _ptr(vmax), _ptr(taus), T, _ptr(gt), _ptr(ngt),
                                  G, _ptr(top1), _ptr(top5), _ptr(iou_thr), iou_thr.shape[0],
                                  _ptr(counters), _ptr(best_iou), B, _stream()),
          "tcam_box_accumulate")
    return counters


_STREAM_WS = {}


def _stream_workspace(name: str, device: torch.device, nbytes: int) -> torch.Tensor:
    key = (name, device, _stream())
    ws = _STREAM_WS.get(key)
    if ws is None or ws.numel() < nbytes:
        ws = torch.empty(max(nbytes, 256), device=device, dtype=torch.uint8)
        _STREAM_WS[key] = ws
    return ws


def bbox_multi_iou(cam_u8: torch.Tensor, gt: torch.Tensor, ngt: torch.Tensor):
    lib = _lib.load()
    _dev(cam_u8, gt, ngt)
    assert cam_u8.dtype == torch.uint8 and cam_u8.dim() == 3
    assert gt.dtype == torch.int32 and gt.dim() == 3 and gt.shape[0] == cam_u8.shape[0]
    B, H, W = cam_u8.shape
    dev = cam_u8.device
    iou = torch.empty((B, 256), device=dev, dtype=torch.float64)
    canon = torch.empty((B, 256), device=dev, dtype=torch.int32)
    vmax = torch.empty((B,), device=dev, dtype=torch.int32)
    ws = _stream_workspace("bbox_multi", dev, int(lib.tcam_bbox_multi_ws_bytes(B, H, W)))
    check(lib.tcam_bbox_multi_iou(_ptr(cam_u8), _ptr(gt), _ptr(ngt.to(torch.int32)),
                                  gt.shape[1], _ptr(iou), _ptr(vmax), _ptr(canon), _ptr(ws),
                                  B, H, W, _stream()), "tcam_bbox_multi_iou")
    return iou, canon, vmax


def box_accumulate_multi(iou: torch.Tensor, canon: torch.Tensor, vmax: torch.Tensor,
                         taus: torch.Tensor, gt: torch.Tensor, ngt: torch.Tensor,
                         top1: torch.Tensor, top5: torch.Tensor, iou_thr: torch.Tensor,
                         counters: torch.Tensor,
                         best_iou: Optional[torch.Tensor] = None) -> torch.Tensor:
    lib = _lib.load()
    _dev(iou, canon, vmax, taus, gt, ngt, top1, top5, iou_thr, counters, best_iou)
    B, T = iou.shape[0], taus.shape[0]
    assert counters.shape == (3, iou_thr.shape[0], T) and counters.dtype == torch.int32
    check(lib.tcam_box_accumulate_multi(_ptr(iou), _ptr(canon), _ptr(vmax), _ptr(taus), T,
                                        _ptr(gt), _ptr(ngt), gt.shape[1], _ptr(top1),
                                        _ptr(top5), _ptr(iou_thr), iou_thr.shape[0],
                                        _ptr(counters), _ptr(best_iou), B, _stream()),
          "tcam_box_accumulate_multi")
    return counters


def bbox_contours(cam_u8: torch.Tensor, level: int, cap: Optional[int] = None):
    lib = _lib.load()
    _dev(cam_u8)
    assert cam_u8.dtype == torch.uint8 and cam_u8.dim() == 2
    H, W = cam_u8.shape
    cap = int(cap or H * W + 4)
    dev = cam_u8.device
    rec = torch.empty((cap, 8), device=dev, dtype=torch.int32)
    cnt = torch.zeros(1, device=dev, dtype=torch.int32)
    ws = torch.empty(int(lib.tcam_bbox_contours_ws_bytes(H, W)), device=dev, dtype=torch.uint8)
    check(lib.tcam_bbox_contours(_ptr(cam_u8.contiguous()), int(level), _ptr(rec), cap,
                                 _ptr(cnt), _ptr(ws), H, W, _stream()), "tcam_bbox_contours")
    n = int(cnt.item())
    if n > cap:
        raise RuntimeError(f"bbox_contours: {n} contours > capacity {cap}")
    return rec[:n].cpu().numpy()


def flag_count(flags: torch.Tensor, acc: torch.Tensor) -> torch.Tensor:
    lib = _lib.load()
    _dev(flags, acc)
    assert flags.dtype == torch.int32 and acc.dtype == torch.int32
    check(lib.tcam_flag_count(_ptr(flags.contiguous()), flags.numel(), _ptr(acc), _stream()),
          "tcam_flag_count")
    return acc



def is_s3(t: torch.Tensor) -> bool:
    return t.dim() == 6 and t.dtype == torch.bfloat16 and t.shape[-2:] == (3, 8)


def is_s2(t: torch.Tensor) -> bool:
    return t.dim() == 6 and t.dtype == torch.float16 and t.shape[-2:] == (2, 8)


def is_s1(t: torch.Tensor) -> bool:
    return t.dim() == 6 and t.dtype == torch.float16 and t.shape[-2:] == (1, 8)


def is_act(t: torch.Tensor) -> bool:
    return is_s3(t) or is_s2(t) or is_s1(t)


def _lay(t: torch.Tensor) -> str:
    if is_s3(t):
        return "s3"
    if is_s2(t):
        return "s2"
    if is_s1(t):
        return "s1"
    raise ValueError(f"not an S3 / S2 / S1 activation tensor: {tuple(t.shape)} {t.dtype}")


FMT_LAYOUT = {"x6": "s3", "f16x3": "s2", "amp": "s1"}


def s3_dims(t: torch.Tensor) -> Tuple[int, int, int, int]:
    return t.shape[0], t.shape[1], t.shape[2], t.shape[3] * 8


def s3_empty(B: int, H: int, W: int, C: int, device) -> torch.Tensor:
    assert C % 8 == 0
    return torch.empty((B, H, W, C // 8, 3, 8), device=device, dtype=torch.bfloat16)


def s2_empty(B: int, H: int, W: int, C: int, device) -> torch.Tensor:
    assert C % 8 == 0
    return torch.empty((B, H, W, C // 8, 2, 8), device=device, dtype=torch.float16)


def s1_empty(B: int, H: int, W: int, C: int, device) -> torch.Tensor:
    assert C % 8 == 0
    return torch.empty((B, H, W, C // 8, 1, 8), device=device, dtype=torch.float16)


_EMPTY = {"s3": s3_empty, "s2": s2_empty, "s1": s1_empty}


def lay_empty(lay: str, B: int, H: int, W: int, C: int, device) -> torch.Tensor:
    return _EMPTY[lay](B, H, W, C, device)


def act_empty(like: torch.Tensor, B: int, H: int, W: int, C: int) -> torch.Tensor:
    return lay_empty(_lay(like), B, H, W, C, like.device)


def s3_from_nchw(x: torch.Tensor, cpad: Optional[int] = None, fmt: str = "x6") -> torch.Tensor:
    lib = _lib.load()
    _dev(x)
    assert x.dtype == torch.float32 and x.dim() == 4
    B, Cc, H, W = x.shape
    cpad = cpad or (Cc + 7) // 8 * 8
    lay = FMT_LAYOUT[fmt]
    out = lay_empty(lay, B, H, W, cpad, x.device)
    check(getattr(lib, f"tcam_{lay}_from_nchw")(_ptr(x), _ptr(out), B, Cc, H, W, cpad,
                                                _stream()), f"tcam_{lay}_from_nchw")
    out.tcam_logical_channels = Cc
    return out


def s3_to_nchw(t: torch.Tensor) -> torch.Tensor:
    lib = _lib.load()
    _dev(t)
    lay = _lay(t)
    B, H, W, Cc = s3_dims(t)
    out = torch.empty((B, Cc, H, W), device=t.device, dtype=torch.float32)
    check(getattr(lib, f"tcam_{lay}_to_nchw")(_ptr(t), _ptr(out), B, Cc, H, W, _stream()),
          f"tcam_{lay}_to_nchw")
    return out


def relayout(t: torch.Tensor, fmt: str) -> torch.Tensor:
    lib = _lib.load()
    _dev(t)
    if fmt == "amp":
        if is_s1(t):
            return t
        raise ValueError("S1 (amp) activations come from the amp plans, not from a relayout")
    want_s2 = fmt == "f16x3"
    if is_s2(t) == want_s2:
        return t
    B, H, W, Cc = s3_dims(t)
    out = (s2_empty if want_s2 else s3_empty)(B, H, W, Cc, t.device)
    name = "tcam_s3_to_s2" if want_s2 else "tcam_s2_to_s3"
    check(getattr(lib, name)(_ptr(t), _ptr(out), B * H * W * (Cc // 8), _stream()), name)
    return out


def scale_channels(t: torch.Tensor, e: Optional[torch.Tensor],
                   negate: bool = False) -> torch.Tensor:
    if e is None:
        return t
    if is_s2(t):
        raise ValueError("scale an S3 / S1 tensor (fp16 S2 parts could leave their range)")
    B, H, W, Cc = s3_dims(t)
    f = torch.pow(2.0, (-e if negate else e).double())
    f = torch.cat([f, torch.ones(Cc - f.numel(), dtype=torch.float64)]) if f.numel() < Cc else f
    f = f.reshape(Cc // 8, 1, 8).to(device=t.device, dtype=t.dtype)
    return t * f


def split3(x: torch.Tensor) -> Tuple[torch.Tensor, torch.Tensor, torch.Tensor]:
    hi = x.to(torch.bfloat16)
    r = x - hi.float()
    mid = r.to(torch.bfloat16)
    lo = (r - mid.float()).to(torch.bfloat16)
    return hi, mid, lo


def conv_x6_weight_dims(k: int, cout: int) -> Tuple[int, int]:
    kp, mp = C.c_int(), C.c_int()
    check(_lib.load().tcam_conv_x6_weight_dims(k, cout, C.byref(kp), C.byref(mp)),
          "tcam_conv_x6_weight_dims")
    return kp.value, mp.value


def pack_conv_weight_x6(ws: Sequence[torch.Tensor]) -> torch.Tensor:
    w = torch.cat(list(ws), dim=1).float()
    cout, ctot, kh, kw = w.shape
    k = ctot * kh * kw
    kp, mp = conv_x6_weight_dims(k, cout)
    wt = torch.zeros((kp, mp), dtype=torch.float32, device=w.device)
    wt[:k, :cout] = w.permute(2, 3, 1, 0).reshape(k, cout)
    parts = [t.view(kp // 32, 4, 8, mp).permute(0, 1, 3, 2) for t in split3(wt)]
    return torch.stack(parts, dim=2).contiguous()


def pack_conv_weight_f16(ws: Sequence[torch.Tensor]) -> Tuple[torch.Tensor, torch.Tensor]:
    w = torch.cat(list(ws), dim=1).float()
    cout, ctot, kh, kw = w.shape
    k = ctot * kh * kw
    kp, mp = conv_x6_weight_dims(k, cout)
    wt = torch.zeros((kp, mp), dtype=torch.float32, device=w.device)
    wt[:k, :cout] = w.permute(2, 3, 1, 0).reshape(k, cout)
    amax = wt.abs().amax(dim=0)
    e = torch.floor(torch.log2(torch.where(amax > 0, amax, torch.ones_like(amax))))
    scale = torch.where(amax > 0, torch.exp2(e - 14), torch.ones_like(amax)).contiguous()
    u = wt / scale
    h = u.to(torch.float16)
    lo = (u - h.float()).to(torch.float16)
    parts = [t.view(kp // 32, 4, 8, mp).permute(0, 1, 3, 2) for t in (h, lo)]
    return torch.stack(parts, dim=2).contiguous(), scale


def pack_conv_weight_h1(ws: Sequence[torch.Tensor]) -> torch.Tensor:
    w = torch.cat(list(ws), dim=1).float()
    cout, ctot, kh, kw = w.shape
    k = ctot * kh * kw
    kp, mp = conv_x6_weight_dims(k, cout)
    wt = torch.zeros((kp, mp), dtype=torch.float32, device=w.device)
    wt[:k, :cout] = w.permute(2, 3, 1, 0).reshape(k, cout)
    h = wt.to(torch.float16).view(kp // 32, 4, 8, mp).permute(0, 1, 3, 2)
    return h.unsqueeze(2).contiguous()


class StemF16:

    __slots__ = ("wt", "wscale", "bias", "nk", "cout", "cin", "k", "stride", "pad", "_tabs")

    def __init__(self, w: torch.Tensor, bias: torch.Tensor, stride: int, pad: int):
        cout, cin, kh, kw = w.shape
        assert kh == kw and cout <= 64 and cout % 8 == 0
        k = cin * kh * kw
        kp = (k + 31) // 32 * 32
        rows = w.float().permute(0, 2, 3, 1).reshape(cout, k)
        wk = torch.zeros((cout, kp, 1, 1), dtype=torch.float32, device=w.device)
        wk[:, :k, 0, 0] = rows
        self.wt, self.wscale = pack_conv_weight_f16([wk])
        self.nk = kp // 32
        self.bias = bias.float().contiguous().to(w.device)
        self.cout, self.cin, self.k, self.stride, self.pad = cout, cin, kh, stride, pad
        self._tabs = {}

    def ktab(self, device) -> torch.Tensor:
        t = self._tabs.get(device)
        if t is None:
            ir, ic = C.c_int(), C.c_int()
            check(_lib.load().tcam_stem_window(self.k, self.k, self.stride, C.byref(ir),
                                               C.byref(ic)), "tcam_stem_window")
            k = self.cin * self.k * self.k
            tab = torch.full((self.nk * 32,), -1, dtype=torch.int32)
            i = torch.arange(k)
            c, tap = i % self.cin, i // self.cin
            tab[:k] = (c * ir.value * ic.value + (tap // self.k) * ic.value +
                       tap % self.k).to(torch.int32)
            t = tab.to(device)
            self._tabs[device] = t
        return t


def stem_f16x3(x: torch.Tensor, st: StemF16) -> torch.Tensor:
    lib = _lib.load()
    _dev(x, st.wt)
    assert x.dtype == torch.float32 and x.dim() == 4 and x.shape[1] == st.cin
    x = x.contiguous()
    B, _, H, W = x.shape
    Ho = (H + 2 * st.pad - st.k) // st.stride + 1
    Wo = (W + 2 * st.pad - st.k) // st.stride + 1
    out = s2_empty(B, Ho, Wo, st.cout, x.device)
    tab = st.ktab(x.device)
    timer = _TIMER
    if timer is not None:
        e0, e1 = _timer_events()
        _timer_arm(lib, e0, e1)
    check(lib.tcam_stem_f16x3(_ptr(x), _ptr(st.wt), _ptr(st.wscale), _ptr(st.bias), _ptr(tab),
                              st.nk, _ptr(out), B, st.cin, H, W, st.cout, st.k, st.k, st.stride,
                              st.pad, _ptr(f16_overflow_flag(x.device)), _stream()),
          "tcam_stem_f16x3")
    if timer is not None:
        _timer_disarm(lib)
        timer.append(("conv", 2.0 * st.cout * st.cin * st.k * st.k * B * Ho * Wo, e0, e1,
                      f"M{st.cout} K{st.cin * st.k * st.k} N{B * Ho * Wo} k{st.k}x{st.k} stem"))
    return out


def weight_fmt(wt: torch.Tensor) -> str:
    if wt.dtype == torch.bfloat16:
        return "x6"
    return "amp" if wt.shape[2] == 1 else "f16x3"


_F16_OFLOW = {}
_F16_REDIRECT = {}


def f16_overflow_flag(device: torch.device) -> torch.Tensor:
    r = _F16_REDIRECT.get(device)
    if r is not None:
        return r
    f = _F16_OFLOW.get(device)
    if f is None:
        f = torch.zeros(1, dtype=torch.int32, device=device)
        _F16_OFLOW[device] = f
    return f


class f16_overflow_into:

    def __init__(self, flag: torch.Tensor):
        self.flag = flag

    def __enter__(self):
        dev = self.flag.device
        self._prev = _F16_REDIRECT.get(dev)
        _F16_REDIRECT[dev] = self.flag
        return self.flag

    def __exit__(self, *exc):
        dev = self.flag.device
        if self._prev is None:
            _F16_REDIRECT.pop(dev, None)
        else:
            _F16_REDIRECT[dev] = self._prev
        return False


def merge_f16_overflow(flag: torch.Tensor) -> None:
    f16_overflow_flag(flag.device).bitwise_or_(flag)


def _all_ranks_max(t: torch.Tensor) -> torch.Tensor:
    import torch.distributed as dist
    if not (dist.is_available() and dist.is_initialized()) or dist.get_world_size() == 1:
        return t
    if dist.get_backend() == "nccl":
        dist.all_reduce(t, op=dist.ReduceOp.MAX)
        return t
    h = t.cpu()
    dist.all_reduce(h, op=dist.ReduceOp.MAX)
    return h


def check_f16_overflow(device: torch.device, reset: bool = True,
                       all_ranks: bool = False) -> None:
    f = _F16_OFLOW.get(device)
    if f is None:
        f = f16_overflow_flag(device) if all_ranks else None
        if f is None:
            return
    v = f.clone()
    if reset:
        f.zero_()
    if all_ranks:
        v = _all_ranks_max(v)
    if int(v.item()):
        raise FloatingPointError(
# ... 351 lines not shown
```

Baseline: 5729.

## Tabulate sweep levels in registers, prefetch next pixels, gate accumulation kernels

The sorted level sweep kernel now loads each level and its cumulative count into per-lane registers once and reads them with readlane, instead of a scalar global load every iteration. It also prefetches the next level's pixel list during the current level and reads LDS through explicit address-space-3 pointers. Separately, the accumulate and flag-count kernels take a device gate flag and skip the counter atomics when it is set. This replaces the Python path that allocated temporary zero counters and swapped them in. Both changes are on by default and can be turned off through an environment mask, at the cost of more register use and extra template variants.

```diff
diff --git a/include/tcam_hip.h b/include/tcam_hip.h
--- a/include/tcam_hip.h
+++ b/include/tcam_hip.h
@@ -183,6 +183,8 @@
                         void* stream);
 int tcam_bbox_level_variant(int v);
 int tcam_bbox_set_inc_debug(uint64_t* buf);
+int tcam_bbox_sweep_opt(int mask);
+int tcam_bbox_sweep_scap(void);
 
 int tcam_box_accumulate(const int32_t* boxes, const int32_t* vmax,
                         const double* taus, int T, const int32_t* gt,
@@ -190,6 +192,12 @@
                         const int32_t* top5, const double* iou_thr, int n_iou,
                         int32_t* counters, double* best_iou, int B,
                         void* stream);
+int tcam_box_accumulate_gated(const int32_t* boxes, const int32_t* vmax,
+                              const double* taus, int T, const int32_t* gt,
+                              const int32_t* ngt, int G, const int32_t* top1,
+                              const int32_t* top5, const double* iou_thr, int n_iou,
+                              int32_t* counters, double* best_iou, int B,
+                              const int32_t* gate, void* stream);
 
 size_t tcam_bbox_multi_ws_bytes(int B, int H, int W);
 int tcam_bbox_multi_iou(const uint8_t* cam_u8, const int32_t* gt, const int32_t* ngt, int G,
@@ -200,11 +208,20 @@
                               const int32_t* ngt, int G, const int32_t* top1,
                               const int32_t* top5, const double* iou_thr, int n_iou,
                               int32_t* counters, double* best_iou, int B, void* stream);
+int tcam_box_accumulate_multi_gated(const double* iou, const int32_t* canon,
+                                    const int32_t* vmax, const double* taus, int T,
+                                    const int32_t* gt, const int32_t* ngt, int G,
+                                    const int32_t* top1, const int32_t* top5,
+                                    const double* iou_thr, int n_iou, int32_t* counters,
+                                    double* best_iou, int B, const int32_t* gate,
+                                    void* stream);
 size_t tcam_bbox_contours_ws_bytes(int H, int W);
 int tcam_bbox_contours(const uint8_t* cam_u8, int level, int32_t* records, int cap,
                        int32_t* count, void* ws, int H, int W, void* stream);
 
 int tcam_flag_count(const int32_t* flags, int B, int32_t* acc, void* stream);
+int tcam_flag_count_gated(const int32_t* flags, int B, int32_t* acc, const int32_t* gate,
+                          void* stream);
 
 size_t tcam_bilateral_ws_bytes(int N, int K, int H, int W, int dim);
 int tcam_bilateral_batch(const float* images, const float* ins, float* outs,
diff --git a/tcam_wsol_video_amd/_lib.py b/tcam_wsol_video_amd/_lib.py
--- a/tcam_wsol_video_amd/_lib.py
+++ b/tcam_wsol_video_amd/_lib.py
@@ -106,6 +106,13 @@
     "tcam_bbox_contours_ws_bytes": (C.c_size_t, [_I, _I]),
     "tcam_bbox_contours": (_I, [_P, _I, _P, _I, _P, _P, _I, _I, _P]),
     "tcam_flag_count": (_I, [_P, _I, _P, _P]),
+    "tcam_box_accumulate_multi_gated": (_I, [_P, _P, _P, _P, _I, _P, _P, _I, _P, _P, _P, _I, _P,
+                                             _P, _I, _P, _P]),
+    "tcam_flag_count_gated": (_I, [_P, _I, _P, _P, _P]),
+    "tcam_box_accumulate_gated": (_I, [_P, _P, _P, _I, _P, _P, _I, _P, _P, _P, _I, _P, _P, _I,
+                                       _P, _P]),
+    "tcam_bbox_sweep_opt": (_I, [_I]),
+    "tcam_bbox_sweep_scap": (_I, []),
     "tcam_bbox_levels": (_I, [_P, _P, _P, _P, _I, _I, _I, _P]),
     "tcam_bbox_scan_line": (_I, [_P, _P, _P, _I, _I, _P]),
     "tcam_s2_to_s3": (_I, [_P, _P, C.c_long, _P]),
diff --git a/tcam_wsol_video_amd/csrc/bbox.hip b/tcam_wsol_video_amd/csrc/bbox.hip
--- a/tcam_wsol_video_amd/csrc/bbox.hip
+++ b/tcam_wsol_video_amd/csrc/bbox.hip
@@ -16,6 +16,11 @@
 int g_level_variant = 0;
 int g_bbox_chunks = 0;
 uint64_t* g_inc_dbg = nullptr;
+constexpr int SWEEP_TAB = 1, SWEEP_GATE = 2, SWEEP_ALL = 3;
+int g_sweep_opt = [] {
+    const char* e = getenv("TCAM_BBOX_SWEEP_OPT");
+    return e ? atoi(e) & SWEEP_ALL : SWEEP_ALL;
+}();
 
 __device__ inline uint64_t rt() { return __builtin_amdgcn_s_memrealtime(); }
 
@@ -1041,7 +1046,7 @@
                                   const int32_t* __restrict__ top5,
                                   const double* __restrict__ iou_thr, int n_iou,
                                   int32_t* __restrict__ counters, double* __restrict__ best_iou,
-                                  int B) {
+                                  int B, const int32_t* __restrict__ gate) {
     long id = (long)blockIdx.x * blockDim.x + threadIdx.x;
     if (id >= (long)B * T) return;
     const int b = (int)(id / T), i = (int)(id % T);
@@ -1066,6 +1071,7 @@
         if (g == 0 || iou > best) best = iou;
     }
     if (best_iou) best_iou[id] = best;
+    if (gate && gate[0] != 0) return;
     for (int j = 0; j < n_iou; ++j) {
         if (best >= iou_thr[j]) {
             atomicAdd(&counters[(0 * n_iou + j) * T + i], 1);
@@ -1422,10 +1428,16 @@
 constexpr uint32_t SAMASK = (1u << 17) - 1;
 constexpr uint32_t XR_EMPTY = 0x00FFu;
 
-__device__ inline uint32_t lds_ld(const uint32_t* p) { return *(const volatile uint32_t*)p; }
-
-__device__ inline void ar_max_y1(uint32_t* w, uint32_t y) {
-    uint32_t old = lds_ld(w);
+template <bool DS> __device__ inline uint32_t lds_ld(const uint32_t* p) {
+    if (DS) return *(const volatile __attribute__((address_space(3))) uint32_t*)p;
+    return *(const volatile uint32_t*)p;
+}
+__device__ inline uint32_t lds_u16(const uint16_t* p) {
+    return *(const __attribute__((address_space(3))) uint16_t*)p;
+}
+
+template <bool DS> __device__ inline void ar_max_y1(uint32_t* w, uint32_t y) {
+    uint32_t old = lds_ld<DS>(w);
     while ((old >> 24) < y) {
         const uint32_t prev = atomicCAS(w, old, (old & 0x00FFFFFFu) | (y << 24));
         if (prev == old) return;
@@ -1433,10 +1445,11 @@
     }
 }
 
+template <bool DS>
 __device__ inline void xr_widen(uint32_t* xr, uint32_t r, uint32_t x0, uint32_t x1) {
     uint32_t* w = xr + (r >> 1);
     const int sh = (int)(r & 1u) * 16;
-    uint32_t old = lds_ld(w);
+    uint32_t old = lds_ld<DS>(w);
     for (;;) {
         const uint32_t cur = (old >> sh) & 0xFFFFu;
         const uint32_t nv = min(cur & 255u, x0) | max(cur >> 8, x1) << 8;
@@ -1462,6 +1475,7 @@
     return v;
 }
 
+template <bool TAB>
 __global__ __launch_bounds__(NTB) void level_sorted_kernel(
     const uint16_t* __restrict__ slist_g, const int32_t* __restrict__ cgt_g,
     const int32_t* __restrict__ lev_list, const int32_t* __restrict__ nlev,
@@ -1504,10 +1518,38 @@
         return (db[y * wpr + (x >> 5)] >> (x & 31)) & 1;
     };
     int s_hi = 0;
+    uint32_t tab[4] = {0u, 0u, 0u, 0u};
+    auto entry = [&](int i) -> uint32_t {
+        const int k = i >> 6;
+        const uint32_t v = k == 0 ? tab[0] : k == 1 ? tab[1] : k == 2 ? tab[2] : tab[3];
+        return (uint32_t)__builtin_amdgcn_readlane((int)v, i & 63);
+    };
+    uint32_t pf = 0;
+    if constexpr (TAB) {
+#pragma unroll
+        for (int k = 0; k < 4; ++k) {
+            const int i = k * 64 + lane;
+            if (i >= l0 && i < l1) {
+                const int Lv = lev_list[b * 256 + i];
+                tab[k] = (uint32_t)Lv << 16 | (uint32_t)min(max(cgt[Lv], 0), H * W);
+            }
+        }
+        const int n = min((int)(entry(l1 - 1) & 0xFFFFu), H * W);
+        if (tid < n) pf = slist[tid];
+    }
 
     for (int li = l1 - 1; li >= l0; --li) {
-        const int L = __builtin_amdgcn_readfirstlane(lev_list[b * 256 + li]);
-        const int s0 = s_hi, s1 = min(max(__builtin_amdgcn_readfirstlane(cgt[L]), s0), H * W);
+        int L, s1;
+        const int s0 = s_hi;
+        uint32_t pf_next = 0;
+        if constexpr (TAB) {
+            const uint32_t e = entry(li);
+            L = (int)(e >> 16);
+            s1 = min(max((int)(e & 0xFFFFu), s0), H * W);
+        } else {
+            L = __builtin_amdgcn_readfirstlane(lev_list[b * 256 + li]);
+            s1 = min(max(__builtin_amdgcn_readfirstlane(cgt[L]), s0), H * W);
+        }
         s_hi = s1;
         const int nnew = s1 - s0;
         const bool inl = nnew <= SCAP;
@@ -1520,7 +1562,7 @@
         __syncthreads();
         SPHASE(0);
         for (int it = tid; it < nnew; it += NTB) {
-            const uint32_t pp = slist[s0 + it];
+            const uint32_t pp = TAB && it < NTB ? pf : slist[s0 + it];
             if (inl) lst[it] = (uint16_t)pp;
             const int y = (int)(pp >> 8), x = (int)(pp & 255);
             const uint32_t bit = 1u << (x & 31);
@@ -1530,28 +1572,48 @@
             if (pk[blk] == INACT) pk[blk] = blk << 16 | 0xFFFFu;
         }
         __syncthreads();
-        auto newpx = [&](int it) -> uint32_t { return inl ? (uint32_t)lst[it] : slist[s0 + it]; };
+        auto px_lds = [&](int it) -> uint32_t { return lds_u16(&lst[it]); };
+        auto px_mem = [&](int it) -> uint32_t { return slist[s0 + it]; };
+        auto px_any = [&](int it) -> uint32_t {
+            return inl ? (uint32_t)lst[it] : slist[s0 + it];
+        };
+        auto with_px = [&](auto&& step) {
+            if constexpr (TAB) {
+                if (inl) step(px_lds);
+                else step(px_mem);
+            } else {
+                step(px_any);
+            }
+        };
         SPHASE(1);
-        for (int it = tid; it < nnew * 3; it += NTB) {
-            const int q = it / 3, k = it - 3 * q;
-            const uint32_t pp = newpx(q);
-            const int y = (int)(pp >> 8), x = (int)(pp & 255);
-            const int sy = (y & 1) ? 1 : -1, sx = (x & 1) ? 1 : -1;
-            int ny, nx, set;
-            if (k == 0) {
-                ny = y; nx = x + sx;
-                set = cx.bit(y, nx) | cx.bit(y - sy, nx);
-            } else if (k == 1) {
-                ny = y + sy; nx = x;
-                set = cx.bit(ny, x) | cx.bit(ny, x - sx);
-            } else {
-                ny = y + sy; nx = x + sx;
-                set = cx.bit(ny, nx);
-            }
-            if (set)
-                unite_pk(pk, (y >> 1) * BW + (x >> 1), (ny >> 1) * BW + (nx >> 1), hlist,
-                         &s_nhook);
-        }
+        if constexpr (TAB) {
+            if (li > l0) {
+                const int n1 = min(max((int)(entry(li - 1) & 0xFFFFu), s1), H * W);
+                if (tid < n1 - s1) pf_next = slist[s1 + tid];
+            }
+        }
+        with_px([&](auto newpx) {
+            for (int it = tid; it < nnew * 3; it += NTB) {
+                const int q = it / 3, k = it - 3 * q;
+                const uint32_t pp = newpx(q);
+                const int y = (int)(pp >> 8), x = (int)(pp & 255);
+                const int sy = (y & 1) ? 1 : -1, sx = (x & 1) ? 1 : -1;
+                int ny, nx, set;
+                if (k == 0) {
+                    ny = y; nx = x + sx;
+                    set = cx.bit(y, nx) | cx.bit(y - sy, nx);
+                } else if (k == 1) {
+                    ny = y + sy; nx = x;
+                    set = cx.bit(ny, x) | cx.bit(ny, x - sx);
+                } else {
+                    ny = y + sy; nx = x + sx;
+                    set = cx.bit(ny, nx);
+                }
+                if (set)
+                    unite_pk(pk, (y >> 1) * BW + (x >> 1), (ny >> 1) * BW + (nx >> 1), hlist,
+                             &s_nhook);
+            }
+        });
         __syncthreads();
         SPHASE(2);
         const int nhook = s_nhook;
@@ -1563,38 +1625,40 @@
                 const uint32_t a = ar[i];
                 const uint32_t xi = (xr[i >> 1] >> ((i & 1u) * 16)) & 0xFFFFu;
                 atomicAdd(&ar[r], a & SAMASK);
-                ar_max_y1(&ar[r], a >> 24);
-                xr_widen(xr, r, xi & 255u, xi >> 8);
+                ar_max_y1<TAB>(&ar[r], a >> 24);
+                xr_widen<TAB>(xr, r, xi & 255u, xi >> 8);
                 atomicMin(&pk[r], r << 16 | k);
                 s_nmerge = 1;
             }
         }
         SPHASE(3);
-        for (int it = tid; it < nnew * 4; it += NTB) {
-            {
-                const uint32_t pp = newpx(it >> 2);
-                const int y = (int)(pp >> 8), x = (int)(pp & 255);
-                const uint32_t r = find_root_pk(pk, (y >> 1) * BW + (x >> 1));
-                if ((it & 3) == 0) atomicMin(&pk[r], r << 16 | (uint32_t)(y * W + x));
-                const int wy = y - 1 + ((it >> 1) & 1), wx = x - 1 + (it & 1);
-                int cn = 0, co = 0;
-                bool owner = true;
-#pragma unroll
-                for (int k = 0; k < 4; ++k) {
-                    const int qy = wy + (k >> 1), qx = wx + (k & 1);
-                    const int nbit = cx.bit(qy, qx), nw = isnew(qy, qx);
-                    cn += nbit;
-                    co += nbit & (nw ^ 1);
-                    if (nw && (qy < y || (qy == y && qx < x))) owner = false;
-                }
-                const int dsum = owner ? win_contrib(cn) - win_contrib(co) : 0;
-                if (dsum) atomicAdd(&ar[r], (uint32_t)dsum);
-                if ((it & 3) == 0) {
-                    xr_widen(xr, r, (uint32_t)x, (uint32_t)x);
-                    ar_max_y1(&ar[r], (uint32_t)y);
-                }
-            }
-        }
+        with_px([&](auto newpx) {
+            for (int it = tid; it < nnew * 4; it += NTB) {
+                {
+                    const uint32_t pp = newpx(it >> 2);
+                    const int y = (int)(pp >> 8), x = (int)(pp & 255);
+                    const uint32_t r = find_root_pk(pk, (y >> 1) * BW + (x >> 1));
+                    if ((it & 3) == 0) atomicMin(&pk[r], r << 16 | (uint32_t)(y * W + x));
+                    const int wy = y - 1 + ((it >> 1) & 1), wx = x - 1 + (it & 1);
+                    int cn = 0, co = 0;
+                    bool owner = true;
+#pragma unroll
+                    for (int k = 0; k < 4; ++k) {
+                        const int qy = wy + (k >> 1), qx = wx + (k & 1);
+                        const int nbit = cx.bit(qy, qx), nw = isnew(qy, qx);
+                        cn += nbit;
+                        co += nbit & (nw ^ 1);
+                        if (nw && (qy < y || (qy == y && qx < x))) owner = false;
+                    }
+                    const int dsum = owner ? win_contrib(cn) - win_contrib(co) : 0;
+                    if (dsum) atomicAdd(&ar[r], (uint32_t)dsum);
+                    if ((it & 3) == 0) {
+                        xr_widen<TAB>(xr, r, (uint32_t)x, (uint32_t)x);
+                        ar_max_y1<TAB>(&ar[r], (uint32_t)y);
+                    }
+                }
+            }
+        });
         __syncthreads();
         SPHASE(4);
         if (__builtin_amdgcn_readfirstlane(s_nmerge) && compress) {
@@ -1615,10 +1679,12 @@
                 ((unsigned long long)(ar[r] & SAMASK) << 32) | (pk[r] & 0xFFFFu);
             best = a > best ? a : best;
         };
-        for (int it = tid; it < nnew; it += NTB) {
-            const uint32_t pp = newpx(it);
-            cand(((pp >> 8) >> 1) * BW + ((pp & 255) >> 1));
-        }
+        with_px([&](auto newpx) {
+            for (int it = tid; it < nnew; it += NTB) {
+                const uint32_t pp = newpx(it);
+                cand(((pp >> 8) >> 1) * BW + ((pp & 255) >> 1));
+            }
+        });
         for (int it = tid; it < nhook; it += NTB) cand(hlv[it] >> 16);
         if (tid == 0 && pwin != INACT) cand(pwin);
         SPHASE(5);
@@ -1656,6 +1722,7 @@
             s_pbest = best;
         }
         pwin = wroot;
+        pf = pf_next;
         __syncthreads();
         SPHASE(7);
     }
@@ -1734,12 +1801,14 @@
         const char* e = getenv("TCAM_BBOX_COMPRESS");
         return e ? atoi(e) : 0;
     }();
-    if (sorted)
-        level_sorted_kernel<<<B * nc, NTB, 0, st>>>(
+    if (sorted) {
+        auto kern = level_sorted_kernel<false>;
+        if (g_sweep_opt & SWEEP_TAB) kern = level_sorted_kernel<true>;
+        kern<<<B * nc, NTB, 0, st>>>(
             slist, cgt, lev_list, nlev, boxes, H, W,
             reinterpret_cast<uint32_t*>((char*)ws + inc_hook_offset(B, H, W)), g_inc_dbg, nc,
             compress);
-    else if (small && g_level_variant == 2)
+    } else if (small && g_level_variant == 2)
         level_inc_kernel<<<B * nc, NTB, 0, st>>>(
             psi, lev_list, nlev, boxes, H, W,
             reinterpret_cast<uint32_t*>((char*)ws + inc_list_offset(B, H, W)),
@@ -1774,6 +1843,14 @@
     return TCAM_OK;
 }
 
+extern "C" int tcam_bbox_sweep_opt(int mask) {
+    const int prev = g_sweep_opt;
+    if (mask >= 0) g_sweep_opt = mask & SWEEP_ALL;
+    return prev;
+}
+
+extern "C" int tcam_bbox_sweep_scap(void) { return SCAP; }
+
 extern "C" int tcam_bbox_fill_variant(int v) {
     if (v >= 1000) {
         g_fill_maxit = v == 1000 ? 1 << 30 : v - 1000;
@@ -1789,6 +1866,22 @@
 
 extern "C" int tcam_bbox_set_debug(uint64_t* buf) {
     g_dbg = buf;
+    return TCAM_OK;
+}
+
+extern "C" int tcam_box_accumulate_gated(const int32_t* boxes, const int32_t* vmax,
+                                         const double* taus, int T, const int32_t* gt,
+                                         const int32_t* ngt, int G, const int32_t* top1,
+                                         const int32_t* top5, const double* iou_thr, int n_iou,
+                                         int32_t* counters, double* best_iou, int B,
+                                         const int32_t* gate, void* stream) {
+    TCAM_REQUIRE(boxes && vmax && taus && gt && ngt && top1 && top5 && iou_thr && counters);
+    TCAM_REQUIRE(T > 0 && G > 0 && n_iou > 0 && B > 0);
+    long total = (long)B * T;
+    accumulate_kernel<<<cdiv(total, 256), 256, 0, as_stream(stream)>>>(
+        boxes, vmax, taus, T, gt, ngt, G, top1, top5, iou_thr, n_iou, counters, best_iou, B,
+        gate);
+    TCAM_CHECK_LAUNCH();
     return TCAM_OK;
 }
 
@@ -1797,11 +1890,6 @@
                                    const int32_t* top1, const int32_t* top5,
                                    const double* iou_thr, int n_iou, int32_t* counters,
                                    double* best_iou, int B, void* stream) {
-    TCAM_REQUIRE(boxes && vmax && taus && gt && ngt && top1 && top5 && iou_thr && counters);
-    TCAM_REQUIRE(T > 0 && G > 0 && n_iou > 0 && B > 0);
-    long total = (long)B * T;
-    accumulate_kernel<<<cdiv(total, 256), 256, 0, as_stream(stream)>>>(
-        boxes, vmax, taus, T, gt, ngt, G, top1, top5, iou_thr, n_iou, counters, best_iou, B);
-    TCAM_CHECK_LAUNCH();
-    return TCAM_OK;
-}
+    return tcam_box_accumulate_gated(boxes, vmax, taus, T, gt, ngt, G, top1, top5, iou_thr,
+                                     n_iou, counters, best_iou, B, nullptr, stream);
+}
diff --git a/tcam_wsol_video_amd/csrc/bbox_multi.hip b/tcam_wsol_video_amd/csrc/bbox_multi.hip
--- a/tcam_wsol_video_amd/csrc/bbox_multi.hip
+++ b/tcam_wsol_video_amd/csrc/bbox_multi.hip
@@ -270,7 +270,8 @@
                                         const int32_t* __restrict__ top5,
                                         const double* __restrict__ iou_thr, int n_iou,
                                         int32_t* __restrict__ counters,
-                                        double* __restrict__ best_iou, int B) {
+                                        double* __restrict__ best_iou, int B,
+                                        const int32_t* __restrict__ gate) {
     const long id = (long)blockIdx.x * blockDim.x + threadIdx.x;
     if (id >= (long)B * T) return;
     const int b = (int)(id / T), i = (int)(id % T);
@@ -284,6 +285,7 @@
         best = max_iou(zero, gt + (long)b * G * 4, ngt[b]);
     }
     if (best_iou) best_iou[id] = best;
+    if (gate && gate[0] != 0) return;
     for (int j = 0; j < n_iou; ++j) {
         if (best >= iou_thr[j]) {
             atomicAdd(&counters[(0 * n_iou + j) * T + i], 1);
@@ -294,7 +296,8 @@
 }
 
 __global__ void flag_count_kernel(const int32_t* __restrict__ flags, int B,
-                                  int32_t* __restrict__ acc) {
+                                  int32_t* __restrict__ acc, const int32_t* __restrict__ gate) {
+    if (gate && gate[0] != 0) return;
     int v = 0;
     for (int i = threadIdx.x; i < B; i += 64) v += flags[i] != 0;
     for (int o = 32; o > 0; o >>= 1) v += __shfl_xor(v, o, 64);
@@ -332,21 +335,33 @@
     return TCAM_OK;
 }
 
+extern "C" int tcam_box_accumulate_multi_gated(const double* iou, const int32_t* canon,
+                                               const int32_t* vmax, const double* taus, int T,
+                                               const int32_t* gt, const int32_t* ngt, int G,
+                                               const int32_t* top1, const int32_t* top5,
+                                               const double* iou_thr, int n_iou,
+                                               int32_t* counters, double* best_iou, int B,
+                                               const int32_t* gate, void* stream) {
+    TCAM_REQUIRE(iou && canon && vmax && taus && gt && ngt && top1 && top5 && iou_thr &&
+                 counters);
+    TCAM_REQUIRE(T > 0 && G > 0 && n_iou > 0 && B > 0);
+    const long total = (long)B * T;
+    multi_accumulate_kernel<<<cdiv(total, 256), 256, 0, as_stream(stream)>>>(
+        iou, canon, vmax, taus, T, gt, ngt, G, top1, top5, iou_thr, n_iou, counters, best_iou,
+        B, gate);
+    TCAM_CHECK_LAUNCH();
+    return TCAM_OK;
+}
+
 extern "C" int tcam_box_accumulate_multi(const double* iou, const int32_t* canon,
                                          const int32_t* vmax, const double* taus, int T,
                                          const int32_t* gt, const int32_t* ngt, int G,
                                          const int32_t* top1, const int32_t* top5,
                                          const double* iou_thr, int n_iou, int32_t* counters,
                                          double* best_iou, int B, void* stream) {
-    TCAM_REQUIRE(iou && canon && vmax && taus && gt && ngt && top1 && top5 && iou_thr &&
-                 counters);
-    TCAM_REQUIRE(T > 0 && G > 0 && n_iou > 0 && B > 0);
-    const long total = (long)B * T;
-    multi_accumulate_kernel<<<cdiv(total, 256), 256, 0, as_stream(stream)>>>(
-        iou, canon, vmax, taus, T, gt, ngt, G, top1, top5, iou_thr, n_iou, counters, best_iou,
-        B);
-    TCAM_CHECK_LAUNCH();
-    return TCAM_OK;
+    return tcam_box_accumulate_multi_gated(iou, canon, vmax, taus, T, gt, ngt, G, top1, top5,
+                                           iou_thr, n_iou, counters, best_iou, B, nullptr,
+                                           stream);
 }
 
 extern "C" size_t tcam_bbox_contours_ws_bytes(int H, int W) {
@@ -363,9 +378,14 @@
     return TCAM_OK;
 }
 
+extern "C" int tcam_flag_count_gated(const int32_t* flags, int B, int32_t* acc,
+                                     const int32_t* gate, void* stream) {
+    TCAM_REQUIRE(flags && acc && B > 0);
+    flag_count_kernel<<<1, 64, 0, as_stream(stream)>>>(flags, B, acc, gate);
+    TCAM_CHECK_LAUNCH();
+    return TCAM_OK;
+}
+
 extern "C" int tcam_flag_count(const int32_t* flags, int B, int32_t* acc, void* stream) {
-    TCAM_REQUIRE(flags && acc && B > 0);
-    flag_count_kernel<<<1, 64, 0, as_stream(stream)>>>(flags, B, acc);
-    TCAM_CHECK_LAUNCH();
-    return TCAM_OK;
-}
+    return tcam_flag_count_gated(flags, B, acc, nullptr, stream);
+}
diff --git a/tcam_wsol_video_amd/metrics.py b/tcam_wsol_video_amd/metrics.py
--- a/tcam_wsol_video_amd/metrics.py
+++ b/tcam_wsol_video_amd/metrics.py
@@ -196,7 +196,7 @@
                          top1: torch.Tensor, top5: torch.Tensor,
                          best_iou: Optional[torch.Tensor] = None, drain: bool = False,
                          gate: Optional[torch.Tensor] = None) -> None:
-        if gate is not None:
+        if gate is not None and not ops.bbox_sweep_opt() & 2:
             tot, cls = self.counters, self.cls_correct
             self.counters, self.cls_correct = torch.zeros_like(tot), torch.zeros_like(cls)
             try:
@@ -210,12 +210,12 @@
         if self.multi_contour_eval:
             iou, canon, vmax = ops.bbox_multi_iou(cam_u8, gt, ngt)
             ops.box_accumulate_multi(iou, canon, vmax, self.taus, gt, ngt, top1, top5,
-                                     self.iou_thr, self.counters, best_iou)
+                                     self.iou_thr, self.counters, best_iou, gate=gate)
         else:
             boxes, vmax = ops.bbox_levels(cam_u8, chunks=_DRAIN_CHUNKS if drain else 0)
             ops.box_accumulate(boxes, vmax, self.taus, gt, ngt, top1, top5, self.iou_thr,
-                               self.counters, best_iou)
-        ops.flag_count(top1, self.cls_correct)
+                               self.counters, best_iou, gate=gate)
+        ops.flag_count(top1, self.cls_correct, gate=gate)
         self.cnt += int(cam_u8.shape[0])
 
     def accumulate(self, scoremap, image_id: str, target: int, preds_ordered,
diff --git a/tcam_wsol_video_amd/ops.py b/tcam_wsol_video_amd/ops.py
--- a/tcam_wsol_video_amd/ops.py
+++ b/tcam_wsol_video_amd/ops.py
@@ -250,22 +250,39 @@
     return boxes, vmax
 
 
+def bbox_sweep_opt(mask: int = -1) -> int:
+    return int(_lib.load().tcam_bbox_sweep_opt(int(mask)))
+
+
+def bbox_sweep_scap() -> int:
+    return int(_lib.load().tcam_bbox_sweep_scap())
+
+
+def _gate(gate: Optional[torch.Tensor], like: torch.Tensor) -> None:
+    if gate is not None:
+        _dev(gate, like)
+        assert gate.dtype == torch.int32 and gate.numel() == 1
+
+
 def box_accumulate(boxes: torch.Tensor, vmax: torch.Tensor, taus: torch.Tensor,
                    gt: torch.Tensor, ngt: torch.Tensor, top1: torch.Tensor, top5: torch.Tensor,
                    iou_thr: torch.Tensor, counters: torch.Tensor,
-                   best_iou: Optional[torch.Tensor] = None) -> torch.Tensor:
+                   best_iou: Optional[torch.Tensor] = None,
+                   gate: Optional[torch.Tensor] = None) -> torch.Tensor:
     lib = _lib.load()
     _dev(boxes, vmax, taus, gt, ngt, top1, top5, iou_thr, counters, best_iou)
+    _gate(gate, counters)
     B = boxes.shape[0]
     T = taus.shape[0]
     G = gt.shape[1]
     assert taus.dtype == torch.float64 and iou_thr.dtype == torch.float64
     assert gt.dtype == torch.int32 and counters.dtype == torch.int32
     assert counters.shape == (3, iou_thr.shape[0], T)
-    check(lib.tcam_box_accumulate(_ptr(boxes), _ptr(vmax), _ptr(taus), T, _ptr(gt), _ptr(ngt),
-                                  G, _ptr(top1), _ptr(top5), _ptr(iou_thr), iou_thr.shape[0],
-                                  _ptr(counters), _ptr(best_iou), B, _stream()),
-          "tcam_box_accumulate")
+    check(lib.tcam_box_accumulate_gated(_ptr(boxes), _ptr(vmax), _ptr(taus), T, _ptr(gt),
+                                        _ptr(ngt), G, _ptr(top1), _ptr(top5), _ptr(iou_thr),
+                                        iou_thr.shape[0], _ptr(counters), _ptr(best_iou), B,
+                                        _ptr(gate), _stream()),
+          "tcam_box_accumulate_gated")
     return counters
 
 
@@ -302,16 +319,19 @@
                          taus: torch.Tensor, gt: torch.Tensor, ngt: torch.Tensor,
                          top1: torch.Tensor, top5: torch.Tensor, iou_thr: torch.Tensor,
                          counters: torch.Tensor,
-                         best_iou: Optional[torch.Tensor] = None) -> torch.Tensor:
+                         best_iou: Optional[torch.Tensor] = None,
+                         gate: Optional[torch.Tensor] = None) -> torch.Tensor:
     lib = _lib.load()
     _dev(iou, canon, vmax, taus, gt, ngt, top1, top5, iou_thr, counters, best_iou)
+    _gate(gate, counters)
     B, T = iou.shape[0], taus.shape[0]
     assert counters.shape == (3, iou_thr.shape[0], T) and counters.dtype == torch.int32
-    check(lib.tcam_box_accumulate_multi(_ptr(iou), _ptr(canon), _ptr(vmax), _ptr(taus), T,
-                                        _ptr(gt), _ptr(ngt), gt.shape[1], _ptr(top1),
-                                        _ptr(top5), _ptr(iou_thr), iou_thr.shape[0],
-                                        _ptr(counters), _ptr(best_iou), B, _stream()),
-          "tcam_box_accumulate_multi")
+    check(lib.tcam_box_accumulate_multi_gated(_ptr(iou), _ptr(canon), _ptr(vmax), _ptr(taus), T,
+                                              _ptr(gt), _ptr(ngt), gt.shape[1], _ptr(top1),
+                                              _ptr(top5), _ptr(iou_thr), iou_thr.shape[0],
+                                              _ptr(counters), _ptr(best_iou), B, _ptr(gate),
+                                              _stream()),
+          "tcam_box_accumulate_multi_gated")
     return counters
 
 
@@ -333,12 +353,14 @@
     return rec[:n].cpu().numpy()
 
 
-def flag_count(flags: torch.Tensor, acc: torch.Tensor) -> torch.Tensor:
+def flag_count(flags: torch.Tensor, acc: torch.Tensor,
+               gate: Optional[torch.Tensor] = None) -> torch.Tensor:
     lib = _lib.load()
     _dev(flags, acc)
+    _gate(gate, acc)
     assert flags.dtype == torch.int32 and acc.dtype == torch.int32
-    check(lib.tcam_flag_count(_ptr(flags.contiguous()), flags.numel(), _ptr(acc), _stream()),
-          "tcam_flag_count")
+    check(lib.tcam_flag_count_gated(_ptr(flags.contiguous()), flags.numel(), _ptr(acc),
+                                    _ptr(gate), _stream()), "tcam_flag_count_gated")
     return acc
 
 
```

New measurement: 5728 (median of 2 runs). About the same (-0.0%).
